# daveredrum/D3Net

Measured on AMD Instinct MI355X. Metric: scenes/sec fwd+bwd (PointGroup+speaker), higher is better.
Workload: dtype bf16

## Files before the change

d3net_amd/_lib.py:

```python
import ctypes as C
import os

_HERE = os.path.dirname(os.path.abspath(__file__))
SO_PATH = os.path.join(_HERE, "lib", "libd3hip.so")

ERRORS = {-1: "D3_ERR_WORKSPACE", -2: "D3_ERR_RANGE (coordinate/batch outside key range)",
          -3: "D3_ERR_ARG", -4: "D3_ERR_OVERFLOW"}


class D3Error(RuntimeError):
    pass


_lib = None
vp, i32, i64, f32, sz = C.c_void_p, C.c_int, C.c_longlong, C.c_float, C.c_size_t
f64 = C.c_double
pi = C.POINTER(C.c_int)

SIGNATURES = {
    "d3_version": (i32, []),
    "d3_arch": (C.c_char_p, []),
    "d3_sec_mean": (i32, [vp, vp, vp, i32, i32, vp]),
    "d3_sec_min": (i32, [vp, vp, vp, i32, i32, vp]),
    "d3_sec_max": (i32, [vp, vp, vp, i32, i32, vp]),
    "d3_cluster_select": (i32, [vp, vp, vp, vp, vp, i32, vp, vp, vp, vp, vp]),
    "d3_cluster_select2": (i32, [vp, vp, vp, vp, vp, i32, i32, vp, vp, vp, vp, vp, vp]),
    "d3_cluster_merge": (i32, [vp, i32, vp, i32, vp, i32, vp, i32, vp, vp, vp, vp, vp, vp]),
    "d3_proposal_prepare": (i32, [vp, vp, vp, i32, vp, vp, vp, vp, f32, f32, i32, vp, vp, vp, vp, vp]),
    "d3_cluster_coords_stats": (i32, [vp, vp, vp, vp, vp, vp, i32, vp]),
    "d3_cluster_coords_stats_ws_bytes": (sz, [i64]),
    "d3_cluster_coords_stats2": (i32, [vp, vp, vp, i64, vp, vp, vp, i32, vp, sz, vp]),
    "d3_cluster_transform": (i32, [vp, vp, vp, vp, vp, vp, i64, vp]),
    "d3_cluster_norm_params": (i32, [vp, vp, vp, i32, f32, f32, vp, vp, vp, vp, vp, vp]),
    "d3_roipool_fp": (i32, [vp, vp, vp, vp, i32, i32, vp]),
    "d3_roipool_bp": (i32, [vp, vp, vp, vp, i32, i32, vp]),
    "d3_get_iou": (i32, [vp, vp, vp, vp, vp, i32, i32, vp]),
    "d3_voxelize_fp": (i32, [vp, vp, vp, i32, i32, i32, i32, vp]),
    "d3_voxelize_fp2": (i32, [vp, i32, vp, i32, vp, vp, i32, i32, i32, vp]),
    "d3_voxelize_bp": (i32, [vp, vp, vp, i32, i32, i32, i32, vp]),
    "d3_point_recover_fp": (i32, [vp, vp, vp, i32, i32, i32, vp]),
    "d3_point_recover_bp": (i32, [vp, vp, vp, i32, i32, i32, vp]),
    "d3_voxelize_idx_ws_bytes": (sz, [i32]),
    "d3_voxelize_idx_count": (i32, [vp, i32, i32, i32, vp, vp, sz, pi, pi, vp]),
    "d3_voxelize_idx_fill": (i32, [vp, i32, i32, i32, vp, vp, sz, vp, vp, i32, i32, vp]),
    "d3_ballquery_ws_bytes": (sz, [i32]),
    "d3_ballquery_ws_bytes_single_pass": (sz, [i32]),
    "d3_ballquery_count": (i32, [vp, vp, vp, i32, f32, vp, vp, sz, pi, vp]),
    "d3_ballquery_fill": (i32, [vp, vp, vp, i32, f32, vp, vp, sz, vp, i64, vp]),
    "d3_ballquery_cap": (i32, []),
    "d3_ballquery_padded": (i32, [vp, vp, vp, i32, f32, vp, vp, sz, vp, vp]),
    "d3_bfs_cluster_ws_bytes": (sz, [i32]),
    "d3_bfs_cluster_erec_bytes": (sz, [i64]),
    "d3_bfs_cluster_run": (i32, [vp, vp, vp, i32, i32, vp, sz, vp, sz, i64, i32, vp, i64, vp, i64, pi, pi, vp]),
    "d3_bfs_cluster_begin": (i32, [vp, vp, vp, i32, i32, vp, sz, vp, sz, i64, i32, vp, i64, vp, i64, C.POINTER(vp), vp]),
    "d3_bfs_cluster_end": (i32, [vp, pi, pi]),
    "d3_coordmap_ws_bytes": (sz, [i32]),
    "d3_kmap_k3": (i32, [vp, i32, i32, vp, sz, vp, vp]),
    "d3_kmap_k3_pack16": (i32, [vp, i32, vp, vp, vp]),
    "d3_kmap_k3_16": (i32, [vp, i32, i32, vp, sz, vp, vp, vp, vp]),
    "d3_net_set_k3_16": (i32, [vp, vp, vp]),
    "d3_kmap_k3_q16_bytes": (sz, [i32]),
    "d3_kmap_k3_packq": (i32, [vp, i32, vp, vp, vp]),
    "d3_spconv_fwd3_nparts": (i32, [i32, i32, i32]),
    "d3_spconv_fwd3": (i32, [vp, i32, vp, vp, vp, i32, vp, i32, vp, vp, i32, i32, i32, i32, i32, vp]),
    "d3_spconv_fwd3_bnbwd": (i32, [vp, i32, vp, vp, vp, i32, vp, vp, vp, i32, vp, vp, vp, vp, f32, i32, i32, i32, i32, i32, i32, vp]),
    "d3_spconv_fwd3_launches": (i64, []),
    "d3_spconv_last_nparts": (i32, []),
    "d3_net_padded_channels": (i32, [vp]),
    "d3_net_padcast": (i32, [vp, vp, vp, i64, vp]),
    "d3_net_set_padded_input": (i32, [vp, vp]),
    "d3_spconv_t16_launches": (C.c_longlong, []),
    "d3_kmap_down_count": (i32, [vp, i32, i32, vp, sz, vp, vp, pi, vp]),
    "d3_kmap_down_fill": (i32, [vp, i32, i32, vp, sz, vp, vp, vp, vp, vp, i32, vp]),
    "d3_kmap_pyramid": (i32, [vp, i32, i32, vp, sz, vp, vp, vp, vp, vp, pi, vp]),
    "d3_kmap_pyramid_begin": (i32, [vp, i32, i32, vp, sz, vp, vp, vp, vp, vp, C.POINTER(C.c_void_p), vp]),
    "d3_kmap_pyramid_end": (i32, [vp, pi, i32]),
    "d3_kmap_down_fill2": (i32, [i32, i32, vp, vp, vp, vp, vp]),
    "d3_spconv_fwd": (i32, [vp, vp, vp, vp, i32, i32, i32, i32, i32, i32, vp]),
    "d3_spconv_wgrad": (i32, [vp, vp, vp, vp, i32, i32, i32, i32, i32, i32, vp]),
    "d3_spconv_pack_bytes": (sz, [i32, i32, i32]),
    "d3_spconv_pack_bytes_ex": (sz, [i32, i32, i32, i32]),
    "d3_spconv_pack": (i32, [vp, vp, i32, i32, i32, i32, vp]),
    "d3_spconv_fwd2_nparts": (i32, [i32, i32, i32, i32]),
    "d3_spconv_fwd2_nparts_ex": (i32, [i32, i32, i32, i32, i32]),
    "d3_spconv_fwd2_plan": (i32, [i32, i32, i32, i32, pi]),
    "d3_spconv_fwd2": (i32, [vp, i32, vp, vp, vp, i32, vp, i32, vp, i32, i32, i32, i32, i32, i32, vp]),
    "d3_spconv_fwd2_bnbwd": (i32, [vp, i32, vp, vp, vp, i32, vp, vp, i32, vp, vp, vp, vp, f32, i32, i32, i32, i32, i32, i32, i32, vp]),
    "d3_spconv_wgrad2_ws_bytes": (sz, [i32, i32, i32, i32, i32, i32]),
    "d3_spconv_wgrad2_splits": (i32, [i32, i32, i32, i32, i32, i32]),
    "d3_spconv_wgrad2": (i32, [vp, i32, vp, vp, i32, vp, i32, i32, i32, i32, i32, i32, i32, vp, sz, vp]),
    "d3_net_create": (vp, [vp, i32, vp, i32, vp, i32, i32, i32, i32, i32]),
    "d3_net_destroy": (None, [vp]),
    "d3_net_plan": (i32, [vp, vp, C.POINTER(sz), C.POINTER(sz)]),
    "d3_net_tensor_offset": (i64, [vp, i32]),
    "d3_net_describe": (i64, [vp, vp, i64]),
    "d3_net_forward": (i32, [vp, vp, vp, vp, vp, vp, vp, i32, vp]),
    "d3_net_backward": (i32, [vp, vp, vp, vp, vp, vp, vp, vp, vp, vp, vp, vp, vp]),
    "d3_tall_wgrad_ws_bytes": (sz, [i32, i32]),
    "d3_tall_wgrad": (i32, [vp, vp, vp, vp, i32, i32, i32, vp, sz, vp]),
    "d3_stack_to_batch": (i32, [vp, vp, vp, vp, vp, vp, i32, i32, i32, i32, i32, vp, vp, vp, vp, vp, vp, vp, vp, vp]),
    "d3_adamw_chunk": (i32, []),
    "d3_adamw": (i32, [vp, vp, vp, i32, f64, f64, f64, f64, f64, f64, f64, vp]),
    "d3_gather_rows_pad": (i32, [vp, i64, vp, vp, i64, i32, i32, vp]),
    "d3_point_heads_dy": (i32, [vp, vp, vp, i64, vp, vp]),
    "d3_point_heads_dx": (i32, [vp, vp, vp, vp, i64, i32, vp, vp]),
    "d3_point_heads_ws_bytes": (sz, []),
    "d3_point_heads_fwd": (i32, [vp, i64, i32, i32, vp, vp, vp, vp, vp, vp, vp, vp, f32, f32, i32, vp, vp, vp, vp, vp, vp, vp, vp, vp,
                                 vp, sz, vp]),
    "d3_score_loss": (i32, [vp, vp, i32, i32, f32, f32, vp, vp, vp, vp]),
    "d3_query_locals_mask": (i32, [vp, vp, i32, i32, i32, vp]),
    "d3_caption_select_target": (i32, [vp, vp, vp, i32, i32, i32, i32, vp, vp, vp, vp]),
    "d3_caption_inputs_fwd": (i32, [vp, vp, vp, vp, vp, i32, i32, i32, i32, i32, vp, vp, vp, vp, vp]),
    "d3_caption_inputs_bwd": (i32, [vp, vp, vp, vp, i32, i32, i32, i32, i32, vp, vp, vp]),
    "d3_masked_xe_ws_bytes": (sz, [i32, i32]),
    "d3_masked_xe": (i32, [vp, vp, i64, vp, i32, i32, i32, vp, vp, vp, sz, vp]),
    "d3_orientation_loss": (i32, [vp, i64, i64, vp, vp, vp, vp, vp, vp, i32, i32, i32, i32, i32, vp, i32, vp, vp, vp]),
    "d3_offset_loss_ws_bytes": (sz, []),
    "d3_offset_loss": (i32, [vp, vp, vp, i32, vp, i64, vp, vp, vp, i32, vp, sz, vp]),
    "d3_scatter_add_rows": (i32, [vp, vp, vp, i64, i32, vp]),
    "d3_gather_rows": (i32, [vp, vp, vp, i64, i32, vp]),
    "d3_cross_entropy_ws_bytes": (sz, []),
    "d3_cross_entropy": (i32, [vp, vp, vp, vp, i32, i32, i32, vp, sz, vp]),
    "d3_attn_fwd": (i32, [vp, vp, vp, vp, vp, vp, vp, i32, i32, i32, i32, i32, i32, i32, vp]),
    "d3_attn_bwd": (i32, [vp, vp, vp, vp, vp, vp, vp, vp, vp, i32, i32, i32, i32, i32, i32, vp]),
    "d3_scanrefer_match_groups": (i32, [i32, i32]),
    "d3_scanrefer_match_fwd": (i32, [vp, i32, vp]),
    "d3_scanrefer_match_bwd_ws_bytes": (sz, []),
    "d3_scanrefer_match_bwd": (i32, [vp, vp, i32, vp]),
    "d3_hgemm": (i32, [vp, i32, vp]),
    "d3_colsum_ws_bytes": (sz, [i32]),
    "d3_colsum": (i32, [vp, i64, i32, i32, vp, i32, vp, sz, vp]),
    "d3_topdown_ws_bytes": (sz, [i32, i32, i32, i32, i32, i32]),
    "d3_topdown_bwd_ws_bytes": (sz, [i32, i32, i32, i32, i32, i32, i32]),
    "d3_topdown_xe_forward": (i32, [vp, vp]),
    "d3_topdown_xe_backward": (i32, [vp, vp, vp]),
    "d3_topdown_xe_backward_ex": (i32, [vp, vp, vp, vp]),
    "d3_topdown_step_ws_bytes": (sz, [i32, i32, i32, i32, i32]),
    "d3_topdown_feat_proj": (i32, [vp, vp, vp, i32, i32, i32, vp]),
    "d3_topdown_step": (i32, [vp, vp, vp, i32, vp, vp, vp, vp, vp, vp, vp, sz, vp]),
    "d3_beam_select": (i32, [vp, vp, i32, i32, i32, i32, i32, i32, i32, i32, vp, vp, vp, vp, vp, vp, vp, vp, vp, vp, i32, vp]),
    "d3_greedy_select": (i32, [vp, i32, i32, vp, vp, vp]),
    "d3_topdown_greedy": (i32, [vp, vp, i32, vp, vp, vp, vp, vp, vp, vp, sz, vp, i32, vp, vp, vp]),
    "d3_topdown_beam": (i32, [vp, vp, i32, vp, vp, vp, vp, vp, sz, vp, i32, i32, vp, vp, vp, vp, vp, vp, vp]),
    "d3_topdown_beam_greedy": (i32, [vp, vp, i32, vp, vp, vp, vp, vp, sz, vp, i32, i32, vp, vp, vp, vp, vp, vp, i32, vp, vp, vp]),
    "d3_gru_seq_ws_bytes": (sz, [i32, i32, i32, i32]),
    "d3_gru_seq_bwd_ws_bytes": (sz, [i32, i32, i32, i32]),
    "d3_gru_seq_forward": (i32, [vp, vp, vp, vp, vp, vp, i32, i32, i32, i32, vp, vp, vp, sz, vp]),
    "d3_gru_seq_backward": (i32, [vp, vp, vp, vp, i32, i32, i32, i32, vp, vp, vp, vp, vp, vp, vp, vp, vp, sz, vp]),
    "d3_nms3d_samecls": (i32, [vp, vp, vp, i32, i32, f64, i32, vp, vp]),
    "d3_instance_cross_iou": (i32, [vp, vp, i64, i32, i32, vp, vp, vp, vp]),
    "d3_nms_matrix": (i32, [vp, vp, vp, i32, f32, vp, vp, vp, vp]),
    "d3_seg_eval_max_inst": (i32, []),
    "d3_seg_eval_ws_bytes": (sz, [i32, i32]),
    "d3_seg_eval": (i32, [vp, vp, vp, vp, i32, i32, i32, i32, vp, i32, vp, vp, i32, i64, C.c_ulonglong, vp, vp, vp, vp, vp, vp, sz, vp]),
    "d3_lsap_batched": (i32, [vp, vp, i32, i32, i32, vp, vp, vp]),
    "d3_dense_caption_assign": (i32, [vp, vp, vp, i32, i32, i32, vp, vp, vp, vp]),
    "d3_det_match": (i32, [vp, vp, vp, vp, f64, vp, vp, vp, i32, i32, i32, i32, C.POINTER(f64), i32, vp, vp, vp, vp, vp, vp, vp, vp, vp]),
    "d3_det_ap": (i32, [vp, vp, vp, i32, i64, i32, i32, vp, vp]),
    "d3_caption_collect": (i32, [vp, vp, vp, vp, vp, vp, vp, vp, vp, vp, i32, i32, i32, i32, i32, i32, i32, i32, i32, i32, i64, vp, vp, vp,
                                 vp, vp, vp, vp]),
    "d3_caption_stats": (i32, [vp, i32, vp, vp, i32, vp, vp, vp, i32, vp, vp, vp]),
    "d3_scene_limits": (i32, [pi, pi, pi]),
    "d3_scene_transform": (i32, [vp, i32, vp, f64, i32, vp, vp, vp]),
    "d3_scene_reduce": (i32, [vp, vp, i32, vp, vp]),
    "d3_scene_noise": (i32, [vp, i64, C.c_ulonglong, vp]),
    "d3_scene_elastic_ws_bytes": (sz, [i32, i32, i32]),
    "d3_scene_elastic": (i32, [vp, i32, vp, vp, i32, i32, i32, f64, vp, sz, vp]),
    "d3_scene_offset": (i32, [vp, i32, vp, i32, vp]),
    "d3_scene_crop_count": (i32, [vp, i32, vp, vp, vp, vp, vp]),
    "d3_scene_ws_bytes": (sz, [i32, i32]),
    "d3_scene_emit": (i32, [vp, vp, vp, i32, vp, vp, i32, vp, vp, i32, vp, vp, vp, vp, vp, vp, vp, sz, vp]),
    "d3_scene_relabel": (i32, [vp, i32, i32, vp, sz, vp]),
    "d3_scene_instances": (i32, [vp, vp, vp, i32, i32, i32, i32, vp, vp, vp, vp, vp, vp, vp, vp, sz, vp]),
    "d3_lang_features_ws_bytes": (sz, [i32, i32]),
    "d3_lang_features": (i32, [vp, vp, i32, vp, i32, i32, i32, i32, vp, vp, vp, i32, vp, vp, vp, vp, sz, vp]),
    "d3_ref_targets_ws_bytes": (sz, [i32]),
    "d3_ref_targets": (i32, [vp, vp, vp, vp, i32, i32, i32, vp, vp, vp, i32, vp, vp, vp, vp, vp, vp, sz, vp]),
    "d3_multiview_limits": (i32, [pi, pi, pi]),
    "d3_multiview_project_ws_bytes": (sz, [i32, i32]),
    "d3_multiview_project": (i32, [vp, i32, vp, vp, vp, i32, C.POINTER(f64), i32, i32, vp, vp, vp, sz, vp]),
    "d3_multiview_project_frame": (i32, [vp, i32, i32, vp, vp, i32, vp, vp]),
    "d3_multiview_fuse_ws_bytes": (sz, [i32, i32, i32]),
    "d3_multiview_fuse": (i32, [vp, i32, vp, vp, vp, i32, C.POINTER(f64), i32, i32, vp, i32, i32, vp, vp, vp, sz, vp]),
    "d3_enet_layers": (i32, [vp, i32]),
    "d3_enet_param_count": (i64, []),
    "d3_enet_preprocess": (i32, [vp, i32, i32, i32, vp, vp, i32, i32, vp, vp]),
    "d3_enet_ws_bytes": (sz, [i32, i32, i32]),
    "d3_enet_forward": (i32, [vp, i32, i32, i32, vp, i64, vp, i32, i32, vp, vp, sz, vp]),
    "d3_scan_limits": (i32, [pi, pi, pi, pi, pi]),
    "d3_scan_mesh_ws_bytes": (sz, [i32, i32]),
    "d3_scan_mesh": (i32, [vp, i32, vp, i32, C.POINTER(f64), vp, vp, vp, vp, sz, vp]),
    "d3_scan_labels_ws_bytes": (sz, [i32, i32, i32, i32, i32]),
    "d3_scan_labels": (i32, [vp, vp, i32, i32, vp, vp, i32, vp, vp, i32, i32, vp, vp, vp, vp, vp, vp, vp, vp, vp, sz, vp]),
    "d3_cider_ws_bytes": (sz, [i32, i32, i32]),
    "d3_cider_scores": (i32, [vp, i32, vp, vp, vp, vp, vp, i32, i32, vp, i32, vp, i32, i32, f64, i32, vp, vp, vp, sz, vp]),
    "d3_graph_edges": (i32, [vp, vp, i32, i32, i32, vp, vp, vp, vp, vp, vp, vp, vp, vp, vp, vp]),
    "d3_edgeconv_ws_bytes": (sz, [i32, i32, i32]),
    "d3_edgeconv_bwd_ws_bytes": (sz, [i32, i32, i32]),
    "d3_edgeconv_fwd": (i32, [vp, vp, vp, vp, vp, vp, vp, vp, vp, i32, i32, i32, i32, i32, vp, vp, vp, sz, vp]),
    "d3_edgeconv_bwd": (i32, [vp, vp, vp, vp, vp, vp, vp, vp, i32, i32, i32, i32, i32, vp, vp, vp, vp, vp, vp, vp, vp, vp, sz, vp]),
    "d3_query_locals_dist": (i32, [vp, vp, vp, i32, i32, i32, f32, i32, vp]),
    "d3_prof_enable": (i32, [i32]),
    "d3_net_set_chunks": (i32, [vp, vp, i32]),
    "d3_net_chunk_wait": (i32, [vp, i32, vp]),
    "d3_layernorm_fwd": (i32, [vp, vp, vp, vp, vp, vp, vp, i32, i32, f32, vp]),
    "d3_layernorm_ws_bytes": (sz, [i32, i32]),
    "d3_layernorm_bwd": (i32, [vp, vp, vp, vp, vp, vp, vp, vp, vp, i32, i32, vp, sz, vp]),
    "d3_tuning_set": (i32, [C.c_char_p, i32]),
    "d3_tuning_get": (i32, [C.c_char_p, vp]),
    "d3_tuning_count": (i32, []),
    "d3_tuning_name": (C.c_char_p, [i32]),
    "d3_prof_collect": (i32, [i32, C.POINTER(C.c_longlong), C.POINTER(C.c_double), C.POINTER(C.c_double),
                              C.POINTER(C.c_double)]),
    "d3_prof_dump": (i32, [i32, C.POINTER(C.c_double), i32, C.POINTER(i32)]),
    "d3_bn_ws_bytes": (sz, [i32]),
    "d3_bn_stats": (i32, [vp, i32, i32, vp, vp, vp, vp, f32, vp, sz, vp]),
    "d3_bn_relu_fwd": (i32, [vp, vp, vp, vp, vp, vp, i32, i32, f32, i32, vp]),
    "d3_bn_relu_fwd_bf16": (i32, [vp, vp, vp, vp, vp, vp, i32, i32, f32, i32, vp]),
    "d3_bn_relu_bwd": (i32, [vp, vp, vp, vp, vp, vp, vp, vp, vp, i32, i32, f32, i32, vp, sz, vp]),
}


class GemmSeg(C.Structure):
    _fields_ = [("A", vp), ("ia", vp), ("lda", i64), ("a_kmajor", i32), ("B", vp), ("ldb", i64), ("b_kmajor", i32), ("K", i32)]


class GemmProb(C.Structure):
    _fields_ = [("seg", GemmSeg * 3), ("nseg", i32), ("M", i32), ("N", i32), ("C", vp), ("ldc", i64), ("bias", vp), ("add", vp),
                ("ldadd", i64), ("relu", i32), ("accum", i32), ("perm_nb", i32), ("perm_s", i32),
                ("gru", i32), ("gru_H", i32), ("g_d0", vp), ("g_ld0", i64), ("g_d1", vp), ("g_ld1", i64),
                ("g_r", vp), ("g_z", vp), ("g_n", vp), ("g_ghn", vp), ("g_hp", vp), ("g_ldh", i64),
                ("g_dgi", vp), ("g_lddgi", i64), ("g_dgh", vp), ("g_dhp", vp)]


SRM_PARAMS = ("W0", "b0", "g1", "be1", "rm1", "rv1", "alpha", "W3", "b3", "W4", "b4", "g2", "be2", "rm2", "rv2", "W5", "b5", "g3", "be3",
              "rm3", "rv3", "w6", "b6")
SRM_GRADS = ("dW0", "db0", "dg1", "dbe1", "dalpha", "dW3", "db3", "dW4", "db4", "dg2", "dbe2", "dW5", "db5", "dg3", "dbe3", "dw6", "db6")


class SrmArgs(C.Structure):
    _fields_ = ([(k, i32) for k in ("B", "K", "N", "div", "m", "L")] + [(k, vp) for k in ("feats", "lang", "mask")] +
                [(k, vp) for k in SRM_PARAMS] + [("eps", f32 * 3), ("momentum", f32 * 3), ("nbt", vp * 3)] +
                [(k, vp) for k in ("PQ", "part", "x1", "f", "y2", "z2", "y3", "bnstat", "conf")])


class SrmGrads(C.Structure):
    _fields_ = ([("dconf", vp)] + [(k, vp) for k in SRM_GRADS] + [(k, vp) for k in ("dfeats", "dlang")] +
                [(k, vp) for k in ("dpre3", "dz2", "dpre2", "df", "dbn1", "dP", "dQ", "db0part", "part")] +
                [("ws", vp), ("ws_bytes", sz)])


TOPDOWN_PARAMS = ("W_td", "b_td", "Wih1", "Whh1", "bih1", "bhh1", "W_feat", "W_hidd", "w_att", "W_lang", "b_lang",
                  "Wih2", "Whh2", "bih2", "bhh2", "Wc0", "bc0", "Wc2", "bc2")


class TopdownArgs(C.Structure):
    _fields_ = ([(k, i32) for k in ("N", "K", "S", "V", "H", "E", "F", "Tw")] +
                [(k, vp) for k in ("word_ids", "emb", "target", "obj", "mask")] + [(k, vp) for k in TOPDOWN_PARAMS] +
                [("logits", vp), ("attn", vp), ("ws", vp), ("ws_bytes", sz)])


class TopdownGrads(C.Structure):
    _fields_ = ([("dlogits", vp)] + [("d" + k, vp) for k in TOPDOWN_PARAMS] +
                [("dobj", vp), ("dtarget", vp), ("ws", vp), ("ws_bytes", sz)])


class tuning:

    def __init__(self, **switches):
        self.switches, self.saved = switches, {}

    def __enter__(self):
        l = lib()
        for k, v in self.switches.items():
            old = C.c_int(0)
            check(l.d3_tuning_get(k.encode(), C.byref(old)), "tuning_get(%s)" % k)
            self.saved[k] = old.value
            check(l.d3_tuning_set(k.encode(), int(v)), "tuning_set(%s)" % k)
        return self

    def __exit__(self, *exc):
        l = lib()
        for k, v in self.saved.items():
            l.d3_tuning_set(k.encode(), v)
        return False


def lib():
    global _lib
    if _lib is None:
        if not os.path.exists(SO_PATH):
            raise D3Error("libd3hip.so not built (%s); run `python -m d3net_amd.build` -- "
                          "d3net_amd has no CPU/eager fallback" % SO_PATH)
        import torch
        l = C.CDLL(SO_PATH)
        for name, (res, args) in SIGNATURES.items():
            fn = getattr(l, name)
            fn.restype = res
            fn.argtypes = args
        _lib = l
    return _lib


def check(rc, what):
    if rc != 0:
        raise D3Error("%s failed: %s" % (what, ERRORS.get(rc, "hipError_t %d" % rc)))
```

d3net_amd/csrc/seg_ops.hip:

```cpp
#include "dispatch.h"

#define SEG_THREADS 256

template <bool IS_MAX>
__global__ __launch_bounds__(SEG_THREADS) void sec_minmax_kernel(const float *__restrict__ inp,
                                                                const int *__restrict__ offsets,
                                                                float *__restrict__ out, int nProposal, int C) {
    __shared__ float red[SEG_THREADS];
    const int active = (SEG_THREADS / C) * C;
    const int t = threadIdx.x;
    for (int p = blockIdx.x; p < nProposal; p += gridDim.x) {
        const int start = offsets[p], end = offsets[p + 1];
        const long long base = (long long)start * C;
        const long long total = (long long)(end - start) * C;
        float v = IS_MAX ? -INFINITY : INFINITY;
        if (t < active) {
            for (long long f = t; f < total; f += active) {
                float x = inp[base + f];
                if (IS_MAX ? (x > v) : (x < v)) v = x;
            }
        }
        red[t] = v;
        __syncthreads();
        if (t < C) {
            float r = red[t];
            for (int k = t + C; k < active; k += C) {
                float x = red[k];
                if (IS_MAX ? (x > r) : (x < r)) r = x;
            }
            out[(long long)p * C + t] = r;
        }
        __syncthreads();
    }
}

#define MEAN_CHUNK 2048
__global__ __launch_bounds__(SEG_THREADS) void sec_mean_kernel(const float *__restrict__ inp,
                                                              const int *__restrict__ offsets,
                                                              float *__restrict__ out, int nProposal, int C) {
    __shared__ float stage[MEAN_CHUNK];
    const int t = threadIdx.x;
    const int rows_per_chunk = MEAN_CHUNK / C;
    for (int p = blockIdx.x; p < nProposal; p += gridDim.x) {
        const int start = offsets[p], end = offsets[p + 1];
        const float count = (float)(end - start);
        float mean = 0.f;
        for (int r0 = start; r0 < end; r0 += rows_per_chunk) {
            const int rows = min(rows_per_chunk, end - r0);
            const int nflt = rows * C;
            const long long base = (long long)r0 * C;
            for (int f = t; f < nflt; f += SEG_THREADS) stage[f] = __fdiv_rn(inp[base + f], count);
            __syncthreads();
            if (t < C) {
                int r = 0;
                for (; r + 8 <= rows; r += 8) {
                    float v[8];
#pragma unroll
                    for (int j = 0; j < 8; j++) v[j] = stage[(r + j) * C + t];
#pragma unroll
                    for (int j = 0; j < 8; j++) mean = __fadd_rn(mean, v[j]);
                }
                for (; r < rows; r++) mean = __fadd_rn(mean, stage[r * C + t]);
            }
            __syncthreads();
        }
        if (t < C) out[(long long)p * C + t] = mean;
    }
}

#define MEANW_CHUNK 1024
#define MEANW_PB 16
#define MEANW_WAVES(NP) ((NP) <= 3 ? (NP) + 1 : (NP) + 1 + ((NP) - 1) / 3)
#define MEANW_PROD 3
template <int NPROD>
__global__ __launch_bounds__(MEANW_WAVES(NPROD) * 64) void sec_mean_pc_kernel(const float *__restrict__ inp, const int *__restrict__ offsets,
                                                         float *__restrict__ out, int nProposal, int C, const int *__restrict__ gidx, int prediv) {
    extern __shared__ __attribute__((aligned(16))) float meanw_smem[];
    float (*stage)[NPROD][MEANW_CHUNK] = (float (*)[NPROD][MEANW_CHUNK])meanw_smem;
    constexpr int MEANW_PROD_ = NPROD;
    const int lane = threadIdx.x & 63, wave = threadIdx.x >> 6, p = blockIdx.x;
    const int start = offsets[p], end = offsets[p + 1];
    const float count = (float)(end - start);
    const int rpc0 = MEANW_CHUNK / C, rpc = rpc0 >= 256 ? (rpc0 & ~255) : (rpc0 >= 64 ? (rpc0 & ~63) : (rpc0 & ~3)), cf = rpc * C;
    if (rpc == 0) return;
    const long long base = (long long)start * C, total = (long long)(end - start) * C;
    const int nchunk = (int)((total + cf - 1) / cf);
    const int nround = (nchunk + MEANW_PROD_ - 1) / MEANW_PROD_;
    const unsigned int invC = (65536u + C - 1) / C;
    float mean = 0.f;
    if (NPROD > 3 && wave == 0) __builtin_amdgcn_s_setprio(3);
    const int pslot = NPROD <= 3 ? wave - 1 : ((wave & 3) ? wave - 1 - (wave >> 2) : -1);
    for (int rd = 0; rd <= nround; rd++) {
        if (pslot >= 0) {
            const int k = rd * MEANW_PROD_ + pslot;
            if (rd < nround && k < nchunk) {
                float *st = stage[rd & 1][pslot];
                const long long cb = (long long)k * cf;
                int lz;
                asm volatile("v_mov_b32 %0, %1" : "=v"(lz) : "v"(lane));
#pragma unroll
                for (int hf = 0; hf < 16 / MEANW_PB; hf++) {
                    float v[MEANW_PB];
                    int rowj[MEANW_PB], cj[MEANW_PB];
                    bool okj[MEANW_PB];
                    unsigned int src[MEANW_PB];
#pragma unroll
                    for (int j = 0; j < MEANW_PB; j++) {
                        const int f = (hf * MEANW_PB + j) * 64 + lz;
                        okj[j] = f < cf && cb + f < total;
                        rowj[j] = (int)(((unsigned int)f * invC) >> 16); cj[j] = f - rowj[j] * C;
                    }
                    if (gidx) {
                        int pt[MEANW_PB];
                        const int *gi = gidx + ((long long)start + (long long)k * rpc) * 2 + 1;
#pragma unroll
                        for (int j = 0; j < MEANW_PB; j++) pt[j] = gi[(okj[j] ? rowj[j] : 0) * 2];
#pragma unroll
                        for (int j = 0; j < MEANW_PB; j++) src[j] = (unsigned int)pt[j] * (unsigned int)C + (unsigned int)cj[j];
#pragma unroll
                        for (int j = 0; j < MEANW_PB; j++) v[j] = inp[src[j]];
                    } else {
                        const float *ib = inp + base + cb;
#pragma unroll
                        for (int j = 0; j < MEANW_PB; j++) v[j] = ib[okj[j] ? (hf * MEANW_PB + j) * 64 + lz : 0];
                    }
#pragma unroll
                    for (int j = 0; j < MEANW_PB; j++) {
                        const int f = (hf * MEANW_PB + j) * 64 + lz;
                        if (f < cf) st[cj[j] * rpc + rowj[j]] = okj[j] ? (prediv ? v[j] : __fdiv_rn(v[j], count)) : 0.f;
                    }
                }
            }
        } else if (wave == 0 && rd > 0) {
            for (int q = 0; q < MEANW_PROD_; q++) {
                const int k = (rd - 1) * MEANW_PROD_ + q;
                if (k >= nchunk) break;
                const float *st = stage[(rd - 1) & 1][q] + lane * rpc;
                const long long left = total - (long long)k * cf;
                const int rows = (int)((left < cf ? left : cf) / C);
                if (lane < C) {
                    int r = 0;
#define MEANW_LD(W, R0)  _Pragma("unroll") for (int j = 0; j < 8; j++) W[j] = *(const float4 *)(st + (R0) + j * 4)
#define MEANW_ADD(W)     _Pragma("unroll") for (int j = 0; j < 8; j++) { mean = __fadd_rn(mean, W[j].x); mean = __fadd_rn(mean, W[j].y); mean = __fadd_rn(mean, W[j].z); mean = __fadd_rn(mean, W[j].w); }
                    for (; r + 256 <= rows; r += 256) {
                        float4 g0[8], g1[8], g2[8], g3[8], g4[8], g5[8], g6[8], g7[8];
                        MEANW_LD(g0, r); MEANW_LD(g1, r + 32);
                        __builtin_amdgcn_sched_barrier(0);
                        MEANW_ADD(g0); __builtin_amdgcn_sched_barrier(0); MEANW_LD(g2, r + 64); __builtin_amdgcn_sched_barrier(0);
                        MEANW_ADD(g1); __builtin_amdgcn_sched_barrier(0); MEANW_LD(g3, r + 96); __builtin_amdgcn_sched_barrier(0);
                        MEANW_ADD(g2); __builtin_amdgcn_sched_barrier(0); MEANW_LD(g4, r + 128); __builtin_amdgcn_sched_barrier(0);
                        MEANW_ADD(g3); __builtin_amdgcn_sched_barrier(0); MEANW_LD(g5, r + 160); __builtin_amdgcn_sched_barrier(0);
                        MEANW_ADD(g4); __builtin_amdgcn_sched_barrier(0); MEANW_LD(g6, r + 192); __builtin_amdgcn_sched_barrier(0);
                        MEANW_ADD(g5); __builtin_amdgcn_sched_barrier(0); MEANW_LD(g7, r + 224); __builtin_amdgcn_sched_barrier(0);
                        MEANW_ADD(g6); __builtin_amdgcn_sched_barrier(0);
                        MEANW_ADD(g7); __builtin_amdgcn_sched_barrier(0);
                    }
                    for (; r + 32 <= rows; r += 32) {
                        float4 g0[8];
                        MEANW_LD(g0, r);
                        MEANW_ADD(g0);
                    }
#undef MEANW_LD
#undef MEANW_ADD
                    for (; r + 4 <= rows; r += 4) {
                        const float4 w = *(const float4 *)(st + r);
                        mean = __fadd_rn(mean, w.x); mean = __fadd_rn(mean, w.y); mean = __fadd_rn(mean, w.z); mean = __fadd_rn(mean, w.w);
                    }
                    for (; r < rows; r++) mean = __fadd_rn(mean, st[r]);
                }
            }
        }
        __syncthreads();
    }
    if (wave == 0 && lane < C) out[(long long)p * C + lane] = mean;
}

__global__ __launch_bounds__(SEG_THREADS) void roipool_fp_kernel(const float *__restrict__ feats,
                                                                const int *__restrict__ offsets,
                                                                float *__restrict__ out_feats,
                                                                int *__restrict__ out_maxidx, int nProposal, int C) {
    __shared__ float redv[SEG_THREADS];
    __shared__ int redi[SEG_THREADS];
    const int active = (SEG_THREADS / C) * C;
    const int rows_per_pass = active / C;
    const int t = threadIdx.x;
    for (int p = blockIdx.x; p < nProposal; p += gridDim.x) {
        const int start = offsets[p], end = offsets[p + 1];
        float v = -INFINITY;
        int a = -1;
        if (t < active) {
            const int c = t % C;
            for (int r = start + t / C; r < end; r += rows_per_pass) {
                float x = feats[(long long)r * C + c];
                if (x > v) { v = x; a = r; }
            }
        }
        redv[t] = v; redi[t] = a;
        __syncthreads();
        if (t < C) {
            float bv = redv[t]; int bi = redi[t];
            for (int k = t + C; k < active; k += C) {
                float x = redv[k]; int xi = redi[k];
                if (x > bv || (x == bv && xi < bi)) { bv = x; bi = xi; }
            }
            out_feats[(long long)p * C + t] = bv;
            out_maxidx[(long long)p * C + t] = bi;
        }
        __syncthreads();
    }
}

__global__ void roipool_bp_kernel(float *__restrict__ d_feats, const int *__restrict__ maxidx,
                                  const float *__restrict__ d_out, long long total, int C) {
    long long e = (long long)blockIdx.x * blockDim.x + threadIdx.x;
    if (e >= total) return;
    int a = maxidx[e];
    if (a >= 0) atomicAdd(&d_feats[(long long)a * C + (int)(e % C)], d_out[e]);
}

#define IOU_BINS 8192
__global__ __launch_bounds__(SEG_THREADS) void get_iou_kernel(const int *__restrict__ proposals_idx,
                                                             const int *__restrict__ offsets,
                                                             const int64_t *__restrict__ instance_labels,
                                                             const int *__restrict__ instance_pointnum,
                                                             float *__restrict__ iou, int nInstance, int nProposal) {
    __shared__ int hist[IOU_BINS];
    const int t = threadIdx.x;
    for (int p = blockIdx.x; p < nProposal; p += gridDim.x) {
        const int start = offsets[p], end = offsets[p + 1];
        const int proposal_total = end - start;
        for (int w0 = 0; w0 < nInstance; w0 += IOU_BINS) {
            const int wn = min(IOU_BINS, nInstance - w0);
            for (int b = t; b < wn; b += SEG_THREADS) hist[b] = 0;
            __syncthreads();
            for (int i0 = start + t; i0 < end; i0 += 8 * SEG_THREADS) {
                int pi[8];
                int64_t lb[8];
#pragma unroll
                for (int j = 0; j < 8; j++) { const int i = i0 + j * SEG_THREADS; pi[j] = proposals_idx[i < end ? i : start]; }
#pragma unroll
                for (int j = 0; j < 8; j++) lb[j] = instance_labels[pi[j]];
#pragma unroll
                for (int j = 0; j < 8; j++) {
                    const int lab = (int)lb[j] - w0;
                    if (i0 + j * SEG_THREADS < end && lab >= 0 && lab < wn) atomicAdd(&hist[lab], 1);
                }
            }
            __syncthreads();
            for (int b = t; b < wn; b += SEG_THREADS) {
                int inter = hist[b];
                int instance_total = instance_pointnum[w0 + b];
                double denom = (double)(float)(proposal_total + instance_total - inter) + 1e-5;
                iou[(long long)p * nInstance + w0 + b] = (float)((double)(float)inter / denom);
            }
            __syncthreads();
        }
    }
}

#define SEG_FLAT_GRID 1024

__device__ __forceinline__ void seg_atomic_max_f32(float *addr, float v) {
    if (v >= 0.f) atomicMax((int *)addr, __float_as_int(v));
    else atomicMin((unsigned int *)addr, __float_as_uint(v));
}
__device__ __forceinline__ void seg_atomic_min_f32(float *addr, float v) {
    if (v >= 0.f) atomicMin((int *)addr, __float_as_int(v));
    else atomicMax((unsigned int *)addr, __float_as_uint(v));
}
__device__ __forceinline__ int seg_find(const int *__restrict__ offsets, int nProposal, int r) {
    int lo = 0, hi = nProposal - 1;
    while (lo < hi) { const int mid = (lo + hi + 1) >> 1; if (offsets[mid] <= r) lo = mid; else hi = mid - 1; }
    return lo;
}
__global__ void seg_init_kernel(float *f, int *i, long long n, float fval, int ival) {
    const long long e = (long long)blockIdx.x * blockDim.x + threadIdx.x;
    if (e >= n) return;
    f[e] = fval;
    if (i) i[e] = ival;
}
template <bool IS_MAX>
__global__ __launch_bounds__(SEG_THREADS) void seg_minmax_flat_kernel(const float *__restrict__ inp,
                                                                     const int *__restrict__ offsets,
                                                                     float *__restrict__ out, int nProposal, int C) {
    __shared__ float red[SEG_THREADS];
    const int active = (SEG_THREADS / C) * C, rpp = active / C, t = threadIdx.x;
    const int c = t % C;
    const int total = offsets[nProposal], first = offsets[0];
    int per = (total - first + gridDim.x - 1) / gridDim.x;
    per = (per + rpp - 1) / rpp * rpp;
    const int R0 = first + blockIdx.x * per, R1 = min(total, R0 + per);
    if (R0 >= R1) return;
    const int p0 = seg_find(offsets, nProposal, R0);
    if (offsets[p0 + 1] >= R1) {
        float v = IS_MAX ? -INFINITY : INFINITY;
        if (t < active)
            for (int r = R0 + t / C; r < R1; r += rpp) {
                const float x = inp[(long long)r * C + c];
                if (IS_MAX ? (x > v) : (x < v)) v = x;
            }
        red[t] = v;
        __syncthreads();
        if (t < C) {
            float b = red[t];
            for (int k = t + C; k < active; k += C) { const float x = red[k]; if (IS_MAX ? (x > b) : (x < b)) b = x; }
            if (IS_MAX ? (b > -INFINITY) : (b < INFINITY)) {
                if (IS_MAX) seg_atomic_max_f32(&out[(long long)p0 * C + t], b); else seg_atomic_min_f32(&out[(long long)p0 * C + t], b);
            }
        }
        return;
    }
    if (t >= active) return;
    int r = R0 + t / C;
    if (r >= R1) return;
    int p = seg_find(offsets, nProposal, r);
    int pend = offsets[p + 1];
    float v = IS_MAX ? -INFINITY : INFINITY;
    bool any = false;
    for (; r < R1; r += rpp) {
        if (r >= pend) {
            if (any) { if (IS_MAX) seg_atomic_max_f32(&out[(long long)p * C + c], v); else seg_atomic_min_f32(&out[(long long)p * C + c], v); }
            while (r >= pend) { p++; pend = offsets[p + 1]; }
            v = IS_MAX ? -INFINITY : INFINITY; any = false;
        }
        const float x = inp[(long long)r * C + c];
        if (IS_MAX ? (x > v) : (x < v)) { v = x; any = true; }
    }
    if (any) { if (IS_MAX) seg_atomic_max_f32(&out[(long long)p * C + c], v); else seg_atomic_min_f32(&out[(long long)p * C + c], v); }
}
__global__ __launch_bounds__(SEG_THREADS) void seg_minmax_gather_kernel(const float *__restrict__ inp, const int *__restrict__ gidx,
                                                                       const int *__restrict__ offsets, float *__restrict__ omin,
                                                                       float *__restrict__ omax, int nProposal, int C) {
    __shared__ float rmin[SEG_THREADS], rmax[SEG_THREADS];
    const int active = (SEG_THREADS / C) * C, rpp = active / C, t = threadIdx.x;
    const int c = t % C;
    const int total = offsets[nProposal], first = offsets[0];
    int per = (total - first + gridDim.x - 1) / gridDim.x;
    per = (per + rpp - 1) / rpp * rpp;
    const int R0 = first + blockIdx.x * per, R1 = min(total, R0 + per);
    if (R0 >= R1) return;
    const int p0 = seg_find(offsets, nProposal, R0);
    if (offsets[p0 + 1] >= R1) {
        float lo = INFINITY, hi = -INFINITY;
        if (t < active)
            for (int r = R0 + t / C; r < R1; r += rpp) {
                const float x = inp[(long long)gidx[(long long)r * 2 + 1] * C + c];
                if (x < lo) lo = x;
                if (x > hi) hi = x;
            }
        rmin[t] = lo; rmax[t] = hi;
        __syncthreads();
        if (t < C) {
            float a = rmin[t], b = rmax[t];
            for (int k = t + C; k < active; k += C) { if (rmin[k] < a) a = rmin[k]; if (rmax[k] > b) b = rmax[k]; }
            if (a < INFINITY) seg_atomic_min_f32(&omin[(long long)p0 * C + t], a);
            if (b > -INFINITY) seg_atomic_max_f32(&omax[(long long)p0 * C + t], b);
        }
        return;
    }
    if (t >= active) return;
    int r = R0 + t / C;
    if (r >= R1) return;
    int p = seg_find(offsets, nProposal, r);
    int pend = offsets[p + 1];
    float lo = INFINITY, hi = -INFINITY;
    bool any = false;
    for (; r < R1; r += rpp) {
        if (r >= pend) {
            if (any) { seg_atomic_min_f32(&omin[(long long)p * C + c], lo); seg_atomic_max_f32(&omax[(long long)p * C + c], hi); }
            while (r >= pend) { p++; pend = offsets[p + 1]; }
            lo = INFINITY; hi = -INFINITY; any = false;
        }
        const float x = inp[(long long)gidx[(long long)r * 2 + 1] * C + c];
        if (x < lo) lo = x;
        if (x > hi) hi = x;
        any = true;
    }
    if (any) { seg_atomic_min_f32(&omin[(long long)p * C + c], lo); seg_atomic_max_f32(&omax[(long long)p * C + c], hi); }
}
__global__ void cluster_transform_kernel(const float *__restrict__ coords, const int *__restrict__ cidx, const float *__restrict__ mean,
                                         const float *__restrict__ scale, const float *__restrict__ offset, long long *__restrict__ out,
                                         long long S) {
    const long long r = (long long)blockIdx.x * blockDim.x + threadIdx.x;
    if (r >= S) return;
    const int cl = cidx[r * 2], pt = cidx[r * 2 + 1];
    const float sc = scale[cl];
    long long o[4];
    o[0] = cl;
#pragma unroll
    for (int k = 0; k < 3; k++) {
        const float v = __fadd_rn(__fmul_rn(__fsub_rn(coords[(long long)pt * 3 + k], mean[(long long)cl * 3 + k]), sc), offset[(long long)cl * 3 + k]);
        o[k + 1] = (long long)v;
    }
    long long *op = out + r * 4;
    op[0] = o[0]; op[1] = o[1]; op[2] = o[2]; op[3] = o[3];
}

__global__ void cluster_norm_kernel(const float *__restrict__ mean, const float *__restrict__ raw_min, const float *__restrict__ raw_max,
                                    int P, float fullscale, float scale_cap, float r00, float r01, float r02, float r10, float r11,
                                    float r12, float *__restrict__ size, float *__restrict__ center, float *__restrict__ cscale,
                                    float *__restrict__ offset) {
    const int p = blockIdx.x * blockDim.x + threadIdx.x;
    if (p >= P) return;
    const float inv_full = __fdiv_rn(1.f, fullscale);
    const float r0[3] = {r00, r01, r02}, r1[3] = {r10, r11, r12};
    float cmin[3], cmax[3], mx = -INFINITY;
    bool nan = false;
#pragma unroll
    for (int k = 0; k < 3; k++) {
        const float m = mean[p * 3 + k];
        cmin[k] = __fsub_rn(raw_min[p * 3 + k], m);
        cmax[k] = __fsub_rn(raw_max[p * 3 + k], m);
        const float ext = __fsub_rn(cmax[k], cmin[k]);
        size[p * 3 + k] = ext;
        center[p * 3 + k] = __fadd_rn(__fmul_rn(__fadd_rn(cmax[k], cmin[k]), 0.5f), m);
        const float d = __fmul_rn(ext, inv_full);
        nan |= d != d;
        mx = fmaxf(mx, d);
    }
    if (nan) mx = NAN;
    float sc = __fsub_rn(__fdiv_rn(1.f, mx), 0.01f);
    sc = (sc != sc) ? sc : fminf(sc, scale_cap);
    cscale[p] = sc;
#pragma unroll
    for (int k = 0; k < 3; k++) {
        const float lo = __fmul_rn(cmin[k], sc), hi = __fmul_rn(cmax[k], sc);
        const float rng = __fsub_rn(hi, lo);
        const float room = __fsub_rn(fullscale, rng);
        float a = __fsub_rn(room, 0.001f), b = __fadd_rn(room, 0.001f);
        a = (a != a) ? a : fmaxf(a, 0.f);
        b = (b != b) ? b : fminf(b, 0.f);
        offset[p * 3 + k] = __fadd_rn(__fadd_rn(-lo, __fmul_rn(a, r0[k])), __fmul_rn(b, r1[k]));
    }
}
extern "C" int d3_cluster_norm_params(const float *mean, const float *raw_min, const float *raw_max, int P, float fullscale,
                                      float scale_cap, const float *rand6, float *size, float *center, float *cscale, float *offset,
                                      void *stream) {
    D3_CLEAR();
    if (P <= 0) return 0;
    if (!rand6) return D3_ERR_ARG;
    cluster_norm_kernel<<<(P + 255) / 256, 256, 0, d3_stream(stream)>>>(mean, raw_min, raw_max, P, fullscale, scale_cap, rand6[0], rand6[1],
                                                                         rand6[2], rand6[3], rand6[4], rand6[5], size, center, cscale, offset);
    D3_LAUNCH_CHECK();
    return 0;
}

__global__ __launch_bounds__(SEG_THREADS) void roipool_arg_flat_kernel(const float *__restrict__ feats,
                                                                      const int *__restrict__ offsets,
                                                                      const float *__restrict__ out_feats,
                                                                      int *__restrict__ out_maxidx, int nProposal, int C) {
    __shared__ int redi[SEG_THREADS];
    const int active = (SEG_THREADS / C) * C, rpp = active / C, t = threadIdx.x;
    const int c = t % C;
    const int total = offsets[nProposal], first = offsets[0];
    int per = (total - first + gridDim.x - 1) / gridDim.x;
    per = (per + rpp - 1) / rpp * rpp;
    const int R0 = first + blockIdx.x * per, R1 = min(total, R0 + per);
    if (R0 >= R1) return;
    const int p0 = seg_find(offsets, nProposal, R0);
    if (offsets[p0 + 1] >= R1) {
        int a = 0x7FFFFFFF;
        if (t < active) {
            const float mx = out_feats[(long long)p0 * C + c];
            for (int r = R0 + t / C; r < R1; r += rpp)
                if (feats[(long long)r * C + c] == mx) { a = r; break; }
        }
        redi[t] = a;
        __syncthreads();
        if (t < C) {
            int b = redi[t];
            for (int k = t + C; k < active; k += C) b = min(b, redi[k]);
            if (b != 0x7FFFFFFF) atomicMin((unsigned int *)&out_maxidx[(long long)p0 * C + t], (unsigned int)b);
        }
        return;
    }
    if (t >= active) return;
    int r = R0 + t / C;
    if (r >= R1) return;
    int p = seg_find(offsets, nProposal, r);
    int pend = offsets[p + 1];
    float mx = out_feats[(long long)p * C + c];
    int a = -1;
    for (; r < R1; r += rpp) {
        if (r >= pend) {
            if (a >= 0) atomicMin((unsigned int *)&out_maxidx[(long long)p * C + c], (unsigned int)a);
            while (r >= pend) { p++; pend = offsets[p + 1]; }
            mx = out_feats[(long long)p * C + c]; a = -1;
        }
        if (a < 0 && feats[(long long)r * C + c] == mx) a = r;
    }
    if (a >= 0) atomicMin((unsigned int *)&out_maxidx[(long long)p * C + c], (unsigned int)a);
}

static inline int seg_grid(int nProposal) { return nProposal < 65535 ? nProposal : 65535; }

extern "C" int d3_sec_mean(const float *inp, const int *offsets, float *out, int nProposal, int C, void *stream) {
    D3_CLEAR();
    if (nProposal <= 0) return 0;
    if (C <= 0 || C > SEG_THREADS) return D3_ERR_ARG;
    if (C <= 64) sec_mean_pc_kernel<MEANW_PROD><<<nProposal, 256, 2 * MEANW_PROD * MEANW_CHUNK * sizeof(float) + 256, d3_stream(stream)>>>(inp, offsets, out, nProposal, C, nullptr, 0);
    else sec_mean_kernel<<<seg_grid(nProposal), SEG_THREADS, 0, d3_stream(stream)>>>(inp, offsets, out, nProposal, C);
    D3_LAUNCH_CHECK();
    return 0;
}
extern "C" int d3_sec_min(const float *inp, const int *offsets, float *out, int nProposal, int C, void *stream) {
    D3_CLEAR();
    if (nProposal <= 0) return 0;
    if (C <= 0 || C > SEG_THREADS) return D3_ERR_ARG;
    const long long n = (long long)nProposal * C;
    seg_init_kernel<<<(int)((n + 255) / 256), 256, 0, d3_stream(stream)>>>(out, nullptr, n, INFINITY, 0);
    seg_minmax_flat_kernel<false><<<SEG_FLAT_GRID, SEG_THREADS, 0, d3_stream(stream)>>>(inp, offsets, out, nProposal, C);
    D3_LAUNCH_CHECK();
    return 0;
}
extern "C" int d3_sec_max(const float *inp, const int *offsets, float *out, int nProposal, int C, void *stream) {
    D3_CLEAR();
    if (nProposal <= 0) return 0;
    if (C <= 0 || C > SEG_THREADS) return D3_ERR_ARG;
    const long long n = (long long)nProposal * C;
    seg_init_kernel<<<(int)((n + 255) / 256), 256, 0, d3_stream(stream)>>>(out, nullptr, n, -INFINITY, 0);
    seg_minmax_flat_kernel<true><<<SEG_FLAT_GRID, SEG_THREADS, 0, d3_stream(stream)>>>(inp, offsets, out, nProposal, C);
    D3_LAUNCH_CHECK();
    return 0;
}
extern "C" int d3_roipool_fp(const float *feats, const int *proposals_offset, float *output_feats,
                             int *output_maxidx, int nProposal, int C, void *stream) {
    D3_CLEAR();
    if (nProposal <= 0) return 0;
    if (C <= 0 || C > SEG_THREADS) return D3_ERR_ARG;
    hipStream_t s = d3_stream(stream);
    const long long n = (long long)nProposal * C;
    seg_init_kernel<<<(int)((n + 255) / 256), 256, 0, s>>>(output_feats, output_maxidx, n, -INFINITY, -1);
    seg_minmax_flat_kernel<true><<<SEG_FLAT_GRID, SEG_THREADS, 0, s>>>(feats, proposals_offset, output_feats, nProposal, C);
    roipool_arg_flat_kernel<<<SEG_FLAT_GRID, SEG_THREADS, 0, s>>>(feats, proposals_offset, output_feats, output_maxidx, nProposal, C);
    D3_LAUNCH_CHECK();
    return 0;
}
extern "C" int d3_roipool_bp(float *d_feats, const int *proposals_offset, const int *output_maxidx,
                             const float *d_output_feats, int nProposal, int C, void *stream) {
    D3_CLEAR();
    (void)proposals_offset;
    long long total = (long long)nProposal * C;
    if (total <= 0) return 0;
    int blocks = (int)((total + 255) / 256);
    roipool_bp_kernel<<<blocks, 256, 0, d3_stream(stream)>>>(d_feats, output_maxidx, d_output_feats, total, C);
    D3_LAUNCH_CHECK();
    return 0;
}
extern "C" int d3_get_iou(const int *proposals_idx, const int *proposals_offset, const int64_t *instance_labels,
                          const int *instance_pointnum, float *proposals_iou, int nInstance, int nProposal,
                          void *stream) {
    D3_CLEAR();
    if (nProposal <= 0 || nInstance <= 0) return 0;
    get_iou_kernel<<<seg_grid(nProposal), SEG_THREADS, 0, d3_stream(stream)>>>(
        proposals_idx, proposals_offset, instance_labels, instance_pointnum, proposals_iou, nInstance, nProposal);
    D3_LAUNCH_CHECK();
    return 0;
}

__global__ void cluster_quot_kernel(const float *__restrict__ coords, const int *__restrict__ clusters_idx, const int *__restrict__ offsets,
                                    float *__restrict__ q, long long S, int nProposal) {
    const long long t = (long long)blockIdx.x * blockDim.x + threadIdx.x;
    if (t >= S * 3) return;
    const long long e = t / 3;
    const int ch = (int)(t - e * 3);
    const int pt = clusters_idx[e * 2 + 1];
    int lo = 0, hi = nProposal;
    while (hi - lo > 1) { const int m = (lo + hi) >> 1; if ((long long)offsets[m] <= e) lo = m; else hi = m; }
    const int c = lo;
    const float count = (float)(offsets[c + 1] - offsets[c]);
    q[t] = __fdiv_rn(coords[(long long)pt * 3 + ch], count);
}

static int cluster_mean_launch(const float *inp, const int *offsets, float *mean, int nProposal, const int *gidx, int prediv, hipStream_t s) {
    constexpr int NP = 6;
    const size_t lds = (size_t)2 * NP * MEANW_CHUNK * sizeof(float) + 256;
    if (const int rc = d3_allow_lds<sec_mean_pc_kernel<NP>>((int)lds)) return rc;
    sec_mean_pc_kernel<NP><<<nProposal, MEANW_WAVES(NP) * 64, lds, s>>>(inp, offsets, mean, nProposal, 3, gidx, prediv);
    return 0;
}

static int cluster_minmax_launch(const float *coords, const int *clusters_idx, const int *offsets, float *cmin, float *cmax, int nProposal, hipStream_t s);

extern "C" int d3_cluster_coords_stats(const float *coords, const int *clusters_idx, const int *offsets, float *mean, float *cmin,
                                       float *cmax, int nProposal, void *stream) {
    D3_CLEAR();
    if (nProposal <= 0) return 0;
    hipStream_t s = d3_stream(stream);
    int rc = cluster_mean_launch(coords, offsets, mean, nProposal, clusters_idx, 0, s);
    if (rc) return rc;
    return cluster_minmax_launch(coords, clusters_idx, offsets, cmin, cmax, nProposal, s);
}

extern "C" size_t d3_cluster_coords_stats_ws_bytes(long long S) { return (size_t)(S > 0 ? S : 1) * 3 * sizeof(float); }
extern "C" int d3_cluster_coords_stats2(const float *coords, const int *clusters_idx, const int *offsets, long long S, float *mean, float *cmin,
                                        float *cmax, int nProposal, void *ws, size_t ws_bytes, void *stream) {
    D3_CLEAR();
    if (nProposal <= 0) return 0;
    if (S < 0 || ws == nullptr || ws_bytes < d3_cluster_coords_stats_ws_bytes(S)) return D3_ERR_WORKSPACE;
    hipStream_t s = d3_stream(stream);
    float *q = (float *)ws;
    if (S > 0) cluster_quot_kernel<<<(int)((S * 3 + 255) / 256), 256, 0, s>>>(coords, clusters_idx, offsets, q, S, nProposal);
    int rc = cluster_mean_launch(q, offsets, mean, nProposal, nullptr, 1, s);
    if (rc) return rc;
    return cluster_minmax_launch(coords, clusters_idx, offsets, cmin, cmax, nProposal, s);
}

static int cluster_minmax_launch(const float *coords, const int *clusters_idx, const int *offsets, float *cmin, float *cmax, int nProposal, hipStream_t s) {
    const long long n = (long long)nProposal * 3;
    seg_init_kernel<<<(int)((n + 255) / 256), 256, 0, s>>>(cmin, nullptr, n, INFINITY, 0);
    seg_init_kernel<<<(int)((n + 255) / 256), 256, 0, s>>>(cmax, nullptr, n, -INFINITY, 0);
    seg_minmax_gather_kernel<<<SEG_FLAT_GRID, SEG_THREADS, 0, s>>>(coords, clusters_idx, offsets, cmin, cmax, nProposal, 3);
    D3_LAUNCH_CHECK();
    return 0;
}
extern "C" int d3_cluster_transform(const float *coords, const int *clusters_idx, const float *mean, const float *scale,
                                    const float *offset, long long *out, long long S, void *stream) {
    D3_CLEAR();
    if (S <= 0) return 0;
    cluster_transform_kernel<<<(int)((S + 255) / 256), 256, 0, d3_stream(stream)>>>(coords, clusters_idx, mean, scale, offset, out, S);
    D3_LAUNCH_CHECK();
    return 0;
}
```

d3net_amd/csrc/voxelize.hip:

```cpp
#include "common.h"

__global__ void voxelize_fp_kernel(const float *__restrict__ feats, float *__restrict__ out,
                                   const int *__restrict__ rules, long long total, int maxActive, int nPlanes,
                                   bool average) {
    long long e = (long long)blockIdx.x * blockDim.x + threadIdx.x;
    if (e >= total) return;
    const int row = (int)(e / nPlanes), plane = (int)(e % nPlanes);
    const int *r = rules + (long long)row * (maxActive + 1);
    const int nActive = r[0];
    int id[4];
#pragma unroll
    for (int j = 0; j < 4; j++) id[j] = r[j < maxActive ? 1 + j : 0];
    float acc = out[e];
    const float multiplier = (average && nActive > 0) ? __fdiv_rn(1.0f, (float)nActive) : 1.0f;
    float v[4];
#pragma unroll
    for (int j = 0; j < 4; j++) v[j] = feats[(long long)(j < nActive ? id[j] : 0) * nPlanes + plane];
#pragma unroll
    for (int j = 0; j < 4; j++)
        if (j < nActive) acc = __fadd_rn(acc, __fmul_rn(multiplier, v[j]));
    for (int i0 = 5; i0 <= nActive; i0 += 8) {
        int idn[8];
        float vn[8];
#pragma unroll
        for (int j = 0; j < 8; j++) idn[j] = r[i0 + j <= nActive ? i0 + j : 0];
#pragma unroll
        for (int j = 0; j < 8; j++) vn[j] = feats[(long long)(i0 + j <= nActive ? idn[j] : 0) * nPlanes + plane];
#pragma unroll
        for (int j = 0; j < 8; j++)
            if (i0 + j <= nActive) acc = __fadd_rn(acc, __fmul_rn(multiplier, vn[j]));
    }
    out[e] = acc;
}

__global__ void voxelize_fp2_kernel(const float *__restrict__ fa, int Ca, const float *__restrict__ fb, int Cb, float *__restrict__ out,
                                    const int *__restrict__ rules, long long total, int maxActive, bool average) {
    long long e = (long long)blockIdx.x * blockDim.x + threadIdx.x;
    if (e >= total) return;
    const int nPlanes = Ca + Cb;
    const int row = (int)(e / nPlanes), plane = (int)(e % nPlanes);
    const int *r = rules + (long long)row * (maxActive + 1);
    const bool ina = plane < Ca;
    const float *src = ina ? fa : fb;
    const int ld = ina ? Ca : Cb, col = ina ? plane : plane - Ca;
    const int nActive = r[0];
    int id[4];
#pragma unroll
    for (int j = 0; j < 4; j++) id[j] = r[j < maxActive ? 1 + j : 0];
    float acc = 0.f;
    const float multiplier = (average && nActive > 0) ? __fdiv_rn(1.0f, (float)nActive) : 1.0f;
    float v[4];
#pragma unroll
    for (int j = 0; j < 4; j++) v[j] = src[(long long)(j < nActive ? id[j] : 0) * ld + col];
#pragma unroll
    for (int j = 0; j < 4; j++)
        if (j < nActive) acc = __fadd_rn(acc, __fmul_rn(multiplier, v[j]));
    for (int i0 = 5; i0 <= nActive; i0 += 8) {
        int idn[8];
        float vn[8];
#pragma unroll
        for (int j = 0; j < 8; j++) idn[j] = r[i0 + j <= nActive ? i0 + j : 0];
#pragma unroll
        for (int j = 0; j < 8; j++) vn[j] = src[(long long)(i0 + j <= nActive ? idn[j] : 0) * ld + col];
#pragma unroll
        for (int j = 0; j < 8; j++)
            if (i0 + j <= nActive) acc = __fadd_rn(acc, __fmul_rn(multiplier, vn[j]));
    }
    out[e] = acc;
}

__global__ __launch_bounds__(256) void voxelize_fp2_rows_kernel(const float *__restrict__ fa, int Ca, const float *__restrict__ fb, int Cb,
                                                               float *__restrict__ out, const int *__restrict__ rules, int M, int maxActive,
                                                               bool average) {
    const int lane = threadIdx.x & 63;
    const long long row = (long long)blockIdx.x * 4 + (threadIdx.x >> 6);
    if (row >= M) return;
    const int nPlanes = Ca + Cb;
    const int *r = rules + row * (maxActive + 1);
    const int rv = (lane <= maxActive && lane < 5) ? r[lane] : 0;
    const int nActive = __shfl(rv, 0);
    int id[4];
#pragma unroll
    for (int j = 0; j < 4; j++) id[j] = __shfl(rv, 1 + j);
    const float multiplier = (average && nActive > 0) ? __fdiv_rn(1.0f, (float)nActive) : 1.0f;
    for (int p0 = 0; p0 < nPlanes; p0 += 192) {
        float v[3][4];
#pragma unroll
        for (int q = 0; q < 3; q++) {
            const int plane = p0 + q * 64 + lane;
            const bool on = plane < nPlanes;
            const bool ina = plane < Ca || !on;
            const float *src = ina ? fa : fb;
            const int ld = ina ? Ca : Cb, col = on ? (ina ? plane : plane - Ca) : 0;
#pragma unroll
            for (int j = 0; j < 4; j++) v[q][j] = src[(long long)((on && j < nActive) ? id[j] : 0) * ld + col];
        }
#pragma unroll
        for (int q = 0; q < 3; q++) {
            const int plane = p0 + q * 64 + lane;
            if (plane >= nPlanes) continue;
            float acc = 0.f;
#pragma unroll
            for (int j = 0; j < 4; j++)
                if (j < nActive) acc = __fadd_rn(acc, __fmul_rn(multiplier, v[q][j]));
            if (nActive > 4) {
                const bool ina = plane < Ca;
                const float *src = ina ? fa : fb;
                const int ld = ina ? Ca : Cb, col = ina ? plane : plane - Ca;
                for (int i = 5; i <= nActive; i++) acc = __fadd_rn(acc, __fmul_rn(multiplier, src[(long long)r[i] * ld + col]));
            }
            out[row * nPlanes + plane] = acc;
        }
    }
}

__global__ void voxelize_bp_kernel(const float *__restrict__ d_out, float *__restrict__ d_feats,
                                   const int *__restrict__ rules, long long total, int maxActive, int nPlanes,
                                   bool average) {
    long long e = (long long)blockIdx.x * blockDim.x + threadIdx.x;
    if (e >= total) return;
    const int row = (int)(e / nPlanes), plane = (int)(e % nPlanes);
    const int *r = rules + (long long)row * (maxActive + 1);
    const int nActive = r[0];
    const float multiplier = (average && nActive > 0) ? __fdiv_rn(1.0f, (float)nActive) : 1.0f;
    const float g = __fmul_rn(multiplier, d_out[e]);
    for (int i0 = 1; i0 <= nActive; i0 += 8) {
        int idn[8];
#pragma unroll
        for (int j = 0; j < 8; j++) idn[j] = r[i0 + j <= nActive ? i0 + j : 0];
#pragma unroll
        for (int j = 0; j < 8; j++)
            if (i0 + j <= nActive) atomicAdd(&d_feats[(long long)idn[j] * nPlanes + plane], g);
    }
}

static int launch_fp(const float *feats, float *out, const int *rules, int nActive, int maxActive, int nPlane,
                     bool average, void *stream) {
    long long total = (long long)nActive * nPlane;
    if (total <= 0) return 0;
    voxelize_fp_kernel<<<(int)((total + 255) / 256), 256, 0, d3_stream(stream)>>>(feats, out, rules, total, maxActive,
                                                                                nPlane, average);
    D3_LAUNCH_CHECK();
    return 0;
}
static int launch_bp(const float *d_out, float *d_feats, const int *rules, int nActive, int maxActive, int nPlane,
                     bool average, void *stream) {
    long long total = (long long)nActive * nPlane;
    if (total <= 0) return 0;
    voxelize_bp_kernel<<<(int)((total + 255) / 256), 256, 0, d3_stream(stream)>>>(d_out, d_feats, rules, total,
                                                                                maxActive, nPlane, average);
    D3_LAUNCH_CHECK();
    return 0;
}

extern "C" int d3_voxelize_fp(const float *feats, float *output_feats, const int *output_map, int mode, int nActive,
                              int maxActive, int nPlane, void *stream) {
    D3_CLEAR();
    return launch_fp(feats, output_feats, output_map, nActive, maxActive, nPlane, mode == 4, stream);
}
extern "C" int d3_voxelize_fp2(const float *feats_a, int Ca, const float *feats_b, int Cb, float *output_feats, const int *output_map,
                               int mode, int nActive, int maxActive, void *stream) {
    D3_CLEAR();
    if (Ca < 1 || Cb < 0) return D3_ERR_ARG;
    const long long total = (long long)nActive * (Ca + Cb);
    if (total <= 0) return 0;
    if (Ca + Cb >= 48)
        voxelize_fp2_rows_kernel<<<(nActive + 3) / 4, 256, 0, d3_stream(stream)>>>(feats_a, Ca, feats_b, Cb, output_feats, output_map, nActive,
                                                                                  maxActive, mode == 4);
    else
        voxelize_fp2_kernel<<<(int)((total + 255) / 256), 256, 0, d3_stream(stream)>>>(feats_a, Ca, feats_b, Cb, output_feats, output_map, total,
                                                                                     maxActive, mode == 4);
    D3_LAUNCH_CHECK();
    return 0;
}
extern "C" int d3_voxelize_bp(const float *d_output_feats, float *d_feats, const int *output_map, int mode,
                              int nActive, int maxActive, int nPlane, void *stream) {
    D3_CLEAR();
    return launch_bp(d_output_feats, d_feats, output_map, nActive, maxActive, nPlane, mode == 4, stream);
}
extern "C" int d3_point_recover_fp(const float *feats, float *output_feats, const int *idx_map, int nActive,
                                   int maxActive, int nPlane, void *stream) {
    D3_CLEAR();
    return launch_bp(feats, output_feats, idx_map, nActive, maxActive, nPlane, false, stream);
}
extern "C" int d3_point_recover_bp(const float *d_output_feats, float *d_feats, const int *idx_map, int nActive,
                                   int maxActive, int nPlane, void *stream) {
    D3_CLEAR();
    return launch_fp(d_output_feats, d_feats, idx_map, nActive, maxActive, nPlane, false, stream);
}

#define VI_EMPTY 0xFFFFFFFFFFFFFFFFull

struct VoxIdxWs {
    unsigned long long *keys;
    int *first;
    int *slot_vid;
    int *slot_of;
    int *flag;
    int *scan;
    int *cnt;
    int *vstart;
    int *sorted_pts;
    int *sorted_keys;
    int *scalars;
    void *temp; size_t temp_bytes;
    size_t cap;
};

static size_t vi_cap(int n) { size_t c = 1024; while (c < (size_t)n * 2) c <<= 1; return c; }

static void vi_layout(D3Carver &c, int n, VoxIdxWs &w) {
    size_t nn = (size_t)(n > 0 ? n : 1);
    w.cap = vi_cap(n);
    w.keys = c.take<unsigned long long>(w.cap);
    w.first = c.take<int>(w.cap);
    w.slot_vid = c.take<int>(w.cap);
    w.slot_of = c.take<int>(nn);
    w.flag = c.take<int>(nn);
    w.scan = c.take<int>(nn);
    w.cnt = c.take<int>(nn);
    w.vstart = c.take<int>(nn);
    w.sorted_pts = c.take<int>(nn);
    w.sorted_keys = c.take<int>(nn);
    w.scalars = c.take<int>(64);
    size_t t1 = d3_scan_temp_bytes(n), t2 = d3_sort_pairs_temp_bytes(n);
    w.temp_bytes = t1 > t2 ? t1 : t2;
    w.temp = c.take<char>(w.temp_bytes);
}
static bool vi_carve(void *ws, size_t ws_bytes, int n, VoxIdxWs &w) {
    D3Carver c(ws, ws_bytes);
    vi_layout(c, n, w);
    return c.ok();
}

extern "C" size_t d3_voxelize_idx_ws_bytes(int n) {
    D3Carver c(nullptr, 0);
    VoxIdxWs w;
    vi_layout(c, n, w);
    return c.off + 256;
}

__device__ __forceinline__ unsigned long long vi_hash(unsigned long long k) {
    k ^= k >> 33; k *= 0xff51afd7ed558ccdull; k ^= k >> 33; k *= 0xc4ceb9fe1a85ec53ull; k ^= k >> 33;
    return k;
}

__device__ __forceinline__ bool vi_pack(const int64_t *c, int ncols, unsigned long long &key) {
    int b = 0, x, y, z;
    if (ncols == 4) { b = (int)c[0]; x = (int)c[1]; y = (int)c[2]; z = (int)c[3]; }
    else { x = (int)c[0]; y = (int)c[1]; z = (int)c[2]; }
    const int B = 1 << 14;
    bool ok = (b >= 0 && b < (1 << 19)) && (x >= -B && x < B) && (y >= -B && y < B) && (z >= -B && z < B);
    key = ((unsigned long long)(unsigned)b << 45) | ((unsigned long long)(unsigned)(x + B) << 30) |
          ((unsigned long long)(unsigned)(y + B) << 15) | (unsigned long long)(unsigned)(z + B);
    return ok;
}

__global__ void vi_init_kernel(unsigned long long *keys, int *first, size_t cap, int *cnt, int n, int *scalars) {
    size_t i = (size_t)blockIdx.x * blockDim.x + threadIdx.x;
    if (i < cap) { keys[i] = VI_EMPTY; first[i] = 0x7FFFFFFF; }
    if (i < (size_t)n) cnt[i] = 0;
    if (i < 8) scalars[i] = 0;
}

__global__ void vi_insert_kernel(const int64_t *__restrict__ coords, int n, int ncols, unsigned long long *keys,
                                 int *first, size_t cap, int *slot_of, int *scalars) {
    const int i = blockIdx.x * blockDim.x + threadIdx.x, lane = threadIdx.x & 63;
    const bool live = i < n;
    unsigned long long key = VI_EMPTY;
    if (live && !vi_pack(coords + (size_t)i * ncols, ncols, key)) { scalars[2] = 1; key &= ~(1ull << 63); }
    const unsigned long long pk = __shfl_up(key, 1);
    const bool head = live && (lane == 0 || pk != key);
    const unsigned long long heads = __ballot(head);
    int myslot = 0;
    if (head) {
        size_t slot = vi_hash(key) & (cap - 1);
        bool done = false;
        for (size_t probe = 0; probe < cap; probe++) {
            unsigned long long prev = atomicCAS(&keys[slot], VI_EMPTY, key);
            if (prev == VI_EMPTY || prev == key) { atomicMin(&first[slot], i); myslot = (int)slot; done = true; break; }
            slot = (slot + 1) & (cap - 1);
        }
        if (!done) scalars[2] = 2;
    }
    const unsigned long long below = heads & (lane == 63 ? ~0ull : ((2ull << lane) - 1ull));
    const int hl = below ? 63 - __builtin_clzll(below) : lane;
    myslot = __shfl(myslot, hl);
    if (live) slot_of[i] = myslot;
}

__global__ void vi_flag_kernel(const int *first, const int *slot_of, int *flag, int n) {
    int i = blockIdx.x * blockDim.x + threadIdx.x;
    if (i < n) flag[i] = (first[slot_of[i]] == i) ? 1 : 0;
}
__global__ void vi_assign_kernel(const int *flag, const int *scan, const int *slot_of, int *slot_vid, int n) {
    int i = blockIdx.x * blockDim.x + threadIdx.x;
    if (i < n && flag[i]) slot_vid[slot_of[i]] = scan[i];
}
__global__ void vi_p2v_kernel(const int *slot_of, const int *slot_vid, int *input_map, int *cnt, int n,
                              int *scalars) {
    const int i = blockIdx.x * blockDim.x + threadIdx.x, lane = threadIdx.x & 63;
    const bool live = i < n;
    int v = -1;
    if (live) { v = slot_vid[slot_of[i]]; input_map[i] = v; }
    const int prev = __shfl_up(v, 1);
    const bool head = live && (lane == 0 || prev != v);
    const unsigned long long heads = __ballot(head), lives = __ballot(live);
    if (head) {
        const unsigned long long above = (lane == 63) ? 0ull : (heads >> (lane + 1)) << (lane + 1);
        const int end = above ? (int)__builtin_ctzll(above) : 64;
        const unsigned long long span = (end == 64 ? ~0ull : ((1ull << end) - 1ull)) & ~((1ull << lane) - 1ull);
        atomicAdd(&cnt[v], (int)__popcll(span & lives));
    }
    (void)scalars;
}
__global__ void vi_max_kernel(const int *__restrict__ cnt, int n, int *scalars) {
    const int i = blockIdx.x * blockDim.x + threadIdx.x, lane = threadIdx.x & 63;
    const int M = scalars[0];
    if ((int)(blockIdx.x * blockDim.x) >= M) return;
    int c = (i < M && i < n) ? cnt[i] : 0;
    for (int o = 32; o > 0; o >>= 1) c = max(c, __shfl_xor(c, o));
    if (lane == 0 && c > 0 && c > __hip_atomic_load(&scalars[1], __ATOMIC_RELAXED, __HIP_MEMORY_SCOPE_AGENT)) atomicMax(&scalars[1], c);
}
__global__ void vi_total_kernel(const int *flag, const int *scan, int n, int *scalars) {
    if (threadIdx.x == 0 && blockIdx.x == 0) scalars[0] = n > 0 ? scan[n - 1] + flag[n - 1] : 0;
}

extern "C" int d3_voxelize_idx_count(const int64_t *coords, int n, int ncols, int mode, int *input_map, void *ws,
                                     size_t ws_bytes, int *M_host, int *maxActive_host, void *stream) {
    D3_CLEAR();
    if (ncols != 3 && ncols != 4) return D3_ERR_ARG;
    if (mode < 0 || mode > 4) return D3_ERR_ARG;
    *M_host = 0; *maxActive_host = 1;
    if (n <= 0) return 0;
    VoxIdxWs w;
    if (!vi_carve(ws, ws_bytes, n, w)) return D3_ERR_WORKSPACE;
    hipStream_t s = d3_stream(stream);
    const int T = 256;
    size_t initn = w.cap > (size_t)n ? w.cap : (size_t)n;
    vi_init_kernel<<<(int)((initn + T - 1) / T), T, 0, s>>>(w.keys, w.first, w.cap, w.cnt, n, w.scalars);
    const int nb = (n + T - 1) / T;
    vi_insert_kernel<<<nb, T, 0, s>>>(coords, n, ncols, w.keys, w.first, w.cap, w.slot_of, w.scalars);
    vi_flag_kernel<<<nb, T, 0, s>>>(w.first, w.slot_of, w.flag, n);
    int rc = d3_exclusive_scan_i32(w.flag, w.scan, n, w.temp, w.temp_bytes, s);
    if (rc) return rc;
    vi_assign_kernel<<<nb, T, 0, s>>>(w.flag, w.scan, w.slot_of, w.slot_vid, n);
    vi_p2v_kernel<<<nb, T, 0, s>>>(w.slot_of, w.slot_vid, input_map, w.cnt, n, w.scalars);
    vi_total_kernel<<<1, 64, 0, s>>>(w.flag, w.scan, n, w.scalars);
    vi_max_kernel<<<nb, T, 0, s>>>(w.cnt, n, w.scalars);
    D3_LAUNCH_CHECK();
    int h[3];
    D3_CHECK(hipMemcpyAsync(h, w.scalars, sizeof(h), hipMemcpyDeviceToHost, s));
    D3_CHECK(hipStreamSynchronize(s));
    if (h[2] == 1) return D3_ERR_RANGE;
    if (h[2] == 2) return D3_ERR_OVERFLOW;
    *M_host = h[0];
    *maxActive_host = (mode == 3 || mode == 4) ? (h[1] > 1 ? h[1] : 1) : 1;
    return 0;
}

__global__ __launch_bounds__(256) void vi_rules_kernel(int mode, const int *__restrict__ cnt, const int *__restrict__ vstart,
                                                       const int *__restrict__ sorted_pts, int *__restrict__ out_map, int M,
                                                       int maxActive, int gshift) {
    const int G = 1 << gshift, w = maxActive + 1;
    const long long t = (long long)blockIdx.x * blockDim.x + threadIdx.x;
    const long long v = t >> gshift;
    if (v >= M) return;
    const int j0 = (int)(t & (G - 1));
    const int c = cnt[v];
    const int *pts = sorted_pts + vstart[v];
    int *row = out_map + v * w;
    for (int j = j0; j < w; j += G) {
        int val;
        if (mode == 3 || mode == 4) val = (j == 0) ? c : (j - 1 < c ? pts[j - 1] : 0);
        else val = (j == 0) ? 1 : ((mode == 2) ? pts[c - 1] : pts[0]);
        row[j] = val;
    }
}
__global__ void vi_coords_kernel(const int64_t *__restrict__ coords, int ncols, int mode,
                                 const int *__restrict__ cnt, const int *__restrict__ vstart,
                                 const int *__restrict__ sorted_pts, int64_t *__restrict__ out_coords, int M) {
    int e = blockIdx.x * blockDim.x + threadIdx.x;
    if (e >= M * ncols) return;
    const int v = e / ncols, j = e % ncols;
    const int *pts = sorted_pts + vstart[v];
    const int firstListed = (mode == 2) ? pts[cnt[v] - 1] : pts[0];
    out_coords[e] = coords[(size_t)firstListed * ncols + j];
}

__global__ void vi_iota_kernel(int *a, int n) {
    int i = blockIdx.x * blockDim.x + threadIdx.x;
    if (i < n) a[i] = i;
}

extern "C" int d3_voxelize_idx_fill(const int64_t *coords, int n, int ncols, int mode, const int *input_map,
                                    void *ws, size_t ws_bytes, int64_t *output_coords, int *output_map, int M,
                                    int maxActive, void *stream) {
    D3_CLEAR();
    if (n <= 0 || M <= 0) return 0;
    VoxIdxWs w;
    if (!vi_carve(ws, ws_bytes, n, w)) return D3_ERR_WORKSPACE;
    hipStream_t s = d3_stream(stream);
    const int T = 256;
    int rc = d3_exclusive_scan_i32(w.cnt, w.vstart, M, w.temp, w.temp_bytes, s);
    if (rc) return rc;
    vi_iota_kernel<<<(n + T - 1) / T, T, 0, s>>>(w.flag, n);
    int bits = 1; while ((1ll << bits) < (long long)M && bits < 31) bits++;
    rc = d3_sort_pairs_i32(input_map, w.sorted_keys, w.flag, w.sorted_pts, n, bits, w.temp, w.temp_bytes, s);
    if (rc) return rc;
    int gshift = 0; while ((1 << gshift) < maxActive + 1 && gshift < 6) gshift++;
    const long long rthreads = (long long)M << gshift;
    vi_rules_kernel<<<(int)((rthreads + T - 1) / T), T, 0, s>>>(mode, w.cnt, w.vstart, w.sorted_pts, output_map, M, maxActive, gshift);
    vi_coords_kernel<<<(M * ncols + T - 1) / T, T, 0, s>>>(coords, ncols, mode, w.cnt, w.vstart, w.sorted_pts,
                                                         output_coords, M);
    D3_LAUNCH_CHECK();
    return 0;
}
```

d3net_amd/pointgroup.py:

```python
import functools
import threading

import numpy as np
import torch
import torch.nn as nn

from . import common
from . import heads
from . import minkowski as ME
from . import nativelinear
from . import netexec
from . import pointgroup_ops


class _HostStage:

    def __init__(self, slots=64, nbytes=4096):
        self.slots, self.nbytes, self.ring, self.i = slots, nbytes, None, 0

    def put(self, t, device):
        if self.ring is None:
            self.ring = [torch.empty(self.nbytes, dtype=torch.uint8).pin_memory() for _ in range(self.slots)]
        t = t.contiguous()
        n = t.numel() * t.element_size()
        if n > self.nbytes:
            return t.to(device)
        pin = self.ring[self.i][:n].view(t.dtype).view(t.shape)
        self.i = (self.i + 1) % self.slots
        pin.copy_(t)
        return torch.empty(t.shape, dtype=t.dtype, device=device).copy_(pin, non_blocking=True)


_STAGE = _HostStage()
_CONST = {}


def _const(key, device, build):
    k = (key, device.index)
    if k not in _CONST:
        _CONST[k] = build().to(device)
    return _CONST[k]


_WORKER = None


def _cluster_worker():
    global _WORKER
    if _WORKER is None:
        import concurrent.futures
        _WORKER = concurrent.futures.ThreadPoolExecutor(max_workers=1, thread_name_prefix="d3-cluster")
    return _WORKER


_PF_WORKER = None


def _prefetch_worker():
    global _PF_WORKER
    if _PF_WORKER is None:
        import concurrent.futures
        _PF_WORKER = concurrent.futures.ThreadPoolExecutor(max_workers=1, thread_name_prefix="d3-prefetch")
    return _PF_WORKER


class _Done:

    def result(self, timeout=None):
        return None


class _Prefetch:
    __slots__ = ("inputs", "future", "cm", "voxel_feats", "event", "error")

    def __init__(self, inputs):
        self.inputs, self.future, self.cm, self.voxel_feats, self.event, self.error = inputs, None, None, None, None, None


PREFETCH_MODE = 3


class InputPrefetcher:

    def __init__(self, detector, make):
        self.detector, self.make, self.ahead = detector, make, None

    def next(self):
        cur = self.ahead if self.ahead is not None else self.make()
        self.ahead = None
        if PREFETCH_MODE:
            self.detector.prefetch_at = {1: "cluster", 2: "start", 3: "bfs", 4: "scorenet", 5: "caption"}[PREFETCH_MODE]
            self.ahead = self.make()
            self.detector.prefetch(self.ahead[0] if isinstance(self.ahead, (list, tuple)) else self.ahead)
        return cur


PREFETCH_TIMEOUT_S = 120
PREFETCH_PADCAST = 1
SELECT_WITH_OFFSETS = 1
EARLY_POINT_GRADS = 1
PHASES = None


def _mark(name):
    if PHASES is not None:
        ev = torch.cuda.Event(enable_timing=True)
        ev.record()
        PHASES.append((name, ev))


class _PointLossGraft(torch.autograd.Function):

    @staticmethod
    def forward(ctx, value, n, *rest):
        ctx.n = n
        ctx.save_for_backward(*rest[:n])
        return value.clone()

    @staticmethod
    def backward(ctx, go):
        grads = ctx.saved_tensors
        return (None, None) + (None,) * ctx.n + tuple(g * go for g in grads)


class PointGroup(nn.Module):
    def __init__(self, cfg):
        super().__init__()
        self.cfg = cfg
        self.task = cfg.general.task
        in_channel = cfg.model.use_color * 3 + cfg.model.use_normal * 3 + cfg.model.use_coords * 3 + \
            cfg.model.use_multiview * 128
        m = cfg.model.m
        D = 3
        classes = cfg.data.classes
        block = common.ResidualBlock if cfg.model.block_residual else common.VGGBlock

        self.requires_gt_mask = cfg.data.requires_gt_mask
        self.cluster_radius = cfg.cluster.cluster_radius
        self.cluster_meanActive = cfg.cluster.cluster_meanActive
        self.cluster_shift_meanActive = cfg.cluster.cluster_shift_meanActive
        self.cluster_npoint_thre = cfg.cluster.cluster_npoint_thre
        self.freeze_backbone = cfg.cluster.freeze_backbone
        self.score_scale = cfg.train.score_scale
        self.score_fullscale = cfg.train.score_fullscale
        self.mode = cfg.train.score_mode
        self.compact_proposals = True
        self.prepare_epochs = cfg.cluster.prepare_epochs
        self.current_epoch = 0

        sp_norm = functools.partial(ME.MinkowskiBatchNorm, eps=1e-4, momentum=0.1)
        norm = functools.partial(nn.BatchNorm1d, eps=1e-4, momentum=0.1)

        self.backbone = nn.Sequential(
            ME.MinkowskiConvolution(in_channel, m, kernel_size=3, bias=False, dimension=D),
            common.UBlock([m * c for c in cfg.model.blocks], sp_norm, cfg.model.block_reps, block),
            sp_norm(m),
            ME.MinkowskiReLU(inplace=True))
        self.sem_seg = nn.Linear(m, classes)
        self.offset_net = nn.Sequential(nn.Linear(m, m), norm(m), nn.ReLU(inplace=True), nn.Linear(m, 3))
        self.score_net = nn.Sequential(
            common.UBlock([m * c for c in cfg.model.cluster_blocks], sp_norm, 2, block),
            sp_norm(m),
            ME.MinkowskiReLU(inplace=True))
        if cfg.model.pred_bbox:
            raise NotImplementedError("pred_bbox=True is not on the hot path (conf/pointgroup.yaml: pred_bbox False)")
        self.score_linear = nn.Linear(m, 1)
        ME.fuse_bn_relu(self)

        self.teacher = False
        self.concurrent_clustering = True
        self.padded_list_budget = None
        self._mem_total = {}
        self._streams = {}
        self.native_unet = True
        self.native_exact = True
        self.__dict__["_execs"] = {}
        self.__dict__["_pf_pending"] = None
        self.__dict__["_pf_live"] = [None, None]
        self.__dict__["_pf_inflight"] = None
        self.prefetch_at = "bfs"
        self.early_point_grads = True

    def _padded_list_budget(self, device):
        if self.padded_list_budget is not None:
            return int(self.padded_list_budget)
        key = device.index
        if key not in self._mem_total:
            self._mem_total[key] = int(torch.cuda.get_device_properties(device).total_memory)
        return int(0.35 * self._mem_total[key])

    def _side_stream(self, device):
        key = (device.index, threading.get_ident())
        if key not in self._streams:
            self._streams[key] = torch.cuda.Stream(device=device)
        return self._streams[key]

    def _exec(self, name, exact=False):
        key = name + "/f32" if exact else name
        ex = self._execs.get(key)
        if ex is None:
            if name == "backbone":
                in_channel = self.backbone[0].in_channels
                ex = netexec.NativeUNet(self.backbone[0], self.backbone[1], self.backbone[2], in_channel, False, exact=exact)
            else:
                ex = netexec.NativeUNet(None, self.score_net[0], self.score_net[1], self.cfg.model.m, True, exact=exact)
            self._execs[key] = ex
        return ex

    def _begin_maps(self, name, voxel_locs):
        if not (self.native_unet and voxel_locs.is_cuda and voxel_locs.size(0) > 0) or (ME._EXACT and (ME._EXACT_FMA or not self.native_exact)):
            return None
        cm = ME.CoordinateManager(voxel_locs.int().contiguous())
        exact = ME.exact_for(self.training, name)
        if exact:
            cm.want16 = False
        cm.begin_pyramid(self._exec(name, exact=exact).nlevels)
        return cm

    def release_eval_executors(self):
        if ME._EXACT:
            return
        for key in [k for k in self._execs if k.endswith("/f32")]:
            del self._execs[key]

    def _input_stage(self, data_dict):
        f = data_dict["feats"]
        cm = self._begin_maps("backbone", data_dict["voxel_locs"])
        if self.cfg.model.use_coords and f.is_cuda and f.dtype == torch.float32 and not f.requires_grad:
            vf = pointgroup_ops.voxelization_cat(f, data_dict["locs"], data_dict["v2p_map"], self.cfg.data.mode)
        else:
            if self.cfg.model.use_coords:
                f = torch.cat((f, data_dict["locs"]), 1)
                data_dict["feats"] = f
            vf = pointgroup_ops.voxelization(f.contiguous(), data_dict["v2p_map"], self.cfg.data.mode)
        return cm, vf

    def prefetch(self, data_dict):
        v = data_dict.get("voxel_locs")
        f = data_dict.get("feats")
        if not (torch.is_tensor(v) and v.is_cuda and self.native_unet and v.size(0) > 0) or "_prefetch" in data_dict:
            return data_dict
        if not (self.cfg.model.use_coords and torch.is_tensor(f) and f.dtype == torch.float32 and not f.requires_grad):
            return data_dict
        t = _Prefetch({k: data_dict[k] for k in ("feats", "locs", "v2p_map", "voxel_locs")})
        data_dict["_prefetch"] = t
        self._pf_pending = t
        if self.prefetch_at == "start":
            self._kick_prefetch()
        return data_dict

    def _kick_prefetch(self, at=None):
        t = self._pf_pending
        if t is None or t.future is not None or (at is not None and at != self.prefetch_at):
            return
        self._pf_pending = None
        dev = t.inputs["voxel_locs"].device
        cur = torch.cuda.current_stream(dev)
        gate = torch.cuda.Event()
        gate.record(cur)
        training = self.training
        def work():
            try:
                with torch.cuda.device(dev):
                    key = (dev.index, threading.get_ident())
                    if key not in self._streams:
                        self._streams[key] = torch.cuda.Stream(device=dev)
                    side = self._streams[key]
                    with torch.cuda.stream(side):
                        side.wait_event(gate)
                        cm, vf = self._input_stage(t.inputs)
                        if cm is not None:
                            ex = self._exec("backbone", exact=ME.exact_for(training, "backbone"))
                            ex.maps(cm)
                            if PREFETCH_PADCAST:
                                cm.padded_input = ex.pad_input(vf)
                        ev = torch.cuda.Event()
                        ev.record(side)
                    t.cm, t.voxel_feats, t.event = cm, vf, ev
            except BaseException as e:
                t.error = e
        t.future = _prefetch_worker().submit(work)
        self._pf_inflight = t.future

    def _take_prefetch(self, t, data_dict):
        if self._pf_pending is t:
            self._pf_pending = None
        same = t.inputs is not None and all(t.inputs.get(k) is data_dict.get(k) for k in ("feats", "locs", "v2p_map", "voxel_locs"))
        if t.future is None:
            t.inputs = None
            return None
        try:
            t.future.result(timeout=PREFETCH_TIMEOUT_S)
        except Exception as e:
            raise RuntimeError("PointGroup: the input prefetch of this batch did not finish within %d s (helper thread stuck?); "
                               "pointgroup.PREFETCH_MODE = 0 disables the look-ahead" % PREFETCH_TIMEOUT_S) from e
        t.inputs = None
        if t.error is not None:
            raise t.error
        if self._pf_inflight is not None:
            self._pf_inflight.result(timeout=PREFETCH_TIMEOUT_S)
        self._pf_live = [self._pf_live[1], t]
        if not same or t.voxel_feats is None:
            return None
        torch.cuda.current_stream(t.voxel_feats.device).wait_event(t.event)
        return t.cm, t.voxel_feats

    def _run_unet(self, name, module, x):
        if self.native_unet and not (ME._EXACT and (ME._EXACT_FMA or not self.native_exact)) and x.F.size(0) > 0:
            return self._exec(name, exact=ME.exact_for(self.training, name))(x.F, x.coordinate_manager, self.training)
        return module(x).features

    def static_gradient_buckets(self):
        out = []
        dev = self.score_linear.weight.device
        for name in ("score_net", "backbone"):
            ex = self._exec(name, exact=ME._EXACT)
            ex._param_ptrs()
            ex._grads(dev)
            out.append((ex._flat_grad, ex.owned_params(), ex))
        return out

    def drop_stale_grads(self):
        for ex in self._execs.values():
            if ex is not None:
                ex.drop_stale_grads()

    def zero_grad(self, set_to_none=True):
        native = set()
        for ex in self._execs.values():
            if ex is not None and ex._grad_views is not None and set_to_none:
                ex.fresh_grads = True
                native.update(id(p) for p, v in zip(ex.b.params, ex._grad_views) if v is not None and p.grad is v)
        key = (len(native), set_to_none)
        cache = self.__dict__.get("_zg_cache")
        if cache is None or cache[0] != key:
            cache = (key, [p for p in self.parameters() if id(p) not in native])
            self.__dict__["_zg_cache"] = cache
        for p in cache[1]:
            if p.grad is None:
                continue
            if set_to_none:
                p.grad = None
            else:
                p.grad.detach_(); p.grad.zero_()

    @staticmethod
    def get_batch_offsets(batch_idxs, batch_size):
        ids = _const(("arange_i32", batch_size), batch_idxs.device, lambda: torch.arange(batch_size, dtype=torch.int32))
        counts = (batch_idxs.view(-1, 1) == ids.view(1, -1)).sum(0)
        offsets = torch.zeros(batch_size + 1, dtype=torch.int32, device=batch_idxs.device)
        offsets[1:] = torch.cumsum(counts, 0).int()
        return offsets

    def clusters_voxelization(self, clusters_idx, clusters_offset, feats, coords, fullscale, scale, mode, rand=None):
        dev = feats.device
        c_idxs = clusters_idx[:, 1].long()
        clusters_feats = heads.gather_cluster_rows(feats, c_idxs)
        _mark("cv_gather")
        clusters_coords_mean, raw_min, raw_max = pointgroup_ops.cluster_coords_stats(coords, clusters_idx, clusters_offset)
        _mark("cv_sec_mean")
        _mark("cv_sec_minmax")
        if rand is None:
            r0, r1 = torch.rand(3), torch.rand(3)
        else:
            r0, r1 = rand[0].cpu(), rand[1].cpu()
        clusters_size, clusters_center, clusters_scale, offset = pointgroup_ops.cluster_norm_params(
            clusters_coords_mean, raw_min, raw_max, fullscale, scale, r0.float(), r1.float())
        clusters_coords = pointgroup_ops.cluster_transform(coords, clusters_idx, clusters_coords_mean, clusters_scale, offset)
        n_clusters = int(clusters_offset.numel() - 1)
        _mark("cv_elementwise")
        voxel_coords, p2v_map, v2p_map = pointgroup_ops.voxelization_idx(clusters_coords, n_clusters, mode)
        _mark("cv_voxelization_idx")
        cm = self._begin_maps("score_net", voxel_coords)
        voxel_feats = pointgroup_ops.voxelization(clusters_feats, v2p_map, mode)
        voxel_feats = ME.SparseTensor(features=voxel_feats, coordinates=None if cm is not None else voxel_coords.int(), coordinate_manager=cm)
        voxel_feats.v2p_map = v2p_map
        return voxel_feats, p2v_map, (clusters_center, clusters_size)

    def get_object_assignments(self, data_dict):
        pc1, pc2 = data_dict["proposal_center_batched"], data_dict["center_label"]
        dist = (pc1.unsqueeze(2) - pc2.unsqueeze(1)).abs().sum(-1)
        data_dict["object_assignment"] = dist.min(2)[1]
        return data_dict

    @staticmethod
    def _box_corners(center, size):
        c = center.double(); s = size.double()
        sgn = _const("corner_signs", c.device, lambda: torch.tensor(
            [[1, 1, -1, -1, 1, 1, -1, -1], [1, -1, -1, 1, 1, -1, -1, 1], [1, 1, 1, 1, -1, -1, -1, -1]], dtype=torch.float64))
        corners = torch.stack([s[:, 0:1] / 2 * sgn[0], s[:, 1:2] / 2 * sgn[1], s[:, 2:3] / 2 * sgn[2]], -1)
        return corners + c.unsqueeze(1)

    def convert_stack_to_batch(self, data_dict, perms=None):
        batch_size = len(data_dict["batch_offsets"]) - 1
        K = self.cfg.model.max_num_proposal
        lazy = data_dict.pop("_stb_inputs", None)
        if lazy is not None:
            pf, scores_in, crop, bids_in = lazy
        else:
            pf, scores_in, crop, bids_in = (data_dict["proposal_feats"], data_dict["proposal_objectness_scores"],
                                            data_dict["proposal_crop_bbox"], data_dict["proposals_batchId"])
        dev = pf.device
        keys = ("proposal_feats_batched", "proposal_bbox_batched", "proposal_center_batched", "proposal_sem_cls_batched",
                "proposal_scores_batched", "proposal_batch_mask")
        perm = data_dict.pop("_slot_perm_staged", None) if perms is None else None
        if perm is None:
            perm = torch.stack([torch.randperm(K) if perms is None else perms[b].cpu() for b in range(batch_size)])
            perm = _STAGE.put(perm, dev)
        want_assign = self.cfg.general.task != "test"
        fused = heads.stack_to_batch(pf, scores_in, crop.detach(), bids_in,
                                     perm, data_dict["center_label"] if want_assign else None, batch_size, K)
        if fused is None and lazy is not None:
            raise RuntimeError("compact_proposals=False needs the fused stack_to_batch (shapes outside its limits)")
        if fused is not None:
            data_dict.update(zip(keys, fused[:6]))
            if want_assign:
                data_dict["object_assignment"] = fused[6]
            return data_dict
        corners = self._box_corners(crop[:, :3].detach(), crop[:, 3:6].detach()).to(pf.dtype)
        out = {
            "proposal_feats_batched": pf.new_zeros(batch_size, K, self.cfg.model.m),
            "proposal_bbox_batched": pf.new_zeros(batch_size, K, 8, 3),
            "proposal_center_batched": pf.new_zeros(batch_size, K, 3),
            "proposal_sem_cls_batched": pf.new_zeros(batch_size, K),
            "proposal_scores_batched": pf.new_zeros(batch_size, K),
            "proposal_batch_mask": pf.new_zeros(batch_size, K),
        }
        bids = data_dict["proposals_batchId"].long()
        inv = torch.empty_like(perm).scatter_(1, perm, _const(("arange", K), dev, lambda: torch.arange(K)).expand(batch_size, K))
        onehot = torch.nn.functional.one_hot(bids, batch_size)
        rank = (onehot.cumsum(0) - onehot).gather(1, bids.view(-1, 1)).squeeze(1)
        ok = rank < K
        slot = bids * K + inv.view(-1)[bids * K + rank.clamp(max=K - 1)]
        slot = torch.where(ok, slot, torch.full_like(slot, batch_size * K))
        rows = {
            "proposal_feats_batched": pf, "proposal_bbox_batched": corners,
            "proposal_center_batched": crop[:, :3], "proposal_sem_cls_batched": crop[:, 7],
            "proposal_scores_batched": data_dict["proposal_objectness_scores"],
            "proposal_batch_mask": pf.new_ones(pf.size(0)),
        }
        for k, v in rows.items():
            flat = out[k].new_zeros((batch_size * K + 1,) + tuple(out[k].shape[2:]))
            flat.index_copy_(0, slot, v.to(flat.dtype))
            out[k] = flat[:-1].view(out[k].shape)
        data_dict.update(out)
        if self.cfg.general.task != "test":
            data_dict = self.get_object_assignments(data_dict)
        return data_dict

    def forward(self, data_dict):
        batch_size = len(data_dict["batch_offsets"]) - 1
        cm = data_dict.pop("_backbone_cm", None)
        x = ME.SparseTensor(features=data_dict["voxel_feats"], coordinates=None if cm is not None else data_dict["voxel_locs"].int(),
                            coordinate_manager=cm)
        _mark("voxelize")
        out_feats = self._run_unet("backbone", self.backbone, x)
        _mark("backbone_fwd")
        pt_feats = heads.devoxelize(out_feats, data_dict["p2v_map"], data_dict.get("v2p_map"))

        semantic_scores, semantic_preds, pt_offsets = heads.point_heads(self.sem_seg, self.offset_net, pt_feats)
        data_dict["semantic_scores"] = semantic_scores
        data_dict["pt_offsets"] = pt_offsets
        data_dict["_pt_feats"] = pt_feats

        _mark("heads")
        if data_dict["epoch"] > self.prepare_epochs or self.freeze_backbone:
            if self.teacher:
                semantic_preds = data_dict["sem_labels"].clamp(min=0)
                cluster_offsets = (data_dict["instance_info"][:, 0:3] - data_dict["locs"]).detach()
                cluster_offsets = torch.where((data_dict["instance_ids"] >= 0).unsqueeze(1), cluster_offsets,
                                              torch.zeros_like(cluster_offsets))
            else:
                cluster_offsets = pt_offsets
            batch_idxs = data_dict["locs_scaled"][:, 0].int()
            if not self.requires_gt_mask:
                object_idxs = torch.nonzero(semantic_preds > 0, as_tuple=False).view(-1)
                if SELECT_WITH_OFFSETS:
                    batch_idxs_, coords_, shifted_xyz, semantic_preds_, batch_offsets_ = pointgroup_ops.cluster_select(
                        data_dict["locs"], cluster_offsets.detach(), semantic_preds, batch_idxs, object_idxs, batch_size=batch_size)
                else:
                    batch_idxs_, coords_, shifted_xyz, semantic_preds_ = pointgroup_ops.cluster_select(
                        data_dict["locs"], cluster_offsets.detach(), semantic_preds, batch_idxs, object_idxs)
                    batch_offsets_ = self.get_batch_offsets(batch_idxs_, batch_size)

                budget = self._padded_list_budget(coords_.device)
                padded_ok = pointgroup_ops.ballquery_padded_fits(coords_.shape[0]) and \
                    pointgroup_ops.padded_clustering_bytes(coords_.shape[0], 2) <= budget

                def cluster_branch(xyz, mean_active, marks=False):
                    padded = pointgroup_ops.ballquery_batch_p_padded(xyz, batch_idxs_, batch_offsets_, self.cluster_radius) if padded_ok else None
                    idx_, start_len_ = padded if padded is not None else pointgroup_ops.ballquery_batch_p(
                        xyz, batch_idxs_, batch_offsets_, self.cluster_radius, mean_active)
                    if marks:
                        _mark("cl_ballquery")
                    p_idx, p_off = pointgroup_ops.bfs_cluster(semantic_preds_, idx_, start_len_, self.cluster_npoint_thre, True)
                    if marks:
                        _mark("cl_bfs")
                    return p_idx, p_off

                _mark("cl_prepare")
                self._kick_prefetch("cluster")
                cur = torch.cuda.current_stream()
                if self.concurrent_clustering and padded_ok:
                    side = self._side_stream(coords_.device)
                    side.wait_stream(cur)

                    def begin(xyz, mean_active, tag):
                        padded = pointgroup_ops.ballquery_batch_p_padded(xyz, batch_idxs_, batch_offsets_, self.cluster_radius, ws_tag=tag)
                        return pointgroup_ops.bfs_cluster_begin(semantic_preds_, padded[0], padded[1], self.cluster_npoint_thre, True, ws_tag=tag)
                    hs = hm = None
                    try:
                        with torch.cuda.stream(side):
                            hs = begin(shifted_xyz, self.cluster_shift_meanActive, "s")
                        hm = begin(coords_, self.cluster_meanActive, "m")
                        _mark("cl_ballquery")
                        self._kick_prefetch("bfs")
                        self._early_point_losses(data_dict)
                        h, hm = hm, None
                        first = pointgroup_ops.bfs_cluster_end(h)
                        _mark("cl_bfs")
                        with torch.cuda.stream(side):
                            h, hs = hs, None
                            shifted = pointgroup_ops.bfs_cluster_end(h)
                    finally:
                        for h in (hm, hs):
                            if h is not None:
                                try:
                                    pointgroup_ops.bfs_cluster_end(h)
                                except Exception:
                                    pass
                        cur.wait_stream(side)
                    for t in shifted:
                        t.record_stream(cur)
                elif self.concurrent_clustering:
                    side = self._side_stream(coords_.device)
                    side.wait_stream(cur)

                    def work():
                        with torch.cuda.device(coords_.device), torch.cuda.stream(side):
                            return cluster_branch(shifted_xyz, self.cluster_shift_meanActive)
                    fut = _cluster_worker().submit(work)
                    try:
                        first = cluster_branch(coords_, self.cluster_meanActive, True)
                        self._kick_prefetch("bfs")
                        self._early_point_losses(data_dict)
                    finally:
                        shifted = fut.result()
                    cur.wait_stream(side)
                    for t in shifted:
                        t.record_stream(cur)
                else:
                    shifted = cluster_branch(shifted_xyz, self.cluster_shift_meanActive)
                    first = cluster_branch(coords_, self.cluster_meanActive)
                proposals_idx, proposals_offset, proposals_batchId_all = pointgroup_ops.cluster_merge(
                    first[0], first[1], shifted[0], shifted[1], object_idxs, batch_idxs)
            else:
                proposals_idx = data_dict["gt_proposals_idx"].to(pt_feats.device)
                proposals_offset = data_dict["gt_proposals_offset"].to(pt_feats.device)
                proposals_batchId_all = batch_idxs[proposals_idx[:, 1].long()].int()

            _mark("clustering")
            num_proposals = proposals_offset.shape[0] - 1
            data_dict["num_raw_proposals"] = num_proposals
            if num_proposals == 0:
                return self._no_proposals(data_dict, pt_feats)

            proposals_voxel_feats, proposals_p2v_map, (proposals_center, proposals_size) = self.clusters_voxelization(
                proposals_idx, proposals_offset, pt_feats, data_dict["locs"], self.score_fullscale, self.score_scale,
                self.mode, rand=data_dict.get("cluster_rand"))

            _mark("cluster_voxelization")
            score_feats = self._run_unet("score_net", self.score_net, proposals_voxel_feats)
            _mark("score_net_fwd")
            self._kick_prefetch("scorenet")
            self._early_point_losses(data_dict)
            if "slot_perms" not in data_dict:
                K = self.cfg.model.max_num_proposal
                data_dict["_slot_perm_staged"] = _STAGE.put(torch.stack([torch.randperm(K) for _ in range(batch_size)]), pt_feats.device)
            pt_score_feats = heads.devoxelize(score_feats, proposals_p2v_map, getattr(proposals_voxel_feats, "v2p_map", None))
            proposals_score_feats = pointgroup_ops.roipool(pt_score_feats, proposals_offset)
            scores = nativelinear.linear(proposals_score_feats, self.score_linear.weight, self.score_linear.bias)
            data_dict["proposal_scores"] = (scores, proposals_idx, proposals_offset)

            _mark("pr_roipool_score")
            sig = torch.sigmoid(scores.view(-1))
            fused = (self.cfg.model.crop_bbox and sig.is_cuda and proposals_offset.dtype == torch.int32 and proposals_idx.dtype == torch.int32
                     and proposals_batchId_all.dtype == torch.int32 and semantic_preds.dtype == torch.int64
                     and proposals_idx.is_contiguous() and semantic_preds.is_contiguous())
            if fused:
                proposals_npoint, thres_mask, bid_start, crop = pointgroup_ops.proposal_prepare(
                    sig.detach(), proposals_offset.contiguous(), proposals_batchId_all.contiguous(), proposals_idx, semantic_preds,
                    proposals_center, proposals_size, self.cfg.test.TEST_SCORE_THRESH, self.cfg.test.TEST_NPOINT_THRESH)
            else:
                proposals_npoint = (proposals_offset[1:] - proposals_offset[:-1]).float()
                thres_mask = torch.logical_and(sig > self.cfg.test.TEST_SCORE_THRESH,
                                               proposals_npoint > self.cfg.test.TEST_NPOINT_THRESH)
                starts = proposals_offset[:-1].long().clamp(max=max(proposals_batchId_all.numel() - 1, 0))
                bid_start = proposals_batchId_all[starts]
            data_dict["proposals_npoint"] = proposals_npoint
            data_dict["proposal_thres_mask"] = thres_mask
            _mark("pr_mask")
            if (not self.compact_proposals and fused and num_proposals <= 4096 and proposals_score_feats.dtype == torch.float32
                    and batch_size * self.cfg.model.max_num_proposal <= 8192):
                bids_masked = torch.where(thres_mask, bid_start, torch.full_like(bid_start, -1))
                data_dict["_stb_inputs"] = (proposals_score_feats, sig, crop, bids_masked)
                for m_ in ("pr_nonzero", "pr_index", "pr_select"):
                    _mark(m_)
                return data_dict
            keep = torch.nonzero(thres_mask).squeeze(1)
            _mark("pr_nonzero")
            proposals_batchId = bid_start.index_select(0, keep)
            data_dict["proposals_batchId"] = proposals_batchId
            data_dict["proposal_feats"] = proposals_score_feats.index_select(0, keep)
            data_dict["proposal_objectness_scores"] = sig.index_select(0, keep)

            _mark("pr_index")
            if self.cfg.model.crop_bbox:
                if not fused:
                    crop = scores.new_zeros(num_proposals, 9)
                    crop[:, :3] = proposals_center
                    crop[:, 3:6] = proposals_size
                    crop[:, 7] = semantic_preds[proposals_idx[proposals_offset[:-1].long(), 1].long()].to(crop.dtype)
                    crop[:, 8] = sig
                data_dict["proposal_crop_bbox"] = crop.index_select(0, keep)
            _mark("pr_select")
        return data_dict

    def _no_proposals(self, data_dict, pt_feats):
        dev = pt_feats.device
        m = self.cfg.model.m
        z = lambda *s: torch.zeros(*s, device=dev)
        data_dict["proposal_scores"] = (z(0, 1), torch.zeros((0, 2), dtype=torch.int32, device=dev),
                                        torch.zeros(1, dtype=torch.int32, device=dev))
        data_dict["proposals_npoint"] = z(0)
        data_dict["proposal_thres_mask"] = torch.zeros(0, dtype=torch.bool, device=dev)
        data_dict["proposals_batchId"] = torch.zeros(0, dtype=torch.int32, device=dev)
        data_dict["proposal_feats"] = z(0, m)
        data_dict["proposal_objectness_scores"] = z(0)
        data_dict["proposal_crop_bbox"] = z(0, 9)
        return data_dict

    def _point_losses(self, semantic_scores, semantic_labels, pt_offsets, coords, instance_info, instance_ids):
        semantic_loss = heads.cross_entropy(semantic_scores, semantic_labels, ignore_index=self.cfg.data.ignore_label)
        offset_norm_loss, offset_dir_loss, n_valid = heads.offset_losses(pt_offsets, coords, instance_info, instance_ids,
                                                                         self.cfg.data.ignore_label)
        return semantic_loss, offset_norm_loss, offset_dir_loss, n_valid

    def _early_point_losses(self, data_dict):
        if self.mode == "test" or not torch.is_grad_enabled():
            return
        need = ("sem_labels", "locs", "instance_info", "instance_ids")
        if any(k not in data_dict for k in need) or not torch.is_tensor(data_dict["semantic_scores"]):
            return
        if "_point_losses" in data_dict:
            return
        args = (data_dict["semantic_scores"], data_dict["sem_labels"], data_dict["pt_offsets"], data_dict["locs"],
                data_dict["instance_info"], data_dict["instance_ids"])
        losses = self._point_losses(*args)
        graft = None
        pf = data_dict.pop("_pt_feats", None)
        if EARLY_POINT_GRADS and self.early_point_grads and pf is not None and all(torch.is_tensor(l) and l.requires_grad for l in losses[:3]):
            w = self.cfg.train.loss_weight
            value = w[0] * losses[0] + w[1] * losses[1] + w[2] * losses[2]
            wrt = [t for t in [pf] + list(self.sem_seg.parameters()) + list(self.offset_net.parameters()) if t.requires_grad]
            grads = torch.autograd.grad(value, wrt, allow_unused=True)
            keep = [(t, g) for t, g in zip(wrt, grads) if g is not None]
            if keep:
                graft = _PointLossGraft.apply(value.detach(), len(keep), *[g for _, g in keep], *[t for t, _ in keep])
                losses = tuple(l.detach() for l in losses[:3]) + tuple(losses[3:])
        data_dict["_point_losses"] = (args, losses, graft)

    def loss(self, data_dict, epoch):
        semantic_scores, semantic_labels = data_dict["semantic_scores"]
        pt_offsets, coords, instance_info, instance_ids = data_dict["pt_offsets"]
        args = (semantic_scores, semantic_labels, pt_offsets, coords, instance_info, instance_ids)
        early = data_dict.pop("_point_losses", None)
        graft = None
        if early is not None and len(early[0]) == len(args) and all(a is b for a, b in zip(early[0], args)):
            semantic_loss, offset_norm_loss, offset_dir_loss, n_valid = early[1]
            graft = early[2] if len(early) > 2 else None
        else:
            if early is not None and len(early) > 2 and early[2] is not None:
                raise RuntimeError("PointGroup.loss: the point losses were computed (and back-propagated) inside forward() for other tensors "
                                   "than the ones passed to loss(); set early_point_grads = False to recompute them here")
            semantic_loss, offset_norm_loss, offset_dir_loss, n_valid = self._point_losses(*args)
        data_dict["semantic_loss"] = (semantic_loss, semantic_scores.shape[0])
        data_dict["offset_norm_loss"] = (offset_norm_loss, n_valid)
        data_dict["offset_dir_loss"] = (offset_dir_loss, n_valid)

        w = self.cfg.train.loss_weight
        loss = graft if graft is not None else w[0] * semantic_loss + w[1] * offset_norm_loss + w[2] * offset_dir_loss
        if epoch > self.cfg.cluster.prepare_epochs:
            scores, proposals_idx, proposals_offset, instance_pointnum = data_dict["proposal_scores"]
            if scores.shape[0] > 0:
                ious = pointgroup_ops.get_iou(proposals_idx[:, 1].contiguous(), proposals_offset, instance_ids,
                                              instance_pointnum)
                score_loss, gt_ious = heads.score_loss(scores, ious, self.cfg.train.fg_thresh, self.cfg.train.bg_thresh)
            else:
                gt_ious = scores.new_zeros(0)
                score_loss = scores.sum() * 0
            data_dict["score_loss"] = (score_loss, gt_ious.shape[0])
            loss = loss + w[3] * score_loss
        data_dict["total_loss"] = (loss, semantic_labels.shape[0])
        return data_dict

    def feed(self, data_dict, epoch=0):
        data_dict["epoch"] = epoch
        t = data_dict.pop("_prefetch", None)
        got = self._take_prefetch(t, data_dict) if t is not None else None
        if got is None:
            got = self._input_stage(data_dict)
        cm, data_dict["voxel_feats"] = got
        if cm is not None:
            data_dict["_backbone_cm"] = cm
        data_dict = self.forward(data_dict)
        if data_dict["epoch"] > self.prepare_epochs or self.freeze_backbone:
            data_dict = self.convert_stack_to_batch(data_dict, perms=data_dict.get("slot_perms"))
        return data_dict

    def parse_feed_ret(self, data_dict, epoch=0):
        semantic_scores = data_dict["semantic_scores"]
        pt_offsets = data_dict["pt_offsets"]
        preds = {"semantic": semantic_scores, "pt_offsets": pt_offsets}
        if self.mode != "test":
            data_dict["semantic_scores"] = (semantic_scores, data_dict["sem_labels"])
            data_dict["pt_offsets"] = (pt_offsets, data_dict["locs"], data_dict["instance_info"], data_dict["instance_ids"])
        if epoch > self.cfg.cluster.prepare_epochs:
            scores, proposals_idx, proposals_offset = data_dict["proposal_scores"]
            preds["score"] = scores
            preds["proposals"] = (proposals_idx, proposals_offset)
            preds["proposal_crop_bboxes"] = data_dict.get("proposal_crop_bbox")
            if self.mode != "test":
                data_dict["proposal_scores"] = (scores, proposals_idx, proposals_offset, data_dict["instance_num_point"])
                if self.cfg.model.crop_bbox and "proposal_crop_bbox" in data_dict:
                    data_dict["proposal_crop_bboxes"] = data_dict["proposal_crop_bbox"]
        return preds, data_dict

    @torch.no_grad()
    def predict_instances(self, data_dict):
        import ctypes as C
        from . import _lib
        data_dict = self.feed(data_dict, self.current_epoch)
        scores, proposals_idx, proposals_offset = data_dict["proposal_scores"][:3]
        sem_pred = data_dict["semantic_scores"].max(1)[1]
        dev = scores.device
        P, N = proposals_offset.numel() - 1, sem_pred.numel()
        empty = dict(pick=torch.zeros(0, dtype=torch.long, device=dev), scores=scores.new_zeros(0), proposals_idx=proposals_idx,
                     proposals_offset=proposals_offset, semantic_pred=sem_pred)
        if P == 0:
            return empty
        sig = torch.sigmoid(scores.view(-1)).contiguous()
        keep = data_dict["proposal_thres_mask"].to(torch.uint8).contiguous()
        ious = torch.empty((P, P), dtype=torch.float32, device=dev)
        member = torch.empty(2 * N, dtype=torch.int32, device=dev)
        flags = torch.zeros(2, dtype=torch.int32, device=dev)
        order = torch.empty(P, dtype=torch.int32, device=dev)
        picked = torch.empty(P, dtype=torch.int32, device=dev)
        L = _lib.lib()
        cidx, off = proposals_idx.contiguous(), proposals_offset.contiguous()
        p_, st = (lambda t: C.c_void_p(t.data_ptr())), C.c_void_p(torch.cuda.current_stream().cuda_stream)
        with torch.cuda.device(dev):
            _lib.check(L.d3_instance_cross_iou(p_(cidx), p_(off), cidx.shape[0], P, N, p_(ious), p_(member), p_(flags), st), "instance_cross_iou")
            _lib.check(L.d3_nms_matrix(p_(ious), p_(sig), p_(keep), P, float(self.cfg.test.TEST_NMS_THRESH), p_(order), p_(picked),
                                       p_(flags[1:]), st), "nms_matrix")
        over, n = flags.tolist()
        if over:
            raise _lib.D3Error("predict_instances: a point belongs to more than two proposals")
        pick = picked[:n].long()
        empty.update(pick=pick, scores=sig[pick], cross_ious=ious)
        return empty

    def evaluate_segmentation(self, batches, evaluator=None):
        from .seg_eval import SegmentationEvaluator
        ev = evaluator if evaluator is not None else SegmentationEvaluator()
        was_training = self.training
        self.eval()
        try:
            for batch in batches:
                gt = {k: batch[k] for k in ("sem_labels", "instance_ids", "batch_offsets", "instance_offsets") if k in batch}
                ev.add_batch(self.predict_instances(batch), gt)
        finally:
            self.train(was_training)
        return ev.instance_results()[0], ev.semantic_results()[0]

    def evaluate_detection(self, batches, evaluator=None):
        from .evaluator import DetectionEvaluator
        ev = evaluator if evaluator is not None else DetectionEvaluator()
        was_training = self.training
        self.eval()
        try:
            with torch.no_grad():
                for batch in batches:
                    ev.add_batch(self.feed(batch, self.current_epoch))
        finally:
            self.train(was_training)
        return ev.compute_metrics()

    def training_step(self, data_dict, idx=0):
        _mark("begin")
        data_dict = self.feed(data_dict, self.current_epoch)
        _mark("proposals")
        _, data_dict = self.parse_feed_ret(data_dict, self.current_epoch)
        data_dict = self.loss(data_dict, self.current_epoch)
        _mark("loss")
        return data_dict["total_loss"][0], data_dict
```

d3net_amd/pointgroup_ops.py:

```python
import ctypes as C
import threading

import torch
from torch.autograd import Function

from . import _lib
from ._lib import check

_ws_cache = {}


_RAW_STREAM = getattr(torch._C, "_cuda_getCurrentRawStream", None)
_RAW_DEVICE = getattr(torch._C, "_cuda_getDevice", None)


def _stream():
    if _RAW_STREAM is not None and _RAW_DEVICE is not None:
        return C.c_void_p(_RAW_STREAM(_RAW_DEVICE()))
    return C.c_void_p(torch.cuda.current_stream().cuda_stream)


def _ptr(t):
    return C.c_void_p(t.data_ptr())


def _workspace(nbytes, device, tag):
    key = (device.index if device.index is not None else torch.cuda.current_device(), tag, threading.get_ident(),
           (_stream().value or 0) if device.type == "cuda" else 0)
    buf = _ws_cache.get(key)
    if buf is None or buf.numel() < nbytes:
        buf = torch.empty(int(nbytes * 1.25) + 1024, dtype=torch.uint8, device=device)
        _ws_cache[key] = buf
    return buf


class _NoGuard:
    def __enter__(self):
        return self

    def __exit__(self, *a):
        return False


_NOGUARD = _NoGuard()


def _on(device):
    if device.index is None:
        return _NOGUARD
    cur = _RAW_DEVICE() if _RAW_DEVICE is not None else torch.cuda.current_device()
    return _NOGUARD if device.index == cur else torch.cuda.device(device)


def _device_of(*tensors):
    for t in tensors:
        if t.is_cuda:
            return t.device
    if not torch.cuda.is_available():
        raise _lib.D3Error("d3net_amd.pointgroup_ops needs a GPU (no CPU fallback)")
    return torch.device("cuda", torch.cuda.current_device())


class Voxelization_Idx(Function):
    @staticmethod
    def forward(ctx, coords, batchsize, mode=4):
        assert coords.is_contiguous()
        assert coords.dtype == torch.int64
        on_cpu = not coords.is_cuda
        dev = _device_of(coords)
        c = coords.to(dev) if on_cpu else coords
        N, ncols = c.shape
        L = _lib.lib()
        with _on(dev):
            input_map = torch.empty(N, dtype=torch.int32, device=dev)
            ws = _workspace(L.d3_voxelize_idx_ws_bytes(N), dev, "vi")
            M, mA = C.c_int(0), C.c_int(1)
            check(L.d3_voxelize_idx_count(_ptr(c), N, ncols, int(mode), _ptr(input_map), _ptr(ws), ws.numel(),
                                          C.byref(M), C.byref(mA), _stream()), "voxelize_idx_count")
            M, mA = M.value, mA.value
            output_coords = torch.empty((M, ncols), dtype=torch.int64, device=dev)
            output_map = torch.empty((M, mA + 1), dtype=torch.int32, device=dev)
            check(L.d3_voxelize_idx_fill(_ptr(c), N, ncols, int(mode), _ptr(input_map), _ptr(ws), ws.numel(),
                                         _ptr(output_coords), _ptr(output_map), M, mA, _stream()),
                  "voxelize_idx_fill")
        if on_cpu:
            return output_coords.cpu(), input_map.cpu(), output_map.cpu()
        return output_coords, input_map, output_map

    @staticmethod
    def backward(ctx, a=None, b=None, c=None):
        return None


voxelization_idx = Voxelization_Idx.apply


class Voxelization(Function):
    @staticmethod
    def forward(ctx, feats, map_rule, mode=4):
        assert map_rule.is_contiguous() and map_rule.is_cuda and map_rule.dtype == torch.int32
        assert feats.is_contiguous() and feats.is_cuda and feats.dtype == torch.float32
        N, Cc = feats.size()
        M = map_rule.size(0)
        maxActive = map_rule.size(1) - 1
        output_feats = torch.zeros((M, Cc), dtype=torch.float32, device=feats.device)
        ctx.for_backwards = (map_rule, mode, maxActive, N)
        with _on(feats.device):
            check(_lib.lib().d3_voxelize_fp(_ptr(feats), _ptr(output_feats), _ptr(map_rule), int(mode), M, maxActive,
                                            Cc, _stream()), "voxelize_fp")
        return output_feats

    @staticmethod
    def backward(ctx, d_output_feats):
        map_rule, mode, maxActive, N = ctx.for_backwards
        M, Cc = d_output_feats.size()
        d_output_feats = d_output_feats.contiguous()
        d_feats = torch.zeros((N, Cc), dtype=torch.float32, device=d_output_feats.device)
        with _on(d_feats.device):
            check(_lib.lib().d3_voxelize_bp(_ptr(d_output_feats), _ptr(d_feats), _ptr(map_rule), int(mode), M,
                                            maxActive, Cc, _stream()), "voxelize_bp")
        return d_feats, None, None


voxelization = Voxelization.apply


class PointRecover(Function):
    @staticmethod
    def forward(ctx, feats, map_rule, nPoint):
        assert map_rule.is_contiguous() and map_rule.is_cuda
        assert feats.is_contiguous() and feats.is_cuda
        M, Cc = feats.size()
        maxActive = map_rule.size(1) - 1
        output_feats = torch.zeros((nPoint, Cc), dtype=torch.float32, device=feats.device)
        ctx.for_backwards = (map_rule, maxActive, M)
        with _on(feats.device):
            check(_lib.lib().d3_point_recover_fp(_ptr(feats), _ptr(output_feats), _ptr(map_rule), M, maxActive, Cc,
                                                 _stream()), "point_recover_fp")
        return output_feats

    @staticmethod
    def backward(ctx, d_output_feats):
        map_rule, maxActive, M = ctx.for_backwards
        N, Cc = d_output_feats.size()
        d_output_feats = d_output_feats.contiguous()
        d_feats = torch.zeros((M, Cc), dtype=torch.float32, device=d_output_feats.device)
        with _on(d_feats.device):
            check(_lib.lib().d3_point_recover_bp(_ptr(d_output_feats), _ptr(d_feats), _ptr(map_rule), M, maxActive,
                                                 Cc, _stream()), "point_recover_bp")
        return d_feats, None, None


point_recover = PointRecover.apply


class BallQueryBatchP(Function):
    @staticmethod
    def forward(ctx, coords, batch_idxs, batch_offsets, radius, meanActive):
        n = coords.size(0)
        assert coords.is_contiguous() and coords.is_cuda and coords.dtype == torch.float32
        assert batch_idxs.is_contiguous() and batch_idxs.is_cuda and batch_idxs.dtype == torch.int32
        assert batch_offsets.is_contiguous() and batch_offsets.is_cuda and batch_offsets.dtype == torch.int32
        dev = coords.device
        L = _lib.lib()
        with _on(dev):
            start_len = torch.empty((n, 2), dtype=torch.int32, device=dev)
            big = L.d3_ballquery_ws_bytes_single_pass(n)
            ws = _workspace(big if big <= (2 << 30) else L.d3_ballquery_ws_bytes(n), dev, "bq")
            nActive = C.c_int(0)
            check(L.d3_ballquery_count(_ptr(coords), _ptr(batch_idxs), _ptr(batch_offsets), n, float(radius),
                                       _ptr(start_len), _ptr(ws), ws.numel(), C.byref(nActive), _stream()),
                  "ballquery_count")
            nActive = nActive.value
            idx = torch.empty(max(nActive, 1), dtype=torch.int32, device=dev)
            check(L.d3_ballquery_fill(_ptr(coords), _ptr(batch_idxs), _ptr(batch_offsets), n, float(radius),
                                      _ptr(start_len), _ptr(ws), ws.numel(), _ptr(idx), nActive, _stream()),
                  "ballquery_fill")
        return idx[:nActive], start_len

    @staticmethod
    def backward(ctx, a=None, b=None):
        return None, None, None


ballquery_batch_p = BallQueryBatchP.apply


def ballquery_padded_fits(n, max_bytes=None):
    cap = _lib.lib().d3_ballquery_cap()
    return n > 0 and n * cap <= 0x7FFFFFFF and (max_bytes is None or n * cap * 4 <= max_bytes)


def padded_clustering_bytes(n, branches=2):
    return int(branches) * int(n) * _lib.lib().d3_ballquery_cap() * 20


def ballquery_batch_p_padded(coords, batch_idxs, batch_offsets, radius, max_bytes=None, ws_tag=""):
    n = coords.size(0)
    L = _lib.lib()
    cap = L.d3_ballquery_cap()
    if not ballquery_padded_fits(n, max_bytes):
        return None
    assert coords.is_contiguous() and coords.is_cuda and coords.dtype == torch.float32
    assert batch_idxs.is_contiguous() and batch_idxs.is_cuda and batch_idxs.dtype == torch.int32
    assert batch_offsets.is_contiguous() and batch_offsets.is_cuda and batch_offsets.dtype == torch.int32
    dev = coords.device
    with _on(dev):
        start_len = torch.empty((n, 2), dtype=torch.int32, device=dev)
        idx = torch.empty(n * cap, dtype=torch.int32, device=dev)
        ws = _workspace(L.d3_ballquery_ws_bytes(n), dev, "bqp" + ws_tag)
        check(L.d3_ballquery_padded(_ptr(coords), _ptr(batch_idxs), _ptr(batch_offsets), n, float(radius), _ptr(start_len),
                                    _ptr(ws), ws.numel(), _ptr(idx), _stream()), "ballquery_padded")
    return idx, start_len


def _cluster_args(sem, idx, sl, threshold, ascending, ws_tag):
    N = sl.size(0)
    assert sem.is_contiguous() and sem.dtype == torch.int32
    assert idx.is_contiguous() and idx.dtype == torch.int32
    assert sl.is_contiguous() and sl.dtype == torch.int32
    dev = sem.device
    if idx.numel() == 0:
        idx = torch.zeros(1, dtype=torch.int32, device=dev)
    L = _lib.lib()
    nact = int(idx.numel())
    ws = _workspace(L.d3_bfs_cluster_ws_bytes(N), dev, "cl" + ws_tag)
    rec = _workspace(L.d3_bfs_cluster_erec_bytes(nact), dev, "clrec" + ws_tag)
    capP, capC = max(N, 1), N // max(int(threshold), 1) + 1
    cluster_idxs = torch.empty((capP, 2), dtype=torch.int32, device=dev)
    cluster_offsets = torch.empty(capC + 1, dtype=torch.int32, device=dev)
    args = (_ptr(sem), _ptr(idx), _ptr(sl), N, int(threshold), _ptr(ws), ws.numel(), _ptr(rec), rec.numel(), nact, 1 if ascending else 0,
            _ptr(cluster_idxs), capP, _ptr(cluster_offsets), capC)
    return args, (sem, idx, sl, ws, rec), cluster_idxs, cluster_offsets


class BFSCluster(Function):
    @staticmethod
    def forward(ctx, semantic_label, ball_query_idxs, start_len, threshold, ascending=False):
        on_cpu = not semantic_label.is_cuda
        dev = _device_of(semantic_label, ball_query_idxs, start_len)
        S, P = C.c_int(0), C.c_int(0)
        with _on(dev):
            args, _keep, cluster_idxs, cluster_offsets = _cluster_args(*(t.to(dev) for t in (semantic_label, ball_query_idxs, start_len)),
                                                                       threshold, ascending, "")
            check(_lib.lib().d3_bfs_cluster_run(*args, C.byref(S), C.byref(P), _stream()), "bfs_cluster_run")
            cluster_idxs, cluster_offsets = cluster_idxs[:S.value], cluster_offsets[:P.value + 1]
            if start_len.size(0) == 0:
                cluster_offsets.zero_()
        if on_cpu:
            return cluster_idxs.cpu(), cluster_offsets.cpu()
        return cluster_idxs, cluster_offsets

    @staticmethod
    def backward(ctx, a=None, b=None):
        return None, None, None, None, None


bfs_cluster = BFSCluster.apply


class _ClusterRun:
    __slots__ = ("ticket", "keep", "cluster_idxs", "cluster_offsets", "N", "dev")


def bfs_cluster_begin(semantic_label, ball_query_idxs, start_len, threshold, ascending=False, ws_tag=""):
    assert semantic_label.is_cuda
    dev = semantic_label.device
    r = _ClusterRun()
    tk = C.c_void_p()
    with _on(dev):
        args, r.keep, r.cluster_idxs, r.cluster_offsets = _cluster_args(semantic_label, ball_query_idxs, start_len, threshold, ascending, ws_tag)
        check(_lib.lib().d3_bfs_cluster_begin(*args, C.byref(tk), _stream()), "bfs_cluster_begin")
    r.ticket, r.N, r.dev = tk, start_len.size(0), dev
    return r


def bfs_cluster_end(r):
    S, P = C.c_int(0), C.c_int(0)
    tk, r.ticket = r.ticket, None
    with _on(r.dev):
        check(_lib.lib().d3_bfs_cluster_end(tk, C.byref(S), C.byref(P)), "bfs_cluster_end")
    ci, co = r.cluster_idxs[:S.value], r.cluster_offsets[:P.value + 1]
    if r.N == 0:
        co.zero_()
    r.keep = None
    return ci, co


class RoiPool(Function):
    @staticmethod
    def forward(ctx, feats, proposals_offset):
        nProposal = proposals_offset.size(0) - 1
        sumNPoint, Cc = feats.size()
        assert feats.is_contiguous() and feats.is_cuda and feats.dtype == torch.float32
        assert proposals_offset.is_contiguous() and proposals_offset.is_cuda and proposals_offset.dtype == torch.int32
        output_feats = torch.empty((nProposal, Cc), dtype=torch.float32, device=feats.device)
        output_maxidx = torch.empty((nProposal, Cc), dtype=torch.int32, device=feats.device)
        with _on(feats.device):
            check(_lib.lib().d3_roipool_fp(_ptr(feats), _ptr(proposals_offset), _ptr(output_feats),
                                           _ptr(output_maxidx), nProposal, Cc, _stream()), "roipool_fp")
        ctx.for_backwards = (output_maxidx, proposals_offset, sumNPoint)
        return output_feats

    @staticmethod
    def backward(ctx, d_output_feats):
        nProposal, Cc = d_output_feats.size()
        output_maxidx, proposals_offset, sumNPoint = ctx.for_backwards
        d_output_feats = d_output_feats.contiguous()
        d_feats = torch.zeros((sumNPoint, Cc), dtype=torch.float32, device=d_output_feats.device)
        with _on(d_feats.device):
            check(_lib.lib().d3_roipool_bp(_ptr(d_feats), _ptr(proposals_offset), _ptr(output_maxidx),
                                           _ptr(d_output_feats), nProposal, Cc, _stream()), "roipool_bp")
        return d_feats, None


roipool = RoiPool.apply


class GetIoU(Function):
    @staticmethod
    def forward(ctx, proposals_idx, proposals_offset, instance_labels, instance_pointnum):
        nInstance = instance_pointnum.size(0)
        nProposal = proposals_offset.size(0) - 1
        assert proposals_idx.is_contiguous() and proposals_idx.is_cuda and proposals_idx.dtype == torch.int32
        assert proposals_offset.is_contiguous() and proposals_offset.is_cuda and proposals_offset.dtype == torch.int32
        assert instance_labels.is_contiguous() and instance_labels.is_cuda and instance_labels.dtype == torch.int64
        assert instance_pointnum.is_contiguous() and instance_pointnum.is_cuda and instance_pointnum.dtype == torch.int32
        proposals_iou = torch.empty((nProposal, nInstance), dtype=torch.float32, device=proposals_idx.device)
        with _on(proposals_idx.device):
            check(_lib.lib().d3_get_iou(_ptr(proposals_idx), _ptr(proposals_offset), _ptr(instance_labels),
                                        _ptr(instance_pointnum), _ptr(proposals_iou), nInstance, nProposal,
                                        _stream()), "get_iou")
        return proposals_iou

    @staticmethod
    def backward(ctx, a=None):
        return None, None, None, None


get_iou = GetIoU.apply


def _sec(name, inp, offsets):
    nProposal = offsets.size(0) - 1
    Cc = inp.size(1)
    assert inp.is_contiguous() and inp.is_cuda and inp.dtype == torch.float32
    assert offsets.is_contiguous() and offsets.is_cuda and offsets.dtype == torch.int32
    out = torch.empty((nProposal, Cc), dtype=torch.float32, device=inp.device)
    with _on(inp.device):
        check(getattr(_lib.lib(), name)(_ptr(inp), _ptr(offsets), _ptr(out), nProposal, Cc, _stream()), name)
    return out


class SecMean(Function):
    @staticmethod
    def forward(ctx, inp, offsets):
        return _sec("d3_sec_mean", inp, offsets)

    @staticmethod
    def backward(ctx, a=None):
        return None, None


sec_mean = SecMean.apply


class SecMin(Function):
    @staticmethod
    def forward(ctx, inp, offsets):
        return _sec("d3_sec_min", inp, offsets)

    @staticmethod
    def backward(ctx, a=None):
        return None, None


sec_min = SecMin.apply


class SecMax(Function):
    @staticmethod
    def forward(ctx, inp, offsets):
        return _sec("d3_sec_max", inp, offsets)

    @staticmethod
    def backward(ctx, a=None):
        return None, None


sec_max = SecMax.apply


def voxelization_cat(feats_a, feats_b, map_rule, mode=4):
    assert map_rule.is_contiguous() and map_rule.is_cuda and map_rule.dtype == torch.int32
    assert feats_a.is_cuda and feats_a.dtype == torch.float32 and feats_b.dtype == torch.float32 and feats_a.size(0) == feats_b.size(0)
    assert not feats_a.requires_grad and not feats_b.requires_grad
    feats_a, feats_b = feats_a.contiguous(), feats_b.contiguous()
    M, maxActive = map_rule.size(0), map_rule.size(1) - 1
    out = torch.empty((M, feats_a.size(1) + feats_b.size(1)), dtype=torch.float32, device=feats_a.device)
    with _on(feats_a.device):
        check(_lib.lib().d3_voxelize_fp2(_ptr(feats_a), feats_a.size(1), _ptr(feats_b), feats_b.size(1), _ptr(out), _ptr(map_rule),
                                         int(mode), M, maxActive, _stream()), "voxelize_fp2")
    return out


def cluster_select(locs, pt_offsets, semantic_preds, batch_idxs, object_idxs, batch_size=None):
    locs, pt_offsets = locs.contiguous(), pt_offsets.contiguous()
    assert locs.dtype == torch.float32 and pt_offsets.dtype == torch.float32 and semantic_preds.dtype == torch.int64
    assert batch_idxs.dtype == torch.int32 and object_idxs.dtype == torch.int64
    n, dev = object_idxs.numel(), locs.device
    b = torch.empty(n, dtype=torch.int32, device=dev)
    sem = torch.empty(n, dtype=torch.int32, device=dev)
    xyz = torch.empty((2, n, 3), dtype=torch.float32, device=dev)
    if batch_size is not None and n > 0:
        boff = torch.empty(int(batch_size) + 1, dtype=torch.int32, device=dev)
        with _on(dev):
            check(_lib.lib().d3_cluster_select2(_ptr(locs), _ptr(pt_offsets), _ptr(semantic_preds.contiguous()), _ptr(batch_idxs.contiguous()),
                                                _ptr(object_idxs.contiguous()), n, int(batch_size), _ptr(b), _ptr(xyz[0]), _ptr(xyz[1]), _ptr(sem),
                                                _ptr(boff), _stream()), "cluster_select2")
        return b, xyz[0], xyz[1], sem, boff
    with _on(dev):
        check(_lib.lib().d3_cluster_select(_ptr(locs), _ptr(pt_offsets), _ptr(semantic_preds.contiguous()), _ptr(batch_idxs.contiguous()),
                                           _ptr(object_idxs.contiguous()), n, _ptr(b), _ptr(xyz[0]), _ptr(xyz[1]), _ptr(sem), _stream()),
              "cluster_select")
    if batch_size is not None:
        return b, xyz[0], xyz[1], sem, torch.zeros(int(batch_size) + 1, dtype=torch.int32, device=dev)
    return b, xyz[0], xyz[1], sem


def cluster_merge(idx1, off1, idx2, off2, object_idxs, batch_idxs):
    S1, S2, P1, P2 = idx1.shape[0], idx2.shape[0], off1.numel() - 1, off2.numel() - 1
    dev = idx1.device
    out_idx = torch.empty((S1 + S2, 2), dtype=torch.int32, device=dev)
    out_off = torch.empty(P1 + P2 + 1, dtype=torch.int32, device=dev)
    out_bid = torch.empty(max(S1 + S2 - 1, 0) if S2 > 0 else S1, dtype=torch.int32, device=dev)
    with _on(dev):
        check(_lib.lib().d3_cluster_merge(_ptr(idx1.contiguous()), S1, _ptr(off1.contiguous()), P1, _ptr(idx2.contiguous()), S2,
                                          _ptr(off2.contiguous()), P2, _ptr(object_idxs), _ptr(batch_idxs), _ptr(out_idx), _ptr(out_off),
                                          _ptr(out_bid), _stream()), "cluster_merge")
    return out_idx, out_off, out_bid


def cluster_coords_stats(coords, clusters_idx, clusters_offset):
    assert coords.is_cuda and coords.dtype == torch.float32 and coords.is_contiguous() and coords.shape[1] == 3
    assert clusters_idx.dtype == torch.int32 and clusters_idx.is_contiguous() and clusters_offset.dtype == torch.int32
    P = clusters_offset.numel() - 1
    out = torch.empty((3, P, 3), dtype=torch.float32, device=coords.device)
    L = _lib.lib()
    S = int(clusters_idx.shape[0])
    with _on(coords.device):
        ws = _workspace(L.d3_cluster_coords_stats_ws_bytes(S), coords.device, "ccs")
        check(L.d3_cluster_coords_stats2(_ptr(coords), _ptr(clusters_idx), _ptr(clusters_offset.contiguous()), S, _ptr(out[0]), _ptr(out[1]),
                                         _ptr(out[2]), P, _ptr(ws), ws.numel(), _stream()), "cluster_coords_stats2")
    return out[0], out[1], out[2]


def proposal_prepare(sig, proposals_offset, batch_id_all, proposals_idx, semantic_preds, center, size, score_thr, npoint_thr):
    P = proposals_offset.numel() - 1
    dev = sig.device
    npoint = torch.empty(P, dtype=torch.float32, device=dev)
    mask = torch.empty(P, dtype=torch.bool, device=dev)
    bid = torch.empty(P, dtype=torch.int32, device=dev)
    crop = torch.empty((P, 9), dtype=torch.float32, device=dev)
    with _on(dev):
        check(_lib.lib().d3_proposal_prepare(_ptr(sig.contiguous()), _ptr(proposals_offset), _ptr(batch_id_all), batch_id_all.numel(),
                                             _ptr(proposals_idx), _ptr(semantic_preds), _ptr(center.contiguous()), _ptr(size.contiguous()),
                                             float(score_thr), float(npoint_thr), P, _ptr(npoint), _ptr(mask), _ptr(bid), _ptr(crop),
                                             _stream()), "proposal_prepare")
    return npoint, mask, bid, crop


def cluster_norm_params(mean, raw_min, raw_max, fullscale, scale_cap, r0, r1):
    P = mean.shape[0]
    dev = mean.device
    mean, raw_min, raw_max = mean.contiguous(), raw_min.contiguous(), raw_max.contiguous()
    size = torch.empty((P, 3), dtype=torch.float32, device=dev)
    center, offset = torch.empty_like(size), torch.empty_like(size)
    cscale = torch.empty((P,), dtype=torch.float32, device=dev)
    rand6 = (C.c_float * 6)(*[float(v) for v in r0.tolist()], *[float(v) for v in r1.tolist()])
    with _on(dev):
        check(_lib.lib().d3_cluster_norm_params(_ptr(mean), _ptr(raw_min), _ptr(raw_max), P, float(fullscale), float(scale_cap),
                                                C.cast(rand6, C.c_void_p), _ptr(size), _ptr(center), _ptr(cscale),
                                                _ptr(offset), _stream()), "cluster_norm_params")
    return size, center, cscale, offset


def cluster_transform(coords, clusters_idx, mean, scale, offset):
    S = clusters_idx.shape[0]
    mean, scale, offset = mean.contiguous(), scale.contiguous(), offset.contiguous()
    out = torch.empty((S, 4), dtype=torch.int64, device=coords.device)
    with _on(coords.device):
        check(_lib.lib().d3_cluster_transform(_ptr(coords), _ptr(clusters_idx), _ptr(mean), _ptr(scale), _ptr(offset), _ptr(out), S,
                                              _stream()), "cluster_transform")
    return out
```

include/d3hip.h:

```cpp
#ifndef D3HIP_H
#define D3HIP_H
#include <stddef.h>
#include <stdint.h>

#ifdef __cplusplus
extern "C" {
#endif

#define D3_ERR_WORKSPACE (-1)
#define D3_ERR_RANGE     (-2)
#define D3_ERR_ARG       (-3)
#define D3_ERR_OVERFLOW  (-4)

int d3_version(void);
const char *d3_arch(void);

int d3_sec_mean(const float *inp, const int *offsets, float *out, int nProposal, int C, void *stream);
int d3_sec_min(const float *inp, const int *offsets, float *out, int nProposal, int C, void *stream);
int d3_sec_max(const float *inp, const int *offsets, float *out, int nProposal, int C, void *stream);
int d3_cluster_select(const float *locs, const float *pt_offsets, const int64_t *semantic_preds, const int *batch_idxs,
                      const int64_t *object_idxs, int n, int *batch_out, float *coords_out, float *shifted_out, int *semantic_out,
                      void *stream);
int d3_cluster_select2(const float *locs, const float *pt_offsets, const int64_t *semantic_preds, const int *batch_idxs,
                       const int64_t *object_idxs, int n, int batch_size, int *batch_out, float *coords_out, float *shifted_out,
                       int *semantic_out, int *batch_offsets_out, void *stream);
int d3_cluster_merge(const int *idx1, int S1, const int *off1, int P1, const int *idx2, int S2, const int *off2, int P2,
                     const int64_t *object_idxs, const int *batch_idxs, int *out_idx, int *out_off, int *out_bid, void *stream);
int d3_proposal_prepare(const float *sig, const int *offsets, const int *batch_id_all, int n_batch_id, const int *proposals_idx,
                        const int64_t *semantic_preds, const float *center, const float *size, float score_thr, float npoint_thr,
                        int P, float *npoint, unsigned char *mask, int *batch_id, float *crop, void *stream);
int d3_cluster_coords_stats(const float *coords, const int *clusters_idx, const int *offsets, float *mean, float *cmin, float *cmax,
                            int nProposal, void *stream);
size_t d3_cluster_coords_stats_ws_bytes(long long S);
int d3_cluster_coords_stats2(const float *coords, const int *clusters_idx, const int *offsets, long long S, float *mean, float *cmin,
                             float *cmax, int nProposal, void *ws, size_t ws_bytes, void *stream);
int d3_cluster_transform(const float *coords, const int *clusters_idx, const float *mean, const float *scale, const float *offset,
                         long long *out, long long S, void *stream);
int d3_cluster_norm_params(const float *mean, const float *raw_min, const float *raw_max, int P, float fullscale, float scale_cap,
                           const float *rand6, float *size, float *center, float *cscale, float *offset, void *stream);
int d3_roipool_fp(const float *feats, const int *proposals_offset, float *output_feats, int *output_maxidx,
                  int nProposal, int C, void *stream);
int d3_roipool_bp(float *d_feats, const int *proposals_offset, const int *output_maxidx,
                  const float *d_output_feats, int nProposal, int C, void *stream);
int d3_get_iou(const int *proposals_idx, const int *proposals_offset, const int64_t *instance_labels,
               const int *instance_pointnum, float *proposals_iou, int nInstance, int nProposal, void *stream);

int d3_voxelize_fp(const float *feats, float *output_feats, const int *output_map, int mode, int nActive,
                   int maxActive, int nPlane, void *stream);
int d3_voxelize_fp2(const float *feats_a, int Ca, const float *feats_b, int Cb, float *output_feats, const int *output_map, int mode,
                    int nActive, int maxActive, void *stream);
int d3_voxelize_bp(const float *d_output_feats, float *d_feats, const int *output_map, int mode, int nActive,
                   int maxActive, int nPlane, void *stream);
int d3_point_recover_fp(const float *feats, float *output_feats, const int *idx_map, int nActive,
                        int maxActive, int nPlane, void *stream);
int d3_point_recover_bp(const float *d_output_feats, float *d_feats, const int *idx_map, int nActive,
                        int maxActive, int nPlane, void *stream);

size_t d3_voxelize_idx_ws_bytes(int n);
int d3_voxelize_idx_count(const int64_t *coords, int n, int ncols, int mode, int *input_map, void *ws,
                          size_t ws_bytes, int *M_host, int *maxActive_host, void *stream);
int d3_voxelize_idx_fill(const int64_t *coords, int n, int ncols, int mode, const int *input_map, void *ws,
                         size_t ws_bytes, int64_t *output_coords, int *output_map, int M, int maxActive,
                         void *stream);

size_t d3_ballquery_ws_bytes(int n);
size_t d3_ballquery_ws_bytes_single_pass(int n);
int d3_ballquery_count(const float *xyz, const int *batch_idxs, const int *batch_offsets, int n, float radius,
                       int *start_len, void *ws, size_t ws_bytes, int *nActive_host, void *stream);
int d3_ballquery_fill(const float *xyz, const int *batch_idxs, const int *batch_offsets, int n, float radius,
                      const int *start_len, const void *ws, size_t ws_bytes, int *idx, long long idx_capacity,
                      void *stream);
int d3_ballquery_cap(void);
int d3_ballquery_padded(const float *xyz, const int *batch_idxs, const int *batch_offsets, int n, float radius,
                        int *start_len, void *ws, size_t ws_bytes, int *idx_padded, void *stream);

#define D3_BFS_ASCENDING 1
size_t d3_bfs_cluster_ws_bytes(int n);
size_t d3_bfs_cluster_erec_bytes(long long nActive);
int d3_bfs_cluster_begin(const int *semantic_label, const int *ball_query_idxs, const int *start_len, int n, int threshold,
                         void *ws, size_t ws_bytes, void *erec, size_t erec_bytes, long long nActive, int flags,
                         int *cluster_idxs, long long cap_points, int *cluster_offsets, long long cap_clusters,
                         void **ticket, void *stream);
int d3_bfs_cluster_end(void *ticket, int *sumNPoint_host, int *nCluster_host);
int d3_bfs_cluster_run(const int *semantic_label, const int *ball_query_idxs, const int *start_len, int n, int threshold,
                       void *ws, size_t ws_bytes, void *erec, size_t erec_bytes, long long nActive, int flags,
                       int *cluster_idxs, long long cap_points, int *cluster_offsets, long long cap_clusters,
                       int *sumNPoint_host, int *nCluster_host, void *stream);

size_t d3_coordmap_ws_bytes(int M);
int d3_kmap_k3(const int *coords, int M, int ts, void *ws, size_t ws_bytes, int *nbr, void *stream);
int d3_kmap_k3_pack16(const int *nbr, int M, void *nbr16, int *ok16, void *stream);
int d3_kmap_k3_16(const int *coords, int M, int ts, void *ws, size_t ws_bytes, int *nbr, void *nbr16, int *ok16, void *stream);
size_t d3_kmap_k3_q16_bytes(int M);
int d3_kmap_k3_packq(const int *nbr, int M, void *tq, int *okq, void *stream);
int d3_kmap_down_count(const int *coords, int M, int ts, void *ws, size_t ws_bytes, int *parent, int *kidx,
                       int *Mout_host, void *stream);
int d3_kmap_down_fill(const int *coords, int M, int ts, void *ws, size_t ws_bytes, const int *parent,
                      const int *kidx, int *out_coords, int *child, int *up, int Mout, void *stream);

int d3_kmap_pyramid(const int *coords0, int M0, int nlevels, void *ws, size_t ws_bytes, int *coords_out, int *parent,
                    int *kidx, int *flag, int *rows_dev, int *rows_host, void *stream);
int d3_kmap_pyramid_begin(const int *coords0, int M0, int nlevels, void *ws, size_t ws_bytes, int *coords_out, int *parent,
                          int *kidx, int *flag, int *rows_dev, void **ticket, void *stream);
int d3_kmap_pyramid_end(void *ticket, int *rows_host, int nlevels);
int d3_kmap_down_fill2(int M, int Mout, const int *parent, const int *kidx, int *child, int *up, void *stream);

#define D3_CONV_FLIPK 1
#define D3_CONV_TRANSW 2
#define D3_CONV_EXACT 4
#define D3_CONV_XSTAT 8
#define D3_CONV_ACCUM 16
#define D3_CONV_XBF16 32
#define D3_CONV_DYBF16 64
#define D3_CONV_OUTBF16 512
#define D3_CONV_BNXBF16 1024
#define D3_CONV_F32 256
#define D3_CONV_NOREDUCE 128
int d3_spconv_fwd(const float *x, const int *tbl, const float *W, float *out, int Min, int Mout, int K, int Cin,
                  int Cout, int flags, void *stream);
int d3_spconv_wgrad(const float *x, const int *tbl, const float *dy, float *dW, int Min, int Mout, int K, int Cin,
                    int Cout, int flags, void *stream);

size_t d3_spconv_pack_bytes(int K, int Cin, int Cout);
size_t d3_spconv_pack_bytes_ex(int K, int Cin, int Cout, int flags);
int d3_spconv_pack(const float *W, void *Wp, int K, int Cin, int Cout, int flags, void *stream);
int d3_spconv_fwd2_nparts(int Mout, int K, int Cin, int Cout);
int d3_spconv_fwd2_nparts_ex(int Mout, int K, int Cin, int Cout, int flags);
int d3_spconv_last_nparts(void);
int d3_spconv_fwd2_plan(int Mout, int K, int Cin, int Cout, int *out6);
int d3_spconv_fwd2(const void *x, int ldx, const int *tbl, const void *Wp, float *out, int ldo, const float *res,
                   int ldr, float *part, int Min, int Mout, int K, int Cin, int Cout, int flags, void *stream);
int d3_spconv_fwd2_bnbwd(const void *x, int ldx, const int *tbl, const void *Wp, float *out, int ldo, float *part,
                         const float *bnx, int ldbx, const float *mean, const float *var, const float *gamma,
                         const float *beta, float eps, int relu, int Min, int Mout, int K, int Cin, int Cout, int flags,
                         void *stream);
int d3_spconv_fwd3_nparts(int Mout, int Cin, int Cout);
int d3_spconv_fwd3(const void *x, int ldx, const void *tq, const void *Wp, void *out, int ldo, const float *res, int ldr,
                   float *part, double *part2, int Min, int Mout, int Cin, int Cout, int flags, void *stream);
int d3_spconv_fwd3_bnbwd(const void *x, int ldx, const void *tq, const void *Wp, void *out, int ldo, float *part, double *part2,
                         const void *bnx, int ldbx, const float *mean, const float *var, const float *gamma, const float *beta,
                         float eps, int relu, int Min, int Mout, int Cin, int Cout, int flags, void *stream);
long long d3_spconv_fwd3_launches(void);
size_t d3_spconv_wgrad2_ws_bytes(int Min, int Mout, int K, int Cin, int Cout, int flags);
int d3_spconv_wgrad2_splits(int Min, int Mout, int K, int Cin, int Cout, int flags);
int d3_spconv_wgrad2(const void *x, int ldx, const int *tbl, const void *dy, int ldy, float *dW, int Min, int Mout,
                     int K, int Cin, int Cout, int CinW, int flags, void *ws, size_t ws_bytes, void *stream);

int d3_prof_enable(int on);
int d3_prof_collect(int family, long long *launches, double *total_ms, double *total_bytes, double *total_flops);
int d3_prof_dump(int family, double *rows, int cap, int *n);

int d3_tuning_set(const char *name, int value);
int d3_tuning_get(const char *name, int *value);
int d3_tuning_count(void);
const char *d3_tuning_name(int i);

size_t d3_bn_ws_bytes(int C);
int d3_bn_stats(const float *x, int M, int C, float *mean, float *var, float *running_mean, float *running_var,
                float momentum, void *ws, size_t ws_bytes, void *stream);
int d3_bn_relu_fwd(const float *x, const float *mean, const float *var, const float *gamma, const float *beta,
                   float *y, int M, int C, float eps, int relu, void *stream);
int d3_bn_relu_fwd_bf16(const float *x, const float *mean, const float *var, const float *gamma, const float *beta,
                        void *y_bf16, int M, int C, float eps, int relu, void *stream);
int d3_bn_relu_bwd(const float *x, const float *dy, const float *mean, const float *var, const float *gamma,
                   const float *beta, float *dx, float *dgamma, float *dbeta, int M, int C, float eps, int relu,
                   void *ws, size_t ws_bytes, void *stream);

void *d3_net_create(const int64_t *prog, int nops, const int64_t *tensors, int ntensors, const int64_t *bufs, int nbufs,
                    int nlevels, int nparams, int input_needs_grad, int out_tensor);
void d3_net_destroy(void *net);
int d3_net_plan(void *net, const int *rows, size_t *arena_bytes, size_t *grad_bytes);
long long d3_net_tensor_offset(void *net, int tensor);
long long d3_net_describe(void *net, int64_t *out, long long cap);
int d3_net_forward(void *net, const void *const *params, const int *const *k3, const int *const *child,
                   const int *const *up, const void *input, void *arena, int training, void *stream);
int d3_net_backward(void *net, const void *const *params, const int *const *k3, const int *const *child,
                    const int *const *up, const void *input, void *arena, void *grad_arena, const float *gout,
                    float *const *pgrads, const int *paccum, float *gin, void *stream);
int d3_net_set_chunks(void *net, const int *op_idx, int nchunks);
int d3_net_set_k3_16(void *net, const void *const *k3_16, const int *const *k3_q);
int d3_net_padded_channels(void *net);
int d3_net_padcast(void *net, const void *input, void *out, long long M, void *stream);
int d3_net_set_padded_input(void *net, const void *xp);
long long d3_spconv_t16_launches(void);
int d3_net_chunk_wait(void *net, int k, void *stream);

size_t d3_tall_wgrad_ws_bytes(int I, int O);
int d3_tall_wgrad(const float *x, const float *dy, float *dW, float *db, int N, int I, int O, void *ws, size_t ws_bytes,
                  void *stream);
size_t d3_offset_loss_ws_bytes(void);
int d3_offset_loss(const float *pt, const float *coords, const float *info, int ldi, const int64_t *ids, long long ignore,
                   float *g1, float *g2, float *out, int N, void *ws, size_t ws_bytes, void *stream);
size_t d3_point_heads_ws_bytes(void);
int d3_point_heads_fwd(const float *x, long long N, int m, int C, const float *Ws, const float *bs, const float *W0, const float *b0,
                       const float *gamma, const float *beta, const float *W3, const float *b3, float eps, float momentum,
                       int training, float *running_mean, float *running_var, long long *num_batches_tracked, float *scores,
                       long long *preds, float *h, float *y, float *offsets, float *stat, void *ws, size_t ws_bytes, void *stream);
int d3_point_heads_dy(const float *g_off, const float *W3, const float *y, long long N, float *dy, void *stream);
int d3_point_heads_dx(const float *dh, const float *W0, const float *g_scores, const float *Ws, long long N, int C, float *dx,
                      void *stream);
int d3_score_loss(const float *scores, const float *ious, int P, int nInst, float fg, float bg, float *gt_iou,
                  float *dscore, float *out, void *stream);
size_t d3_masked_xe_ws_bytes(int N, int S);
int d3_masked_xe(const float *pred, const long long *target, long long ld_target, const unsigned char *good, int N, int S, int V,
                 float *dpred, float *out2, void *ws, size_t ws_bytes, void *stream);
int d3_orientation_loss(const float *preds, long long ld_batch, long long ld_edge, const float *edge_index,
                        const long long *num_src, const long long *num_tar, const long long *assign, const float *rotations,
                        const float *rot_masks, int B, int E, int K, int G, int num_bins, const float *bounds_host,
                        int nbounds, float *dpreds, float *out2, void *stream);
int d3_stack_to_batch(const float *feats, const float *crop, const float *scores, const int *bids, const long long *perm,
                      const float *center_label, int G, int P, int m, int B, int K, float *feats_b, float *bbox_b,
                      float *center_b, float *sem_b, float *scores_b, float *mask_b, long long *slot, long long *assign,
                      void *stream);
int d3_adamw_chunk(void);
int d3_adamw(const long long *ptrs, const int *numel, const void *blocks, int nblocks, double lr, double beta1, double beta2,
             double eps, double weight_decay, double bias_correction1, double bias_correction2_sqrt, void *stream);
int d3_scatter_add_rows(const float *g, const int64_t *idx, float *out, long long S, int C, void *stream);
int d3_gather_rows(const float *feats, const int64_t *idx, float *out, long long S, int C, void *stream);
int d3_gather_rows_pad(const float *feats, long long rows, const int64_t *idx, float *out, long long S, int C, int scatter,
                       void *stream);
size_t d3_cross_entropy_ws_bytes(void);
int d3_cross_entropy(const float *z, const int64_t *label, float *grad, float *out, int N, int C, int ignore_index,
                     void *ws, size_t ws_bytes, void *stream);

int d3_attn_fwd(const float *q, const float *k, const float *v, const float *bias, const float *mask, float *out,
                float *P, int B, int h, int nq, int nk, int dk, int dv, int bias_div, void *stream);
int d3_attn_bwd(const float *q, const float *k, const float *v, const float *P, const float *dout, float *dS,
                float *dq, float *dk, float *dv, int B, int h, int nq, int nk, int dkdim, int dvdim, void *stream);

int d3_layernorm_fwd(const float *a, const float *b, const float *gamma, const float *beta, float *y, float *mean,
                     float *rstd, int R, int D, float eps, void *stream);
size_t d3_layernorm_ws_bytes(int R, int D);
int d3_layernorm_bwd(const float *a, const float *b, const float *gamma, const float *mean, const float *rstd,
                     const float *dy, float *dx, float *dgamma, float *dbeta, int R, int D, void *ws, size_t ws_bytes,
                     void *stream);

typedef struct {
    int B, K, N, div, m, L;
    const float *feats, *lang, *mask;
    const float *W0, *b0, *g1, *be1; float *rm1, *rv1; const float *alpha;
    const float *W3, *b3, *W4, *b4, *g2, *be2; float *rm2, *rv2;
    const float *W5, *b5, *g3, *be3; float *rm3, *rv3; const float *w6, *b6;
    float eps[3], momentum[3];
    long long *nbt[3];
    float *PQ; double *part;
    float *x1, *f, *y2, *z2, *y3, *bnstat;
    float *conf;
} d3_srm_args;
typedef struct {
    const float *dconf;
    float *dW0, *db0, *dg1, *dbe1, *dalpha, *dW3, *db3, *dW4, *db4, *dg2, *dbe2, *dW5, *db5, *dg3, *dbe3, *dw6, *db6;
    float *dfeats, *dlang;
    float *dpre3, *dz2, *dpre2, *df, *dbn1, *dP, *dQ, *db0part; double *part;
    void *ws; size_t ws_bytes;
} d3_srm_grads;
int d3_scanrefer_match_groups(int N, int K);
int d3_scanrefer_match_fwd(const d3_srm_args *a, int train, void *stream);
size_t d3_scanrefer_match_bwd_ws_bytes(void);
int d3_scanrefer_match_bwd(const d3_srm_args *a, const d3_srm_grads *g, int train, void *stream);

typedef struct {
    const float *A; const int *ia; long long lda; int a_kmajor;
    const float *B; long long ldb; int b_kmajor;
    int K;
} d3_gemm_seg;
typedef struct {
    d3_gemm_seg seg[3]; int nseg;
    int M, N;
    float *C; long long ldc;
    const float *bias; const float *add; long long ldadd;
    int relu, accum, perm_nb, perm_s;
    int gru, gru_H;
    const float *g_d0; long long g_ld0; const float *g_d1; long long g_ld1;
    const float *g_r, *g_z, *g_n, *g_ghn, *g_hp; long long g_ldh;
    float *g_dgi; long long g_lddgi; float *g_dgh; float *g_dhp;
} d3_gemm_prob;
int d3_hgemm(const d3_gemm_prob *probs, int nprobs, void *stream);
size_t d3_colsum_ws_bytes(int C);
int d3_colsum(const float *x, long long ld, int R, int C, float *out, int accum, void *ws, size_t ws_bytes, void *stream);

typedef struct {
    int N, K, S, V, H, E, F, Tw;
    const long long *word_ids;
    const float *emb;
    const float *target;
    const float *obj;
    const float *mask;
    const float *W_td, *b_td;
    const float *Wih1, *Whh1, *bih1, *bhh1;
    const float *W_feat, *W_hidd, *w_att;
    const float *W_lang, *b_lang;
    const float *Wih2, *Whh2, *bih2, *bhh2;
    const float *Wc0, *bc0, *Wc2, *bc2;
    float *logits;
    float *attn;
    void *ws; size_t ws_bytes;
} d3_topdown_args;
typedef struct {
    const float *dlogits;
    float *dW_td, *db_td, *dWih1, *dWhh1, *dbih1, *dbhh1, *dW_feat, *dW_hidd, *dw_att, *dW_lang, *db_lang;
    float *dWih2, *dWhh2, *dbih2, *dbhh2, *dWc0, *dbc0, *dWc2, *dbc2;
    float *dobj, *dtarget;
    void *ws; size_t ws_bytes;
} d3_topdown_grads;
size_t d3_topdown_ws_bytes(int N, int K, int S, int H, int E, int F);
size_t d3_topdown_bwd_ws_bytes(int N, int K, int S, int V, int H, int E, int F);
int d3_topdown_xe_forward(const d3_topdown_args *a, void *stream);
int d3_topdown_xe_backward(const d3_topdown_args *a, const d3_topdown_grads *g, void *stream);
int d3_topdown_xe_backward_ex(const d3_topdown_args *a, const d3_topdown_grads *g, void *stream, void *side);
size_t d3_topdown_step_ws_bytes(int N, int K, int H, int E, int F);
int d3_topdown_feat_proj(const float *obj, const float *W_feat, float *fp, int rows, int H, int F, void *stream);
int d3_topdown_step(const d3_topdown_args *a, const long long *word, const float *fp, int obj_div, const float *h1_in,
                    const float *h2_in, float *h1_out, float *h2_out, float *logits, float *attn, void *ws, size_t ws_bytes,
                    void *stream);

int d3_beam_select(const float *logits, const float *sums_in, int N, int live, int b, int V, int eos, int last, int t, int Tmax,
                   const long long *seq_prev, long long *seq_out, long long *tok_out, float *snap_out, unsigned char *ended_out,
                   float *sums_out, const float *h1_in, const float *h2_in, float *h1_out, float *h2_out, int H, void *stream);
int d3_greedy_select(const float *logits, int N, int V, long long *word, float *lp, void *stream);
int d3_topdown_greedy(const d3_topdown_args *a, const float *fp, int obj_div, float *h1_a, float *h2_a, float *h1_b, float *h2_b,
                      float *logits, float *attn, void *ws, size_t ws_bytes, const long long *first_word, int max_len,
                      long long *words, float *lps, void *stream);
int d3_topdown_beam(const d3_topdown_args *a, const float *fp, int b, float *const *h1, float *const *h2, float *logits, float *attn,
                    void *ws, size_t ws_bytes, const long long *first_word, int eos, int max_len, long long *allseq, float *snap_all,
                    unsigned char *ended_all, float *sums0, float *sums1, long long *tok, void *stream);
int d3_topdown_beam_greedy(const d3_topdown_args *a, const float *fp, int b, float *const *h1, float *const *h2, float *logits,
                           float *attn, void *ws, size_t ws_bytes, const long long *first_word, int eos, int max_len,
                           long long *allseq, float *snap_all, unsigned char *ended_all, float *sums0, float *sums1, long long *tok,
                           int glen, long long *g_words, float *g_lps, void *stream);

size_t d3_gru_seq_ws_bytes(int N, int T, int I, int H);
size_t d3_gru_seq_bwd_ws_bytes(int N, int T, int I, int H);
int d3_gru_seq_forward(const float *x, const int *lens, const float *Wih, const float *Whh, const float *bih, const float *bhh, int N,
                       int T, int I, int H, float *hiddens, float *last, void *ws, size_t ws_bytes, void *stream);
int d3_gru_seq_backward(const float *x, const int *lens, const float *Wih, const float *Whh, int N, int T, int I, int H,
                        const float *d_hiddens, const float *d_last, const void *ws, float *dWih, float *dWhh, float *dbih, float *dbhh,
                        float *dx, void *ws2, size_t ws2_bytes, void *stream);

int d3_graph_edges(const float *adj, const float *mask, int B, int K, int L, int *src, int *dst, float *edge_index, int *cnt,
                   int *in_ptr, int *in_list, int *out_start, int *out_cnt, long long *feat_src, long long *pred_src,
                   void *stream);
size_t d3_edgeconv_ws_bytes(int Emax, int Cin, int Cout);
size_t d3_edgeconv_bwd_ws_bytes(int Emax, int Cin, int Cout);
int d3_edgeconv_fwd(const float *x, const float *W0, const float *b0, const float *W2, const float *b2, const int *src,
                    const int *dst, const int *in_ptr, const int *in_list, int B, int K, int L, int Cin, int Cout, float *node,
                    float *msg, void *ws, size_t ws_bytes, void *stream);
int d3_edgeconv_bwd(const float *W0, const float *W2, const int *src, const int *dst, const int *in_ptr, const int *in_list,
                    const int *out_start, const int *out_cnt, int B, int K, int L, int Cin, int Cout, const float *d_node,
                    const float *d_msg, const void *ws, float *dx, float *dW0, float *db0, float *dW2, float *db2, void *ws2,
                    size_t ws2_bytes, void *stream);

int d3_nms3d_samecls(const float *boxes, const float *valid, const int *visit, int B, int K, double iou_thr, int old_type, float *pick,
                     void *stream);
int d3_instance_cross_iou(const int *cluster_idxs, const int *offsets, long long S, int P, int N, float *ious, int *member,
                          int *overflow_dev, void *stream);
int d3_nms_matrix(const float *ious, const float *scores, const unsigned char *keep, int n, float thr, int *order_scratch, int *picked,
                  int *npicked, void *stream);

int d3_seg_eval_max_inst(void);
size_t d3_seg_eval_ws_bytes(int B, int G);
int d3_seg_eval(const int *gt_sem, const int *gt_inst, const int *pred_sem, const int *batch_offsets, int B, int N, int max_scene_points,
                int G, const int *pick, int n_pick, const int *proposals_idx, const int *proposals_offset, int P, long long S,
                unsigned long long inst_class_mask, int *confusion, int *gt_stats, int *pred_stats, int *inter, int *status, void *ws,
                size_t ws_bytes, void *stream);

int d3_lsap_batched(const float *cost, const int *ncols, int B, int R, int C, int *per_col, int *status, void *stream);
int d3_dense_caption_assign(const float *pred_boxes, const float *gt_boxes, const int *nactual, int B, int K, int G, int *per_gt,
                            int *status, float *cost_out, void *stream);

int d3_det_match(const float *pred_corners, const int *pred_cls, const float *scores, const float *pick, double conf_thresh,
                 const float *gt_corners, const float *gt_mask, const int *gt_cls, int B, int K, int G, int num_class,
                 const double *thresholds, int T, int *kept, int *cls_out, float *score_out, double *ovmax, int *jmax, int *tp_bits,
                 int *gt_count, int *status, void *stream);
int d3_det_ap(const int *tp_sorted, const int *seg_offsets, const int *gt_count, int S, long long N, int num_class, int T,
              double *table, void *stream);

int d3_caption_collect(const int *per_gt, const float *pred_boxes, const float *gt_boxes, const int *gt_mask,
                       const long long *gt_obj_ids, const long long *lang_cap, const int *lut, const int *scene_idx,
                       const int *slot_of, const int *assign_status, int B, int K, int G, int T, int V, int n_scenes, int n_obj,
                       int S, int sos, int eos, long long batch_seq, unsigned long long *owner, int *cap, int *cap_len,
                       float *iou, int *scene_seen, int *status, void *stream);
int d3_caption_stats(const int *cand, int ldc, const int *clen, const int *tokens, int ldt, const int *lens,
                     const int *slot_row, const int *u_off, int E, int *stats, int *lcs, void *stream);

int d3_scene_limits(int *max_points, int *max_grid, int *max_id);
int d3_scene_transform(const float *xyz, int n, const double *m_host, double scale, int fp32, double *y, double *s, void *stream);
int d3_scene_reduce(const double *s, const int *ids, int n, unsigned long long *stats, void *stream);
int d3_scene_noise(float *grid, long long count, unsigned long long seed, void *stream);
size_t d3_scene_elastic_ws_bytes(int X, int Y, int Z);
int d3_scene_elastic(double *s, int n, float *grids, const double *axes, int X, int Y, int Z, double mag, void *ws, size_t ws_bytes,
                     void *stream);
int d3_scene_offset(double *s, int n, const unsigned long long *stats, int fp32, void *stream);
int d3_scene_crop_count(const double *s, int n, const double *off_host, const double *range_host, int *flags, int *count,
                        void *stream);
size_t d3_scene_ws_bytes(int n, int max_id);
int d3_scene_emit(const double *y, const double *s, const float *feats, int C, const int *sem, const int *ids, int n,
                  const int *flags, const double *off_host, int fp32, double *y_out, float *locs, float *locs_scaled,
                  float *feats_out, int *sem_out, int *ids_out, void *ws, size_t ws_bytes, void *stream);
int d3_scene_relabel(int *ids, int n, int max_id, void *ws, size_t ws_bytes, void *stream);
int d3_scene_instances(const double *y, const int *ids, const int *sem, int n, int max_id, int fp32, int R, const double *mean_size,
                       float *info, int *num_point, int *gt_idx, int *gt_off, double *boxes, int *counts, void *ws,
                       size_t ws_bytes, void *stream);

size_t d3_lang_features_ws_bytes(int S, int E);
int d3_lang_features(const int *tokens, const int *lens, int Nd, const float *glove, int V, int D, int L, int unk,
                     const int *rows_host, const int *erase_ptr_host, const int *erase_pos_host, int S, float *lang_feat,
                     long long *lang_ids, long long *lang_len, void *ws, size_t ws_bytes, void *stream);
size_t d3_ref_targets_ws_bytes(int B);
int d3_ref_targets(const long long *gt_ids, const long long *gt_label, const float *gt_bbox, const long long *object_id, int B, int C,
                   int R, const int *rot_off, const int *rot_ids, const float *rot_mats, int Ns, const int *scene_host,
                   long long *ref_label, float *ref_corner, float *rots, long long *rot_masks, void *ws, size_t ws_bytes, void *stream);

int d3_multiview_limits(int *max_points, int *max_frames, int *max_pixels);
size_t d3_multiview_project_ws_bytes(int N, int F);
int d3_multiview_project(const float *points, int N, const float *depths, const float *c2w, const float *w2c, int F,
                         const double *intr_host, int W, int H, long long *idx3d, long long *idx2d, void *ws, size_t ws_bytes,
                         void *stream);
int d3_multiview_project_frame(const float *label, int C, int HW, const long long *idx3d, const long long *idx2d, int N, float *out,
                               void *stream);
size_t d3_multiview_fuse_ws_bytes(int F, int W, int H);
int d3_multiview_fuse(const float *points, int N, const float *depths, const float *c2w, const float *w2c, int F,
                      const double *intr_host, int W, int H, const float *feats, int C, int maxpool, float *out, int *frame_counts,
                      void *ws, size_t ws_bytes, void *stream);

int d3_enet_layers(int *table, int cap);
long long d3_enet_param_count(void);
int d3_enet_preprocess(const unsigned char *frames, int F, int H0, int W0, const int *rows, const int *cols, int H, int W, float *out,
                       void *stream);
size_t d3_enet_ws_bytes(int F, int H, int W);
int d3_enet_forward(const float *x, int F, int H, int W, const float *params, long long n_params, const int *table, int n_table,
                    int upto, float *out, void *ws, size_t ws_bytes, void *stream);

int d3_scan_limits(int *max_vertices, int *max_faces, int *max_segments, int *max_objects, int *max_rows);
size_t d3_scan_mesh_ws_bytes(int N, int F);
int d3_scan_mesh(const void *vertex_rec, int N, const void *face_rec, int F, const double *align_host, float *mesh, float *aligned_mesh,
                 int *flags, void *ws, size_t ws_bytes, void *stream);
size_t d3_scan_labels_ws_bytes(int N, int S, int P, int K, int R);
int d3_scan_labels(const unsigned short *raw, const int *seg, int N, int S, const int *pair_seg, const int *pair_obj, int P,
                   const int *obj_id, const int *obj_label_seg, int K, int R, const float *mesh, const float *aligned_mesh,
                   double *instance_ids, double *sem_labels, int *inst_gt, double *boxes, double *aligned_boxes, int *flags, void *ws,
                   size_t ws_bytes, void *stream);

size_t d3_cider_ws_bytes(int SR, int E, int hash_slots);
int d3_cider_scores(const int *tokens, int ldt, const int *lens, const int *slot_row, const int *u_off, const int *mult,
                    const int *ent_u, int U, int SR, const int *cand, int ldc, const int *clen, int E, int eos, double sigma,
                    int hash_slots, double *scores, int *overflow_dev, void *ws, size_t ws_bytes, void *stream);

int d3_query_locals_dist(const float *corners, const float *masks, float *dist, int B, int K, int include_self,
                         float overlay_threshold, int center_mode, void *stream);
int d3_query_locals_mask(const float *dist, float *mask, int rows, int K, int L, void *stream);
int d3_caption_select_target(const float *corners, const float *ref_corners, const float *ref_labels, int N, int per_scene, int K,
                             int G, long long *target_ids, float *target_ious, long long *labels, void *stream);
int d3_caption_inputs_fwd(const float *base, const float *edge, const float *adj, const float *locals, const long long *target_ids,
                          int N, int per_scene, int K, int L, int F, float *obj, float *target_feats, float *valid, int *nbr,
                          void *stream);
int d3_caption_inputs_bwd(const float *g_obj, const float *g_target, const long long *target_ids, const int *nbr, int N, int per_scene,
                          int K, int L, int F, float *d_base, float *d_edge, void *stream);

#ifdef __cplusplus
}
#endif
#endif
```

Measured before the change: 252.6.

## Fuse cluster min/max into mean kernel, gather-voxelize clusters, sort-free voxel rules

Folds the per-cluster coordinate min/max reduction into the pipelined segmented-mean kernel, so the separate init and atomic min/max gather launches go away. Cluster voxelization now reads point features indirectly through clusters_idx inside new gather forward and backward kernels, instead of first materialising a gathered cluster-feature tensor. Voxelization index building for modes 3/4 replaces the radix sort with a scatter plus per-voxel rank-sort list kernel that also writes output coordinates. The costs are more indirect loads, atomics on the original feature rows in backward, and extra register pressure in the mean kernel.

```diff
diff --git a/d3net_amd/_lib.py b/d3net_amd/_lib.py
--- a/d3net_amd/_lib.py
+++ b/d3net_amd/_lib.py
@@ -38,6 +38,8 @@
     "d3_voxelize_fp": (i32, [vp, vp, vp, i32, i32, i32, i32, vp]),
     "d3_voxelize_fp2": (i32, [vp, i32, vp, i32, vp, vp, i32, i32, i32, vp]),
     "d3_voxelize_bp": (i32, [vp, vp, vp, i32, i32, i32, i32, vp]),
+    "d3_voxelize_gather_fp": (i32, [vp, vp, i32, vp, vp, i32, i32, i32, i32, vp]),
+    "d3_voxelize_gather_bp": (i32, [vp, vp, vp, i32, vp, i32, i32, i32, i32, vp]),
     "d3_point_recover_fp": (i32, [vp, vp, vp, i32, i32, i32, vp]),
     "d3_point_recover_bp": (i32, [vp, vp, vp, i32, i32, i32, vp]),
     "d3_voxelize_idx_ws_bytes": (sz, [i32]),
diff --git a/d3net_amd/csrc/seg_ops.hip b/d3net_amd/csrc/seg_ops.hip
--- a/d3net_amd/csrc/seg_ops.hip
+++ b/d3net_amd/csrc/seg_ops.hip
@@ -72,9 +72,10 @@
 #define MEANW_PB 16
 #define MEANW_WAVES(NP) ((NP) <= 3 ? (NP) + 1 : (NP) + 1 + ((NP) - 1) / 3)
 #define MEANW_PROD 3
-template <int NPROD>
+template <int NPROD, bool MINMAX>
 __global__ __launch_bounds__(MEANW_WAVES(NPROD) * 64) void sec_mean_pc_kernel(const float *__restrict__ inp, const int *__restrict__ offsets,
-                                                         float *__restrict__ out, int nProposal, int C, const int *__restrict__ gidx, int prediv) {
+                                                         float *__restrict__ out, int nProposal, int C, const int *__restrict__ gidx,
+                                                         float *__restrict__ cmin, float *__restrict__ cmax) {
     extern __shared__ __attribute__((aligned(16))) float meanw_smem[];
     float (*stage)[NPROD][MEANW_CHUNK] = (float (*)[NPROD][MEANW_CHUNK])meanw_smem;
     constexpr int MEANW_PROD_ = NPROD;
@@ -88,6 +89,7 @@
     const int nround = (nchunk + MEANW_PROD_ - 1) / MEANW_PROD_;
     const unsigned int invC = (65536u + C - 1) / C;
     float mean = 0.f;
+    float lo[3] = {INFINITY, INFINITY, INFINITY}, hi[3] = {-INFINITY, -INFINITY, -INFINITY};
     if (NPROD > 3 && wave == 0) __builtin_amdgcn_s_setprio(3);
     const int pslot = NPROD <= 3 ? wave - 1 : ((wave & 3) ? wave - 1 - (wave >> 2) : -1);
     for (int rd = 0; rd <= nround; rd++) {
@@ -127,7 +129,11 @@
 #pragma unroll
                     for (int j = 0; j < MEANW_PB; j++) {
                         const int f = (hf * MEANW_PB + j) * 64 + lz;
-                        if (f < cf) st[cj[j] * rpc + rowj[j]] = okj[j] ? (prediv ? v[j] : __fdiv_rn(v[j], count)) : 0.f;
+                        if (f < cf) st[cj[j] * rpc + rowj[j]] = okj[j] ? __fdiv_rn(v[j], count) : 0.f;
+                        if (MINMAX) {
+                            if (okj[j] && v[j] < lo[(hf * MEANW_PB + j) % 3]) lo[(hf * MEANW_PB + j) % 3] = v[j];
+                            if (okj[j] && v[j] > hi[(hf * MEANW_PB + j) % 3]) hi[(hf * MEANW_PB + j) % 3] = v[j];
+                        }
                     }
                 }
             }
@@ -173,6 +179,35 @@
         __syncthreads();
     }
     if (wave == 0 && lane < C) out[(long long)p * C + lane] = mean;
+    if (MINMAX) {
+        float *red = meanw_smem;
+        if (pslot >= 0) {
+            const int r = lane % 3;
+            float m[6] = {r == 0 ? lo[0] : (r == 1 ? lo[2] : lo[1]), r == 0 ? lo[1] : (r == 1 ? lo[0] : lo[2]), r == 0 ? lo[2] : (r == 1 ? lo[1] : lo[0]),
+                          r == 0 ? hi[0] : (r == 1 ? hi[2] : hi[1]), r == 0 ? hi[1] : (r == 1 ? hi[0] : hi[2]), r == 0 ? hi[2] : (r == 1 ? hi[1] : hi[0])};
+#pragma unroll
+            for (int o = 32; o > 0; o >>= 1)
+#pragma unroll
+                for (int c = 0; c < 3; c++) {
+                    const float a = __shfl_xor(m[c], o), b = __shfl_xor(m[3 + c], o);
+                    if (a < m[c]) m[c] = a;
+                    if (b > m[3 + c]) m[3 + c] = b;
+                }
+            if (lane == 0)
+#pragma unroll
+                for (int c = 0; c < 6; c++) red[pslot * 6 + c] = m[c];
+        }
+        __syncthreads();
+        if (pslot == 0 && lane < 3) {
+            float a = red[lane], b = red[3 + lane];
+            for (int q = 1; q < NPROD; q++) {
+                if (red[q * 6 + lane] < a) a = red[q * 6 + lane];
+                if (red[q * 6 + 3 + lane] > b) b = red[q * 6 + 3 + lane];
+            }
+            cmin[(long long)p * 3 + lane] = a;
+            cmax[(long long)p * 3 + lane] = b;
+        }
+    }
 }
 
 __global__ __launch_bounds__(SEG_THREADS) void roipool_fp_kernel(const float *__restrict__ feats,
@@ -328,56 +363,6 @@
     }
     if (any) { if (IS_MAX) seg_atomic_max_f32(&out[(long long)p * C + c], v); else seg_atomic_min_f32(&out[(long long)p * C + c], v); }
 }
-__global__ __launch_bounds__(SEG_THREADS) void seg_minmax_gather_kernel(const float *__restrict__ inp, const int *__restrict__ gidx,
-                                                                       const int *__restrict__ offsets, float *__restrict__ omin,
-                                                                       float *__restrict__ omax, int nProposal, int C) {
-    __shared__ float rmin[SEG_THREADS], rmax[SEG_THREADS];
-    const int active = (SEG_THREADS / C) * C, rpp = active / C, t = threadIdx.x;
-    const int c = t % C;
-    const int total = offsets[nProposal], first = offsets[0];
-    int per = (total - first + gridDim.x - 1) / gridDim.x;
-    per = (per + rpp - 1) / rpp * rpp;
-    const int R0 = first + blockIdx.x * per, R1 = min(total, R0 + per);
-    if (R0 >= R1) return;
-    const int p0 = seg_find(offsets, nProposal, R0);
-    if (offsets[p0 + 1] >= R1) {
-        float lo = INFINITY, hi = -INFINITY;
-        if (t < active)
-            for (int r = R0 + t / C; r < R1; r += rpp) {
-                const float x = inp[(long long)gidx[(long long)r * 2 + 1] * C + c];
-                if (x < lo) lo = x;
-                if (x > hi) hi = x;
-            }
-        rmin[t] = lo; rmax[t] = hi;
-        __syncthreads();
-        if (t < C) {
-            float a = rmin[t], b = rmax[t];
-            for (int k = t + C; k < active; k += C) { if (rmin[k] < a) a = rmin[k]; if (rmax[k] > b) b = rmax[k]; }
-            if (a < INFINITY) seg_atomic_min_f32(&omin[(long long)p0 * C + t], a);
-            if (b > -INFINITY) seg_atomic_max_f32(&omax[(long long)p0 * C + t], b);
-        }
-        return;
-    }
-    if (t >= active) return;
-    int r = R0 + t / C;
-    if (r >= R1) return;
-    int p = seg_find(offsets, nProposal, r);
-    int pend = offsets[p + 1];
-    float lo = INFINITY, hi = -INFINITY;
-    bool any = false;
-    for (; r < R1; r += rpp) {
-        if (r >= pend) {
-            if (any) { seg_atomic_min_f32(&omin[(long long)p * C + c], lo); seg_atomic_max_f32(&omax[(long long)p * C + c], hi); }
-            while (r >= pend) { p++; pend = offsets[p + 1]; }
-            lo = INFINITY; hi = -INFINITY; any = false;
-        }
-        const float x = inp[(long long)gidx[(long long)r * 2 + 1] * C + c];
-        if (x < lo) lo = x;
-        if (x > hi) hi = x;
-        any = true;
-    }
-    if (any) { seg_atomic_min_f32(&omin[(long long)p * C + c], lo); seg_atomic_max_f32(&omax[(long long)p * C + c], hi); }
-}
 __global__ void cluster_transform_kernel(const float *__restrict__ coords, const int *__restrict__ cidx, const float *__restrict__ mean,
                                          const float *__restrict__ scale, const float *__restrict__ offset, long long *__restrict__ out,
                                          long long S) {
@@ -498,7 +483,7 @@
     D3_CLEAR();
     if (nProposal <= 0) return 0;
     if (C <= 0 || C > SEG_THREADS) return D3_ERR_ARG;
-    if (C <= 64) sec_mean_pc_kernel<MEANW_PROD><<<nProposal, 256, 2 * MEANW_PROD * MEANW_CHUNK * sizeof(float) + 256, d3_stream(stream)>>>(inp, offsets, out, nProposal, C, nullptr, 0);
+    if (C <= 64) sec_mean_pc_kernel<MEANW_PROD, false><<<nProposal, 256, 2 * MEANW_PROD * MEANW_CHUNK * sizeof(float) + 256, d3_stream(stream)>>>(inp, offsets, out, nProposal, C, nullptr, nullptr, nullptr);
     else sec_mean_kernel<<<seg_grid(nProposal), SEG_THREADS, 0, d3_stream(stream)>>>(inp, offsets, out, nProposal, C);
     D3_LAUNCH_CHECK();
     return 0;
@@ -558,38 +543,29 @@
     return 0;
 }
 
-__global__ void cluster_quot_kernel(const float *__restrict__ coords, const int *__restrict__ clusters_idx, const int *__restrict__ offsets,
-                                    float *__restrict__ q, long long S, int nProposal) {
+__global__ void cluster_gather_kernel(const float *__restrict__ coords, const int *__restrict__ clusters_idx, float *__restrict__ g, long long S) {
     const long long t = (long long)blockIdx.x * blockDim.x + threadIdx.x;
     if (t >= S * 3) return;
     const long long e = t / 3;
     const int ch = (int)(t - e * 3);
-    const int pt = clusters_idx[e * 2 + 1];
-    int lo = 0, hi = nProposal;
-    while (hi - lo > 1) { const int m = (lo + hi) >> 1; if ((long long)offsets[m] <= e) lo = m; else hi = m; }
-    const int c = lo;
-    const float count = (float)(offsets[c + 1] - offsets[c]);
-    q[t] = __fdiv_rn(coords[(long long)pt * 3 + ch], count);
-}
-
-static int cluster_mean_launch(const float *inp, const int *offsets, float *mean, int nProposal, const int *gidx, int prediv, hipStream_t s) {
+    g[t] = coords[(long long)clusters_idx[e * 2 + 1] * 3 + ch];
+}
+
+static int cluster_stats_launch(const float *inp, const int *offsets, float *mean, float *cmin, float *cmax, int nProposal, const int *gidx,
+                                hipStream_t s) {
     constexpr int NP = 6;
     const size_t lds = (size_t)2 * NP * MEANW_CHUNK * sizeof(float) + 256;
-    if (const int rc = d3_allow_lds<sec_mean_pc_kernel<NP>>((int)lds)) return rc;
-    sec_mean_pc_kernel<NP><<<nProposal, MEANW_WAVES(NP) * 64, lds, s>>>(inp, offsets, mean, nProposal, 3, gidx, prediv);
-    return 0;
-}
-
-static int cluster_minmax_launch(const float *coords, const int *clusters_idx, const int *offsets, float *cmin, float *cmax, int nProposal, hipStream_t s);
+    if (const int rc = d3_allow_lds<sec_mean_pc_kernel<NP, true>>((int)lds)) return rc;
+    sec_mean_pc_kernel<NP, true><<<nProposal, MEANW_WAVES(NP) * 64, lds, s>>>(inp, offsets, mean, nProposal, 3, gidx, cmin, cmax);
+    D3_LAUNCH_CHECK();
+    return 0;
+}
 
 extern "C" int d3_cluster_coords_stats(const float *coords, const int *clusters_idx, const int *offsets, float *mean, float *cmin,
                                        float *cmax, int nProposal, void *stream) {
     D3_CLEAR();
     if (nProposal <= 0) return 0;
-    hipStream_t s = d3_stream(stream);
-    int rc = cluster_mean_launch(coords, offsets, mean, nProposal, clusters_idx, 0, s);
-    if (rc) return rc;
-    return cluster_minmax_launch(coords, clusters_idx, offsets, cmin, cmax, nProposal, s);
+    return cluster_stats_launch(coords, offsets, mean, cmin, cmax, nProposal, clusters_idx, d3_stream(stream));
 }
 
 extern "C" size_t d3_cluster_coords_stats_ws_bytes(long long S) { return (size_t)(S > 0 ? S : 1) * 3 * sizeof(float); }
@@ -599,20 +575,9 @@
     if (nProposal <= 0) return 0;
     if (S < 0 || ws == nullptr || ws_bytes < d3_cluster_coords_stats_ws_bytes(S)) return D3_ERR_WORKSPACE;
     hipStream_t s = d3_stream(stream);
-    float *q = (float *)ws;
-    if (S > 0) cluster_quot_kernel<<<(int)((S * 3 + 255) / 256), 256, 0, s>>>(coords, clusters_idx, offsets, q, S, nProposal);
-    int rc = cluster_mean_launch(q, offsets, mean, nProposal, nullptr, 1, s);
-    if (rc) return rc;
-    return cluster_minmax_launch(coords, clusters_idx, offsets, cmin, cmax, nProposal, s);
-}
-
-static int cluster_minmax_launch(const float *coords, const int *clusters_idx, const int *offsets, float *cmin, float *cmax, int nProposal, hipStream_t s) {
-    const long long n = (long long)nProposal * 3;
-    seg_init_kernel<<<(int)((n + 255) / 256), 256, 0, s>>>(cmin, nullptr, n, INFINITY, 0);
-    seg_init_kernel<<<(int)((n + 255) / 256), 256, 0, s>>>(cmax, nullptr, n, -INFINITY, 0);
-    seg_minmax_gather_kernel<<<SEG_FLAT_GRID, SEG_THREADS, 0, s>>>(coords, clusters_idx, offsets, cmin, cmax, nProposal, 3);
-    D3_LAUNCH_CHECK();
-    return 0;
+    float *g = (float *)ws;
+    if (S > 0) cluster_gather_kernel<<<(int)((S * 3 + 255) / 256), 256, 0, s>>>(coords, clusters_idx, g, S);
+    return cluster_stats_launch(g, offsets, mean, cmin, cmax, nProposal, nullptr, s);
 }
 extern "C" int d3_cluster_transform(const float *coords, const int *clusters_idx, const float *mean, const float *scale,
                                     const float *offset, long long *out, long long S, void *stream) {
diff --git a/d3net_amd/csrc/voxelize.hip b/d3net_amd/csrc/voxelize.hip
--- a/d3net_amd/csrc/voxelize.hip
+++ b/d3net_amd/csrc/voxelize.hip
@@ -134,6 +134,63 @@
     }
 }
 
+__global__ void voxelize_gather_fp_kernel(const float *__restrict__ feats, const int *__restrict__ rows, int rstride, float *__restrict__ out,
+                                          const int *__restrict__ rules, long long total, int maxActive, int nPlanes, bool average) {
+    long long e = (long long)blockIdx.x * blockDim.x + threadIdx.x;
+    if (e >= total) return;
+    const int row = (int)(e / nPlanes), plane = (int)(e % nPlanes);
+    const int *r = rules + (long long)row * (maxActive + 1);
+#define VG_N 8
+#define VG_IDS(ID, I0) _Pragma("unroll") for (int j = 0; j < VG_N; j++) ID[j] = r[(I0) + j <= maxActive ? (I0) + j : 1]
+#define VG_PTS(PT, ID) _Pragma("unroll") for (int j = 0; j < VG_N; j++) PT[j] = rows[(long long)ID[j] * rstride]
+    int id1[VG_N], id2[VG_N] = {}, pt0[VG_N], pt1[VG_N] = {};
+    const int nActive = r[0];
+    VG_IDS(id1, 1);
+    VG_PTS(pt0, id1);
+    if (nActive > VG_N) { VG_IDS(id1, 1 + VG_N); }
+    const float multiplier = (average && nActive > 0) ? __fdiv_rn(1.0f, (float)nActive) : 1.0f;
+    float acc = 0.f;
+    for (int i0 = 1; i0 <= nActive; i0 += VG_N) {
+        float vn[VG_N];
+#pragma unroll
+        for (int j = 0; j < VG_N; j++) vn[j] = feats[(long long)pt0[j] * nPlanes + plane];
+        if (i0 + VG_N <= nActive) { VG_PTS(pt1, id1); }
+        if (i0 + 2 * VG_N <= nActive) { VG_IDS(id2, i0 + 2 * VG_N); }
+#pragma unroll
+        for (int j = 0; j < VG_N; j++)
+            if (i0 + j <= nActive) acc = __fadd_rn(acc, __fmul_rn(multiplier, vn[j]));
+#pragma unroll
+        for (int j = 0; j < VG_N; j++) { pt0[j] = pt1[j]; id1[j] = id2[j]; }
+    }
+    out[e] = acc;
+}
+__global__ void voxelize_gather_bp_kernel(const float *__restrict__ d_out, float *__restrict__ d_feats, const int *__restrict__ rows, int rstride,
+                                          const int *__restrict__ rules, long long total, int maxActive, int nPlanes, bool average) {
+    long long e = (long long)blockIdx.x * blockDim.x + threadIdx.x;
+    if (e >= total) return;
+    const int row = (int)(e / nPlanes), plane = (int)(e % nPlanes);
+    const int *r = rules + (long long)row * (maxActive + 1);
+    int id1[VG_N], id2[VG_N] = {}, pt0[VG_N], pt1[VG_N] = {};
+    const int nActive = r[0];
+    VG_IDS(id1, 1);
+    VG_PTS(pt0, id1);
+    if (nActive > VG_N) { VG_IDS(id1, 1 + VG_N); }
+    const float multiplier = (average && nActive > 0) ? __fdiv_rn(1.0f, (float)nActive) : 1.0f;
+    const float g = __fmul_rn(multiplier, d_out[e]);
+    for (int i0 = 1; i0 <= nActive; i0 += VG_N) {
+        if (i0 + VG_N <= nActive) { VG_PTS(pt1, id1); }
+        if (i0 + 2 * VG_N <= nActive) { VG_IDS(id2, i0 + 2 * VG_N); }
+#pragma unroll
+        for (int j = 0; j < VG_N; j++)
+            if (i0 + j <= nActive) atomicAdd(&d_feats[(long long)pt0[j] * nPlanes + plane], g);
+#pragma unroll
+        for (int j = 0; j < VG_N; j++) { pt0[j] = pt1[j]; id1[j] = id2[j]; }
+    }
+}
+#undef VG_IDS
+#undef VG_N
+#undef VG_PTS
+
 static int launch_fp(const float *feats, float *out, const int *rules, int nActive, int maxActive, int nPlane,
                      bool average, void *stream) {
     long long total = (long long)nActive * nPlane;
@@ -177,6 +234,28 @@
                               int nActive, int maxActive, int nPlane, void *stream) {
     D3_CLEAR();
     return launch_bp(d_output_feats, d_feats, output_map, nActive, maxActive, nPlane, mode == 4, stream);
+}
+extern "C" int d3_voxelize_gather_fp(const float *feats, const int *rows, int rstride, float *output_feats, const int *output_map, int mode,
+                                     int nActive, int maxActive, int nPlane, void *stream) {
+    D3_CLEAR();
+    if (rstride < 1 || maxActive < 1) return D3_ERR_ARG;
+    const long long total = (long long)nActive * nPlane;
+    if (total <= 0) return 0;
+    voxelize_gather_fp_kernel<<<(int)((total + 255) / 256), 256, 0, d3_stream(stream)>>>(feats, rows, rstride, output_feats, output_map, total,
+                                                                                       maxActive, nPlane, mode == 4);
+    D3_LAUNCH_CHECK();
+    return 0;
+}
+extern "C" int d3_voxelize_gather_bp(const float *d_output_feats, float *d_feats, const int *rows, int rstride, const int *output_map, int mode,
+                                     int nActive, int maxActive, int nPlane, void *stream) {
+    D3_CLEAR();
+    if (rstride < 1 || maxActive < 1) return D3_ERR_ARG;
+    const long long total = (long long)nActive * nPlane;
+    if (total <= 0) return 0;
+    voxelize_gather_bp_kernel<<<(int)((total + 255) / 256), 256, 0, d3_stream(stream)>>>(d_output_feats, d_feats, rows, rstride, output_map, total,
+                                                                                       maxActive, nPlane, mode == 4);
+    D3_LAUNCH_CHECK();
+    return 0;
 }
 extern "C" int d3_point_recover_fp(const float *feats, float *output_feats, const int *idx_map, int nActive,
                                    int maxActive, int nPlane, void *stream) {
@@ -314,10 +393,11 @@
     }
     (void)scalars;
 }
-__global__ void vi_max_kernel(const int *__restrict__ cnt, int n, int *scalars) {
+__global__ void vi_max_kernel(const int *__restrict__ cnt, int n, int *scalars, int *__restrict__ cursor) {
     const int i = blockIdx.x * blockDim.x + threadIdx.x, lane = threadIdx.x & 63;
     const int M = scalars[0];
     if ((int)(blockIdx.x * blockDim.x) >= M) return;
+    if (i < M && i < n) cursor[i] = 0;
     int c = (i < M && i < n) ? cnt[i] : 0;
     for (int o = 32; o > 0; o >>= 1) c = max(c, __shfl_xor(c, o));
     if (lane == 0 && c > 0 && c > __hip_atomic_load(&scalars[1], __ATOMIC_RELAXED, __HIP_MEMORY_SCOPE_AGENT)) atomicMax(&scalars[1], c);
@@ -347,7 +427,7 @@
     vi_assign_kernel<<<nb, T, 0, s>>>(w.flag, w.scan, w.slot_of, w.slot_vid, n);
     vi_p2v_kernel<<<nb, T, 0, s>>>(w.slot_of, w.slot_vid, input_map, w.cnt, n, w.scalars);
     vi_total_kernel<<<1, 64, 0, s>>>(w.flag, w.scan, n, w.scalars);
-    vi_max_kernel<<<nb, T, 0, s>>>(w.cnt, n, w.scalars);
+    vi_max_kernel<<<nb, T, 0, s>>>(w.cnt, n, w.scalars, w.scan);
     D3_LAUNCH_CHECK();
     int h[3];
     D3_CHECK(hipMemcpyAsync(h, w.scalars, sizeof(h), hipMemcpyDeviceToHost, s));
@@ -388,6 +468,73 @@
     out_coords[e] = coords[(size_t)firstListed * ncols + j];
 }
 
+#define VI_LIST_MAX 512
+__global__ void vi_scatter_kernel(const int *__restrict__ input_map, const int *__restrict__ vstart, int *__restrict__ cursor,
+                                  int *__restrict__ pts, int n) {
+    const int i = blockIdx.x * blockDim.x + threadIdx.x, lane = threadIdx.x & 63;
+    const bool live = i < n;
+    const int v = live ? input_map[i] : -1;
+    const int prev = __shfl_up(v, 1);
+    const bool head = live && (lane == 0 || prev != v);
+    const unsigned long long heads = __ballot(head), lives = __ballot(live);
+    int base = 0;
+    if (head) {
+        const unsigned long long above = (lane == 63) ? 0ull : (heads >> (lane + 1)) << (lane + 1);
+        const int end = above ? (int)__builtin_ctzll(above) : 64;
+        const unsigned long long span = (end == 64 ? ~0ull : ((1ull << end) - 1ull)) & ~((1ull << lane) - 1ull);
+        base = atomicAdd(&cursor[v], (int)__popcll(span & lives));
+    }
+    const unsigned long long below = heads & (lane == 63 ? ~0ull : ((2ull << lane) - 1ull));
+    const int hl = below ? 63 - __builtin_clzll(below) : lane;
+    base = __shfl(base, hl);
+    if (live) pts[vstart[v] + base + (lane - hl)] = i;
+}
+__global__ __launch_bounds__(256) void vi_rules_list_kernel(const int *__restrict__ cnt, const int *__restrict__ vstart,
+                                                            const int *__restrict__ pts_all, int *__restrict__ cursor,
+                                                            int *__restrict__ out_map, int M, int maxActive, int gshift,
+                                                            const int64_t *__restrict__ coords, int ncols, int64_t *__restrict__ out_coords) {
+    __shared__ __attribute__((aligned(16))) int strip[4][VI_LIST_MAX];
+    const int G = 1 << gshift, w = maxActive + 1;
+    const long long t = (long long)blockIdx.x * blockDim.x + threadIdx.x;
+    const long long v = t >> gshift;
+    if (v >= M) return;
+    const int j0 = (int)(t & (G - 1)), lane = threadIdx.x & 63;
+    const int c = min(cnt[v], maxActive);
+    const int *pts = pts_all + vstart[v];
+    int *row = out_map + v * w;
+    if (j0 == 0) cursor[v] = 0;
+    for (int j = j0; j < w; j += G)
+        if (j == 0) row[0] = c; else if (j > c) row[j] = 0;
+    if (c <= G) {
+        const int x = j0 < c ? pts[j0] : 0x7FFFFFFF;
+        const int gb = lane & ~(G - 1);
+        int rank = 0;
+        for (int k = 0; k < c; k++) rank += (__shfl(x, gb + k) < x) ? 1 : 0;
+        if (j0 < c) {
+            row[1 + rank] = x;
+            if (rank == 0)
+                for (int q = 0; q < ncols; q++) out_coords[v * ncols + q] = coords[(size_t)x * ncols + q];
+        }
+    } else {
+        int *l = strip[threadIdx.x >> 6];
+        for (int j = lane; j < ((c + 3) & ~3); j += 64) l[j] = j < c ? pts[j] : 0x7FFFFFFF;
+        __builtin_amdgcn_fence(__ATOMIC_RELEASE, "wavefront");
+        __builtin_amdgcn_wave_barrier();
+        __builtin_amdgcn_fence(__ATOMIC_ACQUIRE, "wavefront");
+        for (int j = lane; j < c; j += 64) {
+            const int x = l[j];
+            int rank = 0;
+            for (int k = 0; k < c; k += 4) {
+                const int4 q = *(const int4 *)(l + k);
+                rank += (q.x < x ? 1 : 0) + (q.y < x ? 1 : 0) + (q.z < x ? 1 : 0) + (q.w < x ? 1 : 0);
+            }
+            row[1 + rank] = x;
+            if (rank == 0)
+                for (int q = 0; q < ncols; q++) out_coords[v * ncols + q] = coords[(size_t)x * ncols + q];
+        }
+    }
+}
+
 __global__ void vi_iota_kernel(int *a, int n) {
     int i = blockIdx.x * blockDim.x + threadIdx.x;
     if (i < n) a[i] = i;
@@ -404,15 +551,22 @@
     const int T = 256;
     int rc = d3_exclusive_scan_i32(w.cnt, w.vstart, M, w.temp, w.temp_bytes, s);
     if (rc) return rc;
-    vi_iota_kernel<<<(n + T - 1) / T, T, 0, s>>>(w.flag, n);
-    int bits = 1; while ((1ll << bits) < (long long)M && bits < 31) bits++;
-    rc = d3_sort_pairs_i32(input_map, w.sorted_keys, w.flag, w.sorted_pts, n, bits, w.temp, w.temp_bytes, s);
-    if (rc) return rc;
     int gshift = 0; while ((1 << gshift) < maxActive + 1 && gshift < 6) gshift++;
     const long long rthreads = (long long)M << gshift;
-    vi_rules_kernel<<<(int)((rthreads + T - 1) / T), T, 0, s>>>(mode, w.cnt, w.vstart, w.sorted_pts, output_map, M, maxActive, gshift);
-    vi_coords_kernel<<<(M * ncols + T - 1) / T, T, 0, s>>>(coords, ncols, mode, w.cnt, w.vstart, w.sorted_pts,
-                                                         output_coords, M);
-    D3_LAUNCH_CHECK();
-    return 0;
-}
+    const bool lists = (mode == 3 || mode == 4) && maxActive <= VI_LIST_MAX;
+    if (lists) {
+        vi_scatter_kernel<<<(n + T - 1) / T, T, 0, s>>>(input_map, w.vstart, w.scan, w.sorted_pts, n);
+        vi_rules_list_kernel<<<(int)((rthreads + T - 1) / T), T, 0, s>>>(w.cnt, w.vstart, w.sorted_pts, w.scan, output_map, M, maxActive, gshift,
+                                                                         coords, ncols, output_coords);
+    } else {
+        vi_iota_kernel<<<(n + T - 1) / T, T, 0, s>>>(w.flag, n);
+        int bits = 1; while ((1ll << bits) < (long long)M && bits < 31) bits++;
+        rc = d3_sort_pairs_i32(input_map, w.sorted_keys, w.flag, w.sorted_pts, n, bits, w.temp, w.temp_bytes, s);
+        if (rc) return rc;
+        vi_rules_kernel<<<(int)((rthreads + T - 1) / T), T, 0, s>>>(mode, w.cnt, w.vstart, w.sorted_pts, output_map, M, maxActive, gshift);
+        vi_coords_kernel<<<(M * ncols + T - 1) / T, T, 0, s>>>(coords, ncols, mode, w.cnt, w.vstart, w.sorted_pts,
+                                                             output_coords, M);
+    }
+    D3_LAUNCH_CHECK();
+    return 0;
+}
diff --git a/d3net_amd/pointgroup.py b/d3net_amd/pointgroup.py
--- a/d3net_amd/pointgroup.py
+++ b/d3net_amd/pointgroup.py
@@ -354,8 +354,6 @@
 
     def clusters_voxelization(self, clusters_idx, clusters_offset, feats, coords, fullscale, scale, mode, rand=None):
         dev = feats.device
-        c_idxs = clusters_idx[:, 1].long()
-        clusters_feats = heads.gather_cluster_rows(feats, c_idxs)
         _mark("cv_gather")
         clusters_coords_mean, raw_min, raw_max = pointgroup_ops.cluster_coords_stats(coords, clusters_idx, clusters_offset)
         _mark("cv_sec_mean")
@@ -372,7 +370,7 @@
         voxel_coords, p2v_map, v2p_map = pointgroup_ops.voxelization_idx(clusters_coords, n_clusters, mode)
         _mark("cv_voxelization_idx")
         cm = self._begin_maps("score_net", voxel_coords)
-        voxel_feats = pointgroup_ops.voxelization(clusters_feats, v2p_map, mode)
+        voxel_feats = pointgroup_ops.cluster_voxelization(feats.contiguous(), clusters_idx, v2p_map, mode)
         voxel_feats = ME.SparseTensor(features=voxel_feats, coordinates=None if cm is not None else voxel_coords.int(), coordinate_manager=cm)
         voxel_feats.v2p_map = v2p_map
         return voxel_feats, p2v_map, (clusters_center, clusters_size)
diff --git a/d3net_amd/pointgroup_ops.py b/d3net_amd/pointgroup_ops.py
--- a/d3net_amd/pointgroup_ops.py
+++ b/d3net_amd/pointgroup_ops.py
@@ -125,6 +125,39 @@
 voxelization = Voxelization.apply
 
 
+class ClusterVoxelization(Function):
+
+    @staticmethod
+    def forward(ctx, feats, clusters_idx, map_rule, mode=4):
+        assert map_rule.is_contiguous() and map_rule.is_cuda and map_rule.dtype == torch.int32
+        assert clusters_idx.is_contiguous() and clusters_idx.is_cuda and clusters_idx.dtype == torch.int32 and clusters_idx.dim() == 2 \
+            and clusters_idx.size(1) == 2
+        assert feats.is_contiguous() and feats.is_cuda and feats.dtype == torch.float32
+        N, Cc = feats.size()
+        M = map_rule.size(0)
+        maxActive = map_rule.size(1) - 1
+        output_feats = torch.empty((M, Cc), dtype=torch.float32, device=feats.device)
+        ctx.for_backwards = (clusters_idx, map_rule, mode, maxActive, N)
+        with _on(feats.device):
+            check(_lib.lib().d3_voxelize_gather_fp(_ptr(feats), C.c_void_p(clusters_idx.data_ptr() + 4), 2, _ptr(output_feats), _ptr(map_rule),
+                                                   int(mode), M, maxActive, Cc, _stream()), "voxelize_gather_fp")
+        return output_feats
+
+    @staticmethod
+    def backward(ctx, d_output_feats):
+        clusters_idx, map_rule, mode, maxActive, N = ctx.for_backwards
+        M, Cc = d_output_feats.size()
+        d_output_feats = d_output_feats.contiguous()
+        d_feats = torch.zeros((N, Cc), dtype=torch.float32, device=d_output_feats.device)
+        with _on(d_feats.device):
+            check(_lib.lib().d3_voxelize_gather_bp(_ptr(d_output_feats), _ptr(d_feats), C.c_void_p(clusters_idx.data_ptr() + 4), 2,
+                                                   _ptr(map_rule), int(mode), M, maxActive, Cc, _stream()), "voxelize_gather_bp")
+        return d_feats, None, None, None
+
+
+cluster_voxelization = ClusterVoxelization.apply
+
+
 class PointRecover(Function):
     @staticmethod
     def forward(ctx, feats, map_rule, nPoint):
diff --git a/include/d3hip.h b/include/d3hip.h
--- a/include/d3hip.h
+++ b/include/d3hip.h
@@ -51,6 +51,10 @@
                     int nActive, int maxActive, void *stream);
 int d3_voxelize_bp(const float *d_output_feats, float *d_feats, const int *output_map, int mode, int nActive,
                    int maxActive, int nPlane, void *stream);
+int d3_voxelize_gather_fp(const float *feats, const int *rows, int rstride, float *output_feats, const int *output_map, int mode,
+                          int nActive, int maxActive, int nPlane, void *stream);
+int d3_voxelize_gather_bp(const float *d_output_feats, float *d_feats, const int *rows, int rstride, const int *output_map, int mode,
+                          int nActive, int maxActive, int nPlane, void *stream);
 int d3_point_recover_fp(const float *feats, float *output_feats, const int *idx_map, int nActive,
                         int maxActive, int nPlane, void *stream);
 int d3_point_recover_bp(const float *d_output_feats, float *d_feats, const int *idx_map, int nActive,
```

Measured after the change: 254.5, median of 3. Within noise of the previous version (+0.8%).
